# Lab-LVM/imagenet-models

Hardware: AMD Instinct MI355X
Metric: images/sec (whole node) GA-ConvNeXt-T 3x224x224 bf16 training step (higher is better)
Workload: dtype bf16; 1 GPU; ga_convnext_tiny_768 train step (fwd + GA loss lam=-0.8 + bwd + all-reduce + adamw lr=0), batch 256/GPU, drop_path 0.2, synthetic 3x224x224; global_batch=256, parallelism=dp1, dist_backend=none, grad_exchange=torch, allreduce_buckets=0

## Files before the change

### imagenet-models_amd/_lib.py

```python
import ctypes as C
import os

_HERE = os.path.dirname(os.path.abspath(__file__))
LIB_PATH = os.environ.get('GAEXT_LIB') or os.path.join(_HERE, 'csrc', 'libgaext.so')

GA_F32, GA_BF16 = 0, 1
ACT_NONE, ACT_GELU, ACT_RELU = 0, 1, 2
A_PLAIN, A_PATCH2, A_STEM4_NCHW, A_CONV3, A_CONV3S2, A_NEIGH2 = 0, 1, 2, 3, 4, 5
C_PLAIN, C_UNPATCH2 = 0, 1

vp, i32, i64, f32 = C.c_void_p, C.c_int, C.c_int64, C.c_float


class GemmDesc(C.Structure):
    _fields_ = [
        ('M', i32), ('N', i32), ('K', i32), ('batch', i32), ('dtype', i32),
        ('A', vp), ('lda', i64), ('strideA', i64), ('a_batch_mod', i32), ('a_kind', i32),
        ('a_H', i32), ('a_W', i32), ('a_C', i32), ('a_act', i32),
        ('B', vp), ('ldb', i64), ('strideB', i64),
        ('C', vp), ('ldc', i64), ('strideC', i64), ('c_kind', i32),
        ('c_H', i32), ('c_W', i32), ('c_C', i32), ('c_f32', i32), ('C2', vp), ('c2_mode', i32),
        ('alpha', f32), ('bias', vp), ('strideBias', i64), ('act', i32),
        ('H', vp), ('ldh', i64), ('strideH', i64), ('h_is_deriv', i32),
        ('rowscale', vp), ('rows_per_scale', i32),
        ('R', vp), ('ldr', i64), ('strideR', i64), ('relu_after', i32),
        ('colsum', vp), ('colsumsq', vp), ('strideCol', i64),
    ]


class WgradDesc(C.Structure):
    _fields_ = [
        ('M', i32), ('N', i32), ('K', i32), ('batch', i32), ('dtype', i32),
        ('Y', vp), ('ldy', i64), ('strideY', i64),
        ('X', vp), ('ldx', i64), ('strideX', i64), ('x_batch_mod', i32), ('x_kind', i32),
        ('x_H', i32), ('x_W', i32), ('x_C', i32), ('x_act', i32),
        ('dW', vp), ('ldw', i64), ('strideW', i64),
        ('dbias', vp), ('strideDbias', i64),
        ('alpha', f32), ('split_m', i32), ('accumulate', i32), ('workspace', vp), ('ws_bytes', i64),
    ]


class WprepDesc(C.Structure):
    _fields_ = [
        ('w', vp), ('G', i32), ('Co', i32), ('Ci', i32), ('KH', i32), ('KW', i32),
        ('rs', vp), ('cs', vp), ('row_perm', vp), ('dtype', i32),
        ('out', vp), ('ldo', i64), ('outT', vp), ('ldt', i64), ('flip', i32), ('stem', i32), ('t_cols', i32),
    ]


class WunfoldDesc(C.Structure):
    _fields_ = [
        ('G', vp), ('ldg', i64), ('gb', vp), ('W', vp), ('b', vp), ('rs', vp), ('cs', vp), ('v', vp), ('row_perm', vp),
        ('N', i32), ('Ci', i32), ('KH', i32), ('KW', i32), ('stem', i32),
        ('dW', vp), ('db', vp), ('d_rs', vp), ('d_cs', vp), ('d_v', vp),
    ]


class SmallDesc(C.Structure):
    _fields_ = [('kind', i32), ('y', vp), ('x', vp), ('a', f32), ('n', i64), ('R', i32), ('C', i32), ('accumulate', i32),
                ('b', vp), ('rs', vp), ('v', vp), ('row_perm', vp)]


class CswinAttnDesc(C.Structure):
    _fields_ = [('B', i32), ('reso', i32), ('C', i32), ('heads', i32), ('nbranch', i32),
                ('Hs', i32 * 2), ('Ws', i32 * 2), ('lepe_w', vp * 2), ('lepe_b', vp * 2),
                ('scale', f32), ('dtype', i32), ('qkv', vp), ('ldq', i64), ('out', vp), ('ldo', i64)]


class MlpDesc(C.Structure):
    _fields_ = [('X', vp), ('ldx', i64), ('W1', vp), ('ldw1', i64), ('b1', vp), ('W2', vp), ('ldw2', i64), ('b2', vp),
                ('R', vp), ('ldr', i64), ('rowscale', vp), ('rows_per_scale', i32), ('Y', vp), ('ldy', i64),
                ('M', i64), ('C', i32), ('H', i32), ('dtype', i32)]


class MlpBwdDesc(C.Structure):
    _fields_ = [('X', vp), ('ldx', i64), ('DY', vp), ('lddy', i64), ('W1', vp), ('ldw1', i64), ('b1', vp),
                ('W2T', vp), ('ldw2t', i64), ('W1T', vp), ('ldw1t', i64), ('A', vp), ('lda', i64), ('DH', vp), ('lddh', i64),
                ('DX', vp), ('lddx', i64), ('M', i64), ('C', i32), ('H', i32), ('dtype', i32)]


class SmallLinearDesc(C.Structure):
    _fields_ = [('rows', i32), ('groups', i32), ('Ng', i32), ('Kg', i32), ('A', vp), ('lda', i64), ('a_gstride', i64), ('a_perm', vp),
                ('W', vp), ('bias', vp), ('col_scale', vp), ('rowscale', vp), ('rows_per_scale', i32), ('R', vp), ('ldr', i64),
                ('Y', vp), ('ldy', i64), ('Yraw', vp), ('dtype', i32)]


class AttnDesc(C.Structure):
    _fields_ = [('B', i32), ('N', i32), ('H', i32), ('hd', i32), ('scale', f32), ('dtype', i32), ('qkv', vp), ('ldq', i64),
                ('out', vp), ('ldo', i64), ('lse', vp)]


_SIGS = {
    'ga_version': ([], i32),
    'ga_last_error': ([C.c_char_p, C.c_size_t], i32),
    'ga_device_info': ([C.POINTER(i32), C.POINTER(i32), C.POINTER(i32)], i32),
    'ga_comm_unique_id': ([vp], i32),
    'ga_comm_init': ([C.POINTER(vp), i32, i32, vp], i32),
    'ga_comm_destroy': ([vp], i32),
    'ga_comm_info': ([vp, C.POINTER(i32), C.POINTER(i32)], i32),
    'ga_allreduce_workspace': ([i64, i32], C.c_size_t),
    'ga_allreduce_bucket': ([vp, vp, i64, i32, f32, vp, C.c_size_t, vp], i32),
    'ga_reduce_scatter_bucket': ([vp, vp, vp, i64, f32, vp], i32),
    'ga_allgather_bucket': ([vp, vp, vp, i64, vp], i32),
    'ga_comm_broadcast': ([vp, vp, i64, i32, vp], i32),
    'ga_set_knob': ([C.c_char_p, i32], i32),
    'ga_unset_knob': ([C.c_char_p], i32),
    'ga_config_string': ([C.c_char_p, C.c_size_t], i32),
    'ga_gemm': ([C.POINTER(GemmDesc), vp], i32),
    'ga_wgrad': ([C.POINTER(WgradDesc), vp], i32),
    'ga_weight_prep': ([C.POINTER(WprepDesc), vp], i32),
    'ga_bias_fold': ([vp, vp, vp, vp, vp, vp, i32, i32, vp], i32),
    'ga_weight_unfold': ([C.POINTER(WunfoldDesc), vp], i32),
    'ga_dwconv7_fwd': ([vp, vp, vp, vp, i32, i32, i32, i32, i32, vp], i32),
    'ga_dwconv7_bwd_data': ([vp, vp, vp, vp, i32, i32, i32, i32, i32, vp], i32),
    'ga_dwconv7_bwd_data2': ([vp, vp, vp, vp, vp, vp, i32, i32, i32, i32, i32, vp], i32),
    'ga_dwconv7_bwd_weight': ([vp, vp, vp, vp, i32, i32, i32, i32, i32, vp, C.c_size_t, vp], i32),
    'ga_dwconv7_bwd_weight_workspace': ([i32, i32, i32, i32, i32], C.c_size_t),
    'ga_dwconv3_fwd': ([vp, vp, vp, i32, i32, i32, i32, i32, vp, vp, i32, vp], i32),
    'ga_dwconv3_bwd_data': ([vp, vp, vp, i32, i32, i32, i32, i32, i32, vp], i32),
    'ga_dwconv3_bwd_weight': ([vp, vp, vp, i32, i32, i32, i32, i32, i32, vp, C.c_size_t, vp], i32),
    'ga_dwconv3_bwd_weight_workspace': ([i32, i32, i32, i32, i32, i32], C.c_size_t),
    'ga_maxpool3s2_fwd': ([vp, vp, vp, i32, i32, i32, i32, i32, vp], i32),
    'ga_maxpool3s2_bwd': ([vp, vp, vp, i32, i32, i32, i32, i32, i32, vp], i32),
    'ga_bn_gelu_fwd': ([vp, vp, vp, vp, i64, i32, i32, vp], i32),
    'ga_bn_gelu_bwd_workspace': ([i64, i32], C.c_size_t),
    'ga_bn_gelu_bwd_reduce': ([vp, vp, vp, vp, vp, vp, vp, vp, i64, i32, i32, vp, C.c_size_t, vp], i32),
    'ga_bn_gelu_bwd_apply': ([vp, vp, vp, vp, vp, vp, vp, vp, vp, i64, vp, i64, i32, i32, vp], i32),
    'ga_se_bn_fwd': ([vp, i32, vp, vp, vp, vp, vp, vp, vp, vp, vp, vp, vp, vp, vp, vp, i32, i32, i32, i32, vp], i32),
    'ga_se_bn_bwd': ([vp, vp, vp, vp, vp, vp, vp, vp, i32, vp, vp, vp, vp, vp, vp, vp, vp, vp, vp, vp, vp, vp, vp, vp, vp, vp, vp, vp,
                      vp, vp, i32, i32, i32, vp], i32),
    'ga_se_residual_fwd': ([vp, vp, vp, vp, vp, vp, vp, vp, vp, i32, i32, i32, i32, vp], i32),
    'ga_se_residual_bwd_a': ([vp, vp, vp, vp, vp, vp, vp, vp, i32, i32, i32, i32, vp], i32),
    'ga_se_residual_bwd_b': ([vp, vp, vp, vp, vp, vp, vp, vp, vp, vp, vp, i32, i32, i32, i32, vp], i32),
    'ga_subsample2_fwd': ([vp, vp, i32, i32, i32, i32, i32, vp], i32),
    'ga_subsample2_bwd': ([vp, vp, i32, i32, i32, i32, i32, i32, vp], i32),
    'ga_wgrad_workspace': ([C.POINTER(WgradDesc)], C.c_size_t),
    'ga_layernorm_fwd': ([vp, vp, vp, vp, vp, vp, i64, i32, f32, i32, vp], i32),
    'ga_layernorm_bwd': ([vp, vp, vp, vp, vp, vp, vp, vp, vp, i64, i32, i32, i32, vp], i32),
    'ga_layernorm_bwd_dp': ([vp, vp, vp, vp, vp, vp, vp, vp, vp, i64, i32, i32, vp, vp, i64, i32, vp], i32),
    'ga_bn_finalize': ([vp, vp, i64, vp, vp, f32, f32, vp, vp, vp, vp, vp, vp, i32, i32, vp], i32),
    'ga_affine_act': ([vp, vp, vp, vp, vp, i64, vp, i64, i32, i32, i32, i64, vp], i32),
    'ga_bn_bwd_reduce': ([vp, vp, vp, vp, vp, vp, i64, vp, vp, i64, i32, i32, i64, vp], i32),
    'ga_bn_bwd_apply': ([vp, vp, vp, vp, vp, vp, vp, vp, vp, i64, i64, vp, i64, i32, i32, i64, i64, vp], i32),
    'ga_pool_concat_fwd': ([vp, vp, i32, i32, i32, i32, i32, i32, i32, i32, i32, i32, vp], i32),
    'ga_pool_concat_bwd': ([vp, vp, vp, i32, i32, i32, i32, i32, i32, i32, i32, i32, i32, vp], i32),
    'ga_spatial_sum': ([vp, vp, vp, i32, i32, i32, f32, i32, vp], i32),
    'ga_se_mlp_fwd': ([vp, vp, vp, vp, vp, vp, vp, i32, i32, i32, vp], i32),
    'ga_se_mlp_bwd': ([vp, vp, vp, vp, vp, vp, vp, f32, vp, vp, vp, vp, i32, i32, i32, vp], i32),
    'ga_chan_scale': ([vp, vp, vp, vp, i32, i32, i32, i32, vp], i32),
    'ga_gram_pack_fwd': ([vp, vp, vp, i32, i32, i32, i32, i32, vp], i32),
    'ga_gram_pack_bwd': ([vp, vp, vp, vp, i32, i32, i32, i32, i32, vp], i32),
    'ga_gram_f64_fwd_workspace': ([i32, i32], C.c_size_t),
    'ga_gram_f64_bwd_workspace': ([i32, i32], C.c_size_t),
    'ga_gram_f64_fwd': ([vp, vp, vp, vp, C.c_size_t, i32, i32, i32, i32, i32, i32, i32, vp], i32),
    'ga_gram_f64_bwd': ([vp, vp, vp, vp, vp, vp, C.c_size_t, i32, i32, i32, i32, i32, i32, i32, vp], i32),
    'ga_token_cat': ([vp, vp, vp, i32, i32, i32, i32, vp], i32),
    'ga_token_split': ([vp, vp, vp, i32, i32, i32, i32, i32, i32, vp], i32),
    'ga_class_attn_fwd': ([vp, vp, vp, vp, i32, i32, i32, i32, f32, i32, vp], i32),
    'ga_class_attn_bwd': ([vp, vp, vp, vp, vp, vp, i32, i32, i32, i32, f32, i32, vp], i32),
    'ga_class_attn_fwd2': ([vp, vp, vp, i64, vp, vp, i32, i32, i32, i32, f32, i32, vp], i32),
    'ga_class_attn_bwd2': ([vp, vp, vp, vp, i64, vp, vp, vp, vp, i32, i32, i32, i32, f32, i32, vp], i32),
    'ga_loss_fwd_bwd': ([vp, vp, vp, vp, i32, i32, i32, f32, i32, f32, f32, i32, vp], i32),
    'ga_heads_topk': ([vp, i32, i32, i32, i32, vp, vp, vp], i32),
    'ga_sgd_step': ([vp, vp, vp, vp, i64, i32, f32, vp], i32),
    'ga_adamw_step': ([vp, vp, vp, vp, vp, i64, f32, vp], i32),
    'ga_weight_prep_batch': ([vp, i32, vp], i32),
    'ga_weight_unfold_batch': ([vp, i32, vp], i32),
    'ga_small_batch': ([vp, i32, vp], i32),
    'ga_cswin_attn_fwd': ([C.POINTER(CswinAttnDesc), vp], i32),
    'ga_cswin_attn_bwd_workspace': ([C.POINTER(CswinAttnDesc)], C.c_size_t),
    'ga_cswin_attn_bwd': ([C.POINTER(CswinAttnDesc), vp, vp, vp, C.c_size_t, vp], i32),
    'ga_cswin_lepe_wgrad_reduce': ([C.POINTER(CswinAttnDesc), vp, vp, vp, vp, vp, vp], i32),
    'ga_cswin_lepe_wgrad': ([C.POINTER(CswinAttnDesc), vp, vp, vp, vp, vp, vp], i32),
    'ga_layernorm_gelu_fwd': ([vp, vp, vp, vp, vp, vp, i64, i32, f32, i32, vp], i32),
    'ga_layernorm_gelu_bwd': ([vp, vp, vp, vp, vp, vp, vp, vp, vp, i64, i32, i32, vp], i32),
    'ga_nchw3_to_nhwc8': ([vp, vp, i32, i32, i32, i32, vp], i32),
    'ga_convw_pack': ([vp, vp, i32, i32, i32, i32, i64, i32, vp], i32),
    'ga_convw_unpack_grad': ([vp, vp, i32, i32, i32, i32, i64, vp], i32),
    'ga_conv3s2_dgrad_prep': ([vp, vp, i32, i32, i64, i32, vp], i32),
    'ga_gram_pack_fwd2': ([vp, vp, vp, i32, i32, i32, i32, i32, i32, vp], i32),
    'ga_gram_pack_bwd2': ([vp, vp, vp, vp, i32, i32, i32, i32, i32, i32, vp], i32),
    'ga_map_tokens_fwd': ([vp, vp, i32, i32, i32, i32, i32, vp], i32),
    'ga_map_tokens_bwd': ([vp, vp, i32, i32, i32, i32, i32, vp], i32),
    'ga_class_attn_mt_fwd': ([vp, vp, vp, i64, vp, vp, vp, i32, i32, i32, i32, i32, f32, i32, vp], i32),
    'ga_class_attn_mt_bwd': ([vp, vp, vp, vp, i64, vp, vp, vp, vp, vp, i64, i32, i32, i32, i32, i32, f32, i32, vp], i32),
    'ga_class_attn_mt_ia_fwd': ([vp, vp, vp, i64, vp, vp, vp, vp, vp, vp, vp, i32, i32, i32, i32, i32, f32, i32, vp], i32),
    'ga_class_attn_mt_ia_bwd': ([vp, vp, vp, vp, i64, vp, vp, vp, vp, vp, vp, vp, vp, i64, vp, vp, vp, vp, i32, i32, i32, i32, i32, f32, i32,
                                 vp], i32),
    'ga_map_loss_fwd_bwd': ([vp, vp, vp, vp, vp, vp, i32, i32, i32, f32, i32, f32, f32, i32, vp], i32),
    'ga_gelu_fwd': ([vp, vp, i64, i32, vp], i32),
    'ga_gelu_bwd': ([vp, vp, vp, i64, i32, vp], i32),
    'ga_relu_drop': ([vp, vp, vp, vp, i64, i32, vp], i32),
    'ga_mask_mul': ([vp, vp, vp, vp, i64, i32, vp], i32),
    'ga_copy2d': ([vp, i64, vp, i64, i64, i32, i32, i32, vp], i32),
    'ga_dropout_mask_sample': ([vp, i64, f32, C.c_uint64, vp, vp], i32),
    'ga_drop_path_sample': ([vp, vp, i32, i32, C.c_uint64, vp, vp], i32),
    'ga_loss_dense_fwd_bwd': ([vp, vp, vp, vp, vp, vp, vp, i32, i32, i32, f32, i32, f32, f32, f32, i32, vp], i32),
    'ga_u8_normalize': ([vp, vp, i32, i32, i32, i32, C.POINTER(f32), C.POINTER(f32), vp], i32),
    'ga_input_erase': ([vp, i32, vp, i32, i32, i32, i32, C.POINTER(f32), C.POINTER(f32), vp, i32, i32, C.c_uint64, C.c_uint64, vp], i32),
    'ga_mixup_batch': ([vp, vp, i32, i32, i32, i32, C.c_double, i32, i32, i32, i32, i32, vp], i32),
    'ga_mixup_target': ([vp, vp, i32, i32, C.c_double, C.c_double, vp], i32),
    'ga_agc_clip': ([vp, vp, vp, i32, f32, f32, vp], i32),
    'ga_small_linear_fwd': ([C.POINTER(SmallLinearDesc), vp], i32),
    'ga_small_linear_bwd': ([C.POINTER(SmallLinearDesc), vp, vp, i32, vp, vp, vp, vp], i32),
    'ga_colstats': ([vp, i64, i32, i32, vp, vp, i32, vp], i32),
    'ga_pad_copy_f32': ([vp, vp, i64, i64, i64, i64, i32, vp], i32),
    'ga_pad_copy': ([vp, vp, i64, i64, i64, i64, i32, i32, vp], i32),
    'ga_stem4_ln_fwd': ([vp, vp, i64, vp, vp, vp, vp, vp, vp, vp, i32, i32, i32, i32, f32, vp], i32),
    'ga_blockdiag_f32': ([vp, vp, i64, i32, i32, i32, i64, i32, i32, vp], i32),
    'ga_pad_groups_f32': ([vp, vp, i64, i64, i32, i32, i32, i32, i32, i32, vp], i32),
    'ga_attn_fwd': ([C.POINTER(AttnDesc), vp], i32),
    'ga_attn_bwd_workspace': ([C.POINTER(AttnDesc)], C.c_size_t),
    'ga_attn_bwd': ([C.POINTER(AttnDesc), vp, vp, vp, C.c_size_t, vp], i32),
    'ga_patchify': ([vp, vp, i32, i32, i32, i32, i32, i32, vp], i32),
    'ga_vit_embed_fwd': ([vp, vp, vp, vp, i32, i32, i32, i32, vp], i32),
    'ga_vit_embed_bwd': ([vp, vp, vp, vp, i32, i32, i32, i32, vp], i32),
    'ga_patchify_strided': ([vp, vp, i32, i32, i32, i32, i32, i32, i32, vp], i32),
    'ga_pos_add_fwd': ([vp, vp, vp, i32, i32, i32, i32, vp], i32),
    'ga_pos_add_bwd': ([vp, vp, i32, i32, i32, i32, vp], i32),
    'ga_dwpool_fwd': ([vp, vp, vp, vp, i32, i32, i32, i32, i32, i32, vp], i32),
    'ga_dwpool_bwd_data': ([vp, vp, vp, i32, i32, i32, i32, i32, i32, vp], i32),
    'ga_dwpool_bwd_weight': ([vp, vp, vp, vp, i32, i32, i32, i32, i32, i32, vp], i32),
    'ga_resize_concat_fwd': ([vp, vp, i32, i32, i32, i32, i32, i32, i64, i32, i32, vp], i32),
    'ga_resize_concat_bwd': ([vp, vp, i32, i32, i32, i32, i32, i32, i64, i32, i32, vp], i32),
    'ga_rows_bcast': ([vp, vp, i32, i32, i32, f32, i32, vp], i32),
    'ga_token_gap_fwd': ([vp, vp, i32, i32, i32, i32, vp], i32),
    'ga_token_gap_bwd': ([vp, vp, i32, i32, i32, i32, vp], i32),
    'ga_mlp_supported': ([i32, i32, i32], i32),
    'ga_mlp_fwd': ([C.POINTER(MlpDesc), vp], i32),
    'ga_mlp_bwd': ([C.POINTER(MlpBwdDesc), vp], i32),
    'ga_memset': ([vp, i32, C.c_size_t, vp], i32),
    'ga_transpose_f32': ([vp, vp, i32, i32, i32, vp], i32),
    'ga_axpy_f32': ([vp, vp, f32, i64, vp], i32),
    'ga_lerp_f32': ([vp, vp, f32, i64, vp], i32),
    'ga_sumsq_f32': ([vp, i64, vp, vp], i32),
    'ga_lamb_stage1': ([vp, vp, vp, vp, vp, vp, vp, vp, i32, vp, vp], i32),
    'ga_lamb_stage2': ([vp, vp, vp, vp, i32, vp, vp], i32),
    'ga_clip_grad_f32': ([vp, i64, vp, f32, i32, vp], i32),
    'ga_rowscale': ([vp, vp, vp, i64, i64, i32, vp], i32),
    'ga_cast_from_f32': ([vp, vp, i64, i32, vp], i32),
    'ga_cast_to_f32': ([vp, vp, i64, i32, vp], i32),
}

_lib = None


def load():
    global _lib
    if _lib is not None:
        return _lib
    if not os.path.exists(LIB_PATH):
        raise RuntimeError(f'libgaext.so not found at {LIB_PATH}: build it with `make -C {os.path.dirname(LIB_PATH)}` '
                           f'(there is no CPU fallback for the product path)')
    lib = C.CDLL(LIB_PATH)
    for name, (argtypes, restype) in _SIGS.items():
        fn = getattr(lib, name)
        fn.argtypes = argtypes
        fn.restype = restype
    _lib = lib
    return lib


def last_error():
    buf = C.create_string_buffer(512)
    load().ga_last_error(buf, 512)
    return buf.value.decode(errors='replace')


def config_string():
    buf = C.create_string_buffer(1024)
    load().ga_config_string(buf, 1024)
    s = buf.value.decode(errors='replace')
    host = sorted(k for k in os.environ if k.startswith(('GAEXT_', 'GA_FUSED_MLP')) and k != 'GAEXT_LIB')
    known = {'GAEXT_ASYNC_WGRAD', 'GAEXT_FWD_SPLIT', 'GAEXT_PAR_BRANCH', 'GAEXT_FWD_SKEW', 'GAEXT_FUSE_DP', 'GAEXT_HEAD_STREAMS',
             'GA_FUSED_MLP', 'GAEXT_SMALL_SINGLE', 'GAEXT_SYNC_DEBUG'}
    for k in host:
        if k in known:
            s += f' host:{k}={os.environ[k]}'
    if os.environ.get('GAEXT_LIB'):
        s += f' lib={os.environ["GAEXT_LIB"]}'
    return s


class knobs:

    def __init__(self, **kv):
        self.kv = kv

    def __enter__(self):
        lib = load()
        for k, v in self.kv.items():
            check(lib.ga_set_knob(k.encode(), int(v)), f'ga_set_knob({k})')
        return self

    def __exit__(self, *exc):
        lib = load()
        for k in self.kv:
            lib.ga_unset_knob(k.encode())
        return False


def check(rc, what):
    if rc != 0:
        raise RuntimeError(f'libgaext {what} failed (code {rc}): {last_error()}')


def exported_symbols():
    return sorted(_SIGS)
```

### imagenet-models_amd/csrc/mlp.hip

```cpp
#include <stdlib.h>
#include <algorithm>
#include "common.h"

namespace {

constexpr int BM = 128;

__device__ __forceinline__ void lds_barrier() { asm volatile("s_waitcnt lgkmcnt(0)\n\ts_barrier" ::: "memory"); }

__device__ __forceinline__ unsigned slab_off(int r, int c) { return r * 64 + ((c ^ ((r >> 2) & 3)) << 4); }

__device__ __forceinline__ bf16x8_t frag(const unsigned char* slab, int r0, int lane) {
    return *reinterpret_cast<const bf16x8_t*>(slab + slab_off(r0 + (lane & 15), lane >> 4));
}

template <int ROWS, int KS, int NTHR>
__device__ __forceinline__ void stage_rows(unsigned char* dst, const bf16_t* src, long ld, long row0, long limit) {
    constexpr int CPR = KS * 4, NP = ROWS * CPR / NTHR;
    static_assert(ROWS * CPR % NTHR == 0, "tile must split evenly over the threads");
    u32x4_t v[NP];
#pragma unroll
    for (int i = 0; i < NP; ++i) {
        const int idx = threadIdx.x + NTHR * i;
        const int r = idx / CPR, c = idx - r * CPR;
        v[i] = u32x4_t{0, 0, 0, 0};
        if (row0 + r < limit) v[i] = __builtin_nontemporal_load(reinterpret_cast<const u32x4_t*>(src + (row0 + r) * ld + c * 8));
    }
#pragma unroll
    for (int i = 0; i < NP; ++i) {
        const int idx = threadIdx.x + NTHR * i;
        const int r = idx / CPR, c = idx - r * CPR;
        *reinterpret_cast<u32x4_t*>(dst + (c >> 2) * ROWS * 64 + slab_off(r, c & 3)) = v[i];
    }
}

template <int C, int NTHR> struct RowPre {
    static constexpr int P8 = C / 8, RG = NTHR / P8, NR = (64 + RG - 1) / RG;
};
template <int C, int NTHR> using PreArr = u32x4_t[BM / 64][RowPre<C, NTHR>::NR];
template <int C, int NTHR>
__device__ __forceinline__ void rows_prefetch(PreArr<C, NTHR>& v, const bf16_t* R, long ldr, long m0, long M) {
    using P = RowPre<C, NTHR>;
    const int c8 = threadIdx.x % P::P8, rg = threadIdx.x / P::P8;
#pragma unroll
    for (int piece = 0; piece < BM / 64; ++piece)
#pragma unroll
        for (int it = 0; it < P::NR; ++it) {
            const int row = rg + it * P::RG;
            const long m = m0 + piece * 64 + row;
            v[piece][it] = u32x4_t{0, 0, 0, 0};
            if (rg < P::RG && row < 64 && m < M) v[piece][it] = __builtin_nontemporal_load(reinterpret_cast<const u32x4_t*>(R + m * ldr + c8 * 8));
        }
}

template <int C, int NTHR, int NWM, int TM>
__device__ __forceinline__ void store_rows(float* Cs, const f32x4_t (&acc)[C / 32][TM], int wm, int wn, int lane, long m0, long M,
                                           const float* bias, const float* rowscale, int rps, bool has_r,
                                           const PreArr<C, NTHR>& pre, bf16_t* Y, long ldy) {
    constexpr int LDC = C + 4, P8 = C / 8, RG = NTHR / P8, WROWS = 16 * TM, WPH = 64 / WROWS;
    constexpr int NR = (64 + RG - 1) / RG;
    const int c8 = threadIdx.x % P8, rg = threadIdx.x / P8;
    float bv[8];
#pragma unroll
    for (int j = 0; j < 8; ++j) bv[j] = bias ? bias[c8 * 8 + j] : 0.f;
#pragma unroll
    for (int piece = 0; piece < NWM / WPH; ++piece) {
        if (piece) __syncthreads();
        if (wm / WPH == piece) {
#pragma unroll
            for (int tn = 0; tn < C / 32; ++tn)
#pragma unroll
                for (int tm = 0; tm < TM; ++tm) {
                    const int row = (wm % WPH) * WROWS + 16 * tm + (lane & 15), col = wn * (C / 2) + 16 * tn + 4 * (lane >> 4);
                    *reinterpret_cast<f32x4_t*>(Cs + row * LDC + col) = acc[tn][tm];
                }
        }
        __syncthreads();
        if (rg < RG) {
#pragma unroll
            for (int it = 0; it < NR; ++it) {
                const int row = rg + it * RG;
                const long m = m0 + piece * 64 + row;
                if (row >= 64 || m >= M) break;
                const f32x4_t a = *reinterpret_cast<const f32x4_t*>(Cs + row * LDC + c8 * 8);
                const f32x4_t b = *reinterpret_cast<const f32x4_t*>(Cs + row * LDC + c8 * 8 + 4);
                float v[8] = {a[0], a[1], a[2], a[3], b[0], b[1], b[2], b[3]};
#pragma unroll
                for (int j = 0; j < 8; ++j) v[j] += bv[j];
                if (rowscale) {
                    const float s = rowscale[m / rps];
#pragma unroll
                    for (int j = 0; j < 8; ++j) v[j] *= s;
                }
                if (has_r) {
                    float r[8];
                    const u32x4_t q = pre[piece][it];
                    unpack8(make_uint4(q.x, q.y, q.z, q.w), r);
#pragma unroll
                    for (int j = 0; j < 8; ++j) v[j] += r[j];
                }
                store8_nt(Y + m * ldy + c8 * 8, v);
            }
        }
    }
}

template <int C, int HC>
__global__ __launch_bounds__(256, 2) void mlp_fwd_kernel(const ga_mlp_desc d) {
    constexpr int KS1 = C / 32, KS2 = HC / 32, TN1 = HC / 32, TN2 = C / 32;
    constexpr int XS = KS1 * BM * 64, W1S = KS1 * HC * 64, AS = KS2 * BM * 64;
    constexpr int NI = HC * C / 8 / 256;
    static_assert(HC * C / 8 % 256 == 0, "weight chunk must split evenly");
    extern __shared__ __attribute__((aligned(16))) unsigned char smem[];
    unsigned char* Xs = smem;
    unsigned char* W1s = Xs + XS;
    unsigned char* As = W1s + W1S;
    unsigned char* W2s = As + AS;
    float* B1s = reinterpret_cast<float*>(W2s + KS2 * C * 64);
    const int tid = threadIdx.x, lane = tid & 63, wave = tid >> 6, wm = wave >> 1, wn = wave & 1, g = lane >> 4;
    const long m0 = (long)blockIdx.x * BM;
    const bf16_t* W1 = reinterpret_cast<const bf16_t*>(d.W1);
    const bf16_t* W2 = reinterpret_cast<const bf16_t*>(d.W2);

    u32x4_t w1r[NI], w2r[NI];
    auto w_load = [&](int j0) {
#pragma unroll
        for (int i = 0; i < NI; ++i) {
            const int idx = tid + 256 * i;
            const int r1 = idx / (KS1 * 4), c1 = idx - r1 * (KS1 * 4);
            w1r[i] = *reinterpret_cast<const u32x4_t*>(W1 + (long)(j0 + r1) * d.ldw1 + c1 * 8);
            const int r2 = idx / (HC / 8), c2 = idx - r2 * (HC / 8);
            w2r[i] = *reinterpret_cast<const u32x4_t*>(W2 + (long)r2 * d.ldw2 + j0 + c2 * 8);
        }
    };
    auto w1_store = [&]() {
#pragma unroll
        for (int i = 0; i < NI; ++i) {
            const int idx = tid + 256 * i;
            const int r1 = idx / (KS1 * 4), c1 = idx - r1 * (KS1 * 4);
            *reinterpret_cast<u32x4_t*>(W1s + (c1 >> 2) * HC * 64 + slab_off(r1, c1 & 3)) = w1r[i];
        }
    };
    auto w2_store = [&]() {
#pragma unroll
        for (int i = 0; i < NI; ++i) {
            const int idx = tid + 256 * i;
            const int r2 = idx / (HC / 8), c2 = idx - r2 * (HC / 8);
            *reinterpret_cast<u32x4_t*>(W2s + (c2 >> 2) * C * 64 + slab_off(r2, c2 & 3)) = w2r[i];
        }
    };

    w_load(0);
    stage_rows<BM, KS1, 256>(Xs, reinterpret_cast<const bf16_t*>(d.X), d.ldx, m0, d.M);
    for (int i = tid; i < 4 * C; i += 256) B1s[i] = d.b1[i];
    w1_store();
    w2_store();
    __syncthreads();

    f32x4_t y[TN2][4];
#pragma unroll
    for (int i = 0; i < TN2; ++i)
#pragma unroll
        for (int j = 0; j < 4; ++j) y[i][j] = f32x4_t{0.f, 0.f, 0.f, 0.f};
    auto round = [&](const int j0, const bool more) __attribute__((always_inline)) {
        if (more) w_load(j0 + HC);
        f32x4_t h[TN1][4];
#pragma unroll
        for (int i = 0; i < TN1; ++i)
#pragma unroll
            for (int j = 0; j < 4; ++j) h[i][j] = f32x4_t{0.f, 0.f, 0.f, 0.f};
#pragma unroll
        for (int ks = 0; ks < KS1; ++ks) {
            bf16x8_t xf[4];
#pragma unroll
            for (int tm = 0; tm < 4; ++tm) xf[tm] = frag(Xs + ks * BM * 64, wm * 64 + 16 * tm, lane);
#pragma unroll
            for (int tn = 0; tn < TN1; ++tn) {
                const bf16x8_t wf = frag(W1s + ks * HC * 64, wn * (HC / 2) + 16 * tn, lane);
#pragma unroll
                for (int tm = 0; tm < 4; ++tm) h[tn][tm] = __builtin_amdgcn_mfma_f32_16x16x32_bf16(wf, xf[tm], h[tn][tm], 0, 0, 0);
            }
        }
#pragma unroll
        for (int tn = 0; tn < TN1; ++tn) {
            const int nl = wn * (HC / 2) + 16 * tn + 4 * g;
            const float4 b = *reinterpret_cast<const float4*>(B1s + j0 + nl);
            const float bb[4] = {b.x, b.y, b.z, b.w};
#pragma unroll
            for (int tm = 0; tm < 4; ++tm) {
                float a[4], unused;
#pragma unroll
                for (int r = 0; r < 4; ++r) gelu_both_fast(h[tn][tm][r] + bb[r], a[r], unused);
                const int row = wm * 64 + 16 * tm + (lane & 15);
                uint2 p;
                p.x = pack2bf(a[0], a[1]);
                p.y = pack2bf(a[2], a[3]);
                *reinterpret_cast<uint2*>(As + (nl >> 5) * BM * 64 + slab_off(row, (nl & 31) >> 3) + (nl & 7) * 2) = p;
            }
        }
        lds_barrier();
#pragma unroll
        for (int ks = 0; ks < KS2; ++ks) {
            bf16x8_t af[4];
#pragma unroll
            for (int tm = 0; tm < 4; ++tm) af[tm] = frag(As + ks * BM * 64, wm * 64 + 16 * tm, lane);
#pragma unroll
            for (int tn = 0; tn < TN2; ++tn) {
                const bf16x8_t wf = frag(W2s + ks * C * 64, wn * (C / 2) + 16 * tn, lane);
#pragma unroll
                for (int tm = 0; tm < 4; ++tm) y[tn][tm] = __builtin_amdgcn_mfma_f32_16x16x32_bf16(wf, af[tm], y[tn][tm], 0, 0, 0);
            }
        }
        if (more) w1_store();
        lds_barrier();
        if (more) w2_store();
    };
    for (int j0 = 0; j0 + HC < d.H; j0 += HC) round(j0, true);
    u32x4_t rpre[BM / 64][RowPre<C, 256>::NR];
    if (d.R) rows_prefetch<C, 256>(rpre, reinterpret_cast<const bf16_t*>(d.R), d.ldr, m0, d.M);
    round(d.H - HC, false);
    store_rows<C, 256, 2, 4>(reinterpret_cast<float*>(smem), y, wm, wn, lane, m0, d.M, d.b2, d.rowscale, d.rows_per_scale,
                             d.R != nullptr, rpre, reinterpret_cast<bf16_t*>(d.Y), d.ldy);
}

template <int C, int HC> constexpr int fwd_lds() {
    constexpr int ab = (C / 32) * BM * 64 + (C / 32) * HC * 64 + (HC / 32) * BM * 64 + (HC / 32) * C * 64 + 16 * C;
    constexpr int st = 64 * (C + 4) * 4;
    return ab > st ? ab : st;
}

template <int C, int HC>
__global__ __launch_bounds__(512, 1) void mlp_bwd_kernel(const ga_mlp_bwd_desc d) {
    constexpr int KS1 = C / 32, KS2 = HC / 32, TN1 = HC / 32, TN2 = C / 32;
    constexpr int XS = KS1 * BM * 64, WS = KS1 * HC * 64, TS = KS2 * BM * 64;
    constexpr int NPC = HC * C / 8, NI = (NPC + 511) / 512;
    extern __shared__ __attribute__((aligned(16))) unsigned char smem[];
    unsigned char* Xs = smem;
    unsigned char* Ds = Xs + XS;
    unsigned char* W1s = Ds + XS;
    unsigned char* W2Ts = W1s + WS;
    unsigned char* W1Ts = W2Ts + WS;
    unsigned char* DHs = W1Ts + KS2 * C * 64;
    unsigned char* A2s = DHs + TS;
    float* B1s = reinterpret_cast<float*>(A2s + TS);
    const int tid = threadIdx.x, lane = tid & 63, wave = tid >> 6, wm = wave >> 1, wn = wave & 1, g = lane >> 4;
    const long m0 = (long)blockIdx.x * BM;
    const bf16_t* W1 = reinterpret_cast<const bf16_t*>(d.W1);
    const bf16_t* W2T = reinterpret_cast<const bf16_t*>(d.W2T);
    const bf16_t* W1T = reinterpret_cast<const bf16_t*>(d.W1T);
    bf16_t* Aout = reinterpret_cast<bf16_t*>(d.A);
    bf16_t* DHout = reinterpret_cast<bf16_t*>(d.DH);

    u32x4_t w1r[NI], w2r[NI], w3r[NI];
    auto w_load = [&](int j0) {
#pragma unroll
        for (int i = 0; i < NI; ++i) {
            const int idx = NPC % 512 == 0 ? tid + 512 * i : min(tid + 512 * i, NPC - 1);
            const int r1 = idx / (KS1 * 4), c1 = idx - r1 * (KS1 * 4);
            w1r[i] = *reinterpret_cast<const u32x4_t*>(W1 + (long)(j0 + r1) * d.ldw1 + c1 * 8);
            w2r[i] = *reinterpret_cast<const u32x4_t*>(W2T + (long)(j0 + r1) * d.ldw2t + c1 * 8);
            const int r3 = idx / (HC / 8), c3 = idx - r3 * (HC / 8);
            w3r[i] = *reinterpret_cast<const u32x4_t*>(W1T + (long)r3 * d.ldw1t + j0 + c3 * 8);
        }
    };
    auto w12_store = [&]() {
#pragma unroll
        for (int i = 0; i < NI; ++i) {
            const int idx = NPC % 512 == 0 ? tid + 512 * i : min(tid + 512 * i, NPC - 1);
            const int r1 = idx / (KS1 * 4), c1 = idx - r1 * (KS1 * 4);
            const unsigned o = (c1 >> 2) * HC * 64 + slab_off(r1, c1 & 3);
            *reinterpret_cast<u32x4_t*>(W1s + o) = w1r[i];
            *reinterpret_cast<u32x4_t*>(W2Ts + o) = w2r[i];
        }
    };
    auto w3_store = [&]() {
#pragma unroll
        for (int i = 0; i < NI; ++i) {
            const int idx = NPC % 512 == 0 ? tid + 512 * i : min(tid + 512 * i, NPC - 1);
            const int r3 = idx / (HC / 8), c3 = idx - r3 * (HC / 8);
            *reinterpret_cast<u32x4_t*>(W1Ts + (c3 >> 2) * C * 64 + slab_off(r3, c3 & 3)) = w3r[i];
        }
    };

    w_load(0);
    stage_rows<BM, KS1, 512>(Xs, reinterpret_cast<const bf16_t*>(d.X), d.ldx, m0, d.M);
    stage_rows<BM, KS1, 512>(Ds, reinterpret_cast<const bf16_t*>(d.DY), d.lddy, m0, d.M);
    for (int i = tid; i < 4 * C; i += 512) B1s[i] = d.b1[i];
    w12_store();
    w3_store();
    __syncthreads();

    f32x4_t dx[TN2][2];
#pragma unroll
    for (int i = 0; i < TN2; ++i)
#pragma unroll
        for (int j = 0; j < 2; ++j) dx[i][j] = f32x4_t{0.f, 0.f, 0.f, 0.f};

    for (int j0 = 0; j0 < d.H; j0 += HC) {
        const bool more = j0 + HC < d.H;
        if (more) w_load(j0 + HC);
        f32x4_t h[TN1][2], t[TN1][2];
#pragma unroll
        for (int i = 0; i < TN1; ++i)
#pragma unroll
            for (int j = 0; j < 2; ++j) h[i][j] = t[i][j] = f32x4_t{0.f, 0.f, 0.f, 0.f};
#pragma unroll
        for (int ks = 0; ks < KS1; ++ks) {
            bf16x8_t xf[2], df[2];
#pragma unroll
            for (int tm = 0; tm < 2; ++tm) {
                xf[tm] = frag(Xs + ks * BM * 64, wm * 32 + 16 * tm, lane);
                df[tm] = frag(Ds + ks * BM * 64, wm * 32 + 16 * tm, lane);
            }
#pragma unroll
            for (int tn = 0; tn < TN1; ++tn) {
                const bf16x8_t w1f = frag(W1s + ks * HC * 64, wn * (HC / 2) + 16 * tn, lane);
                const bf16x8_t w2f = frag(W2Ts + ks * HC * 64, wn * (HC / 2) + 16 * tn, lane);
#pragma unroll
                for (int tm = 0; tm < 2; ++tm) {
                    h[tn][tm] = __builtin_amdgcn_mfma_f32_16x16x32_bf16(w1f, xf[tm], h[tn][tm], 0, 0, 0);
                    t[tn][tm] = __builtin_amdgcn_mfma_f32_16x16x32_bf16(w2f, df[tm], t[tn][tm], 0, 0, 0);
                }
            }
        }
#pragma unroll
        for (int tn = 0; tn < TN1; ++tn) {
            const int nl = wn * (HC / 2) + 16 * tn + 4 * g;
            const float4 b = *reinterpret_cast<const float4*>(B1s + j0 + nl);
            const float bb[4] = {b.x, b.y, b.z, b.w};
#pragma unroll
            for (int tm = 0; tm < 2; ++tm) {
                float a[4], dh[4];
#pragma unroll
                for (int r = 0; r < 4; ++r) {
                    float gr;
                    gelu_both_fast(h[tn][tm][r] + bb[r], a[r], gr);
                    dh[r] = t[tn][tm][r] * gr;
                }
                const int row = wm * 32 + 16 * tm + (lane & 15);
                const unsigned o = (nl >> 5) * BM * 64 + slab_off(row, (nl & 31) >> 3) + (nl & 7) * 2;
                uint2 p;
                p.x = pack2bf(a[0], a[1]);
                p.y = pack2bf(a[2], a[3]);
                *reinterpret_cast<uint2*>(A2s + o) = p;
                p.x = pack2bf(dh[0], dh[1]);
                p.y = pack2bf(dh[2], dh[3]);
                *reinterpret_cast<uint2*>(DHs + o) = p;
            }
        }
        lds_barrier();
#pragma unroll
        for (int ks = 0; ks < KS2; ++ks) {
            bf16x8_t af[2];
#pragma unroll
            for (int tm = 0; tm < 2; ++tm) af[tm] = frag(DHs + ks * BM * 64, wm * 32 + 16 * tm, lane);
#pragma unroll
            for (int tn = 0; tn < TN2; ++tn) {
                const bf16x8_t wf = frag(W1Ts + ks * C * 64, wn * (C / 2) + 16 * tn, lane);
#pragma unroll
                for (int tm = 0; tm < 2; ++tm) dx[tn][tm] = __builtin_amdgcn_mfma_f32_16x16x32_bf16(wf, af[tm], dx[tn][tm], 0, 0, 0);
            }
        }
        {
            constexpr int PPR = HC / 8, NP = BM * PPR / 512;
            static_assert(BM * PPR % 512 == 0, "chunk rows must split evenly");
#pragma unroll
            for (int i = 0; i < NP; ++i) {
                const int idx = tid + 512 * i;
                const int r = idx / PPR, c = idx - r * PPR;
                const long m = m0 + r;
                if (m < d.M) {
                    const unsigned o = (c >> 2) * BM * 64 + slab_off(r, c & 3);
                    store16_nt(Aout + m * d.lda + j0 + c * 8, *reinterpret_cast<const uint4*>(A2s + o));
                    store16_nt(DHout + m * d.lddh + j0 + c * 8, *reinterpret_cast<const uint4*>(DHs + o));
                }
            }
        }
        if (more) w12_store();
        lds_barrier();
        if (more) w3_store();
    }
    u32x4_t nopre[BM / 64][RowPre<C, 512>::NR];
#pragma unroll
    for (int i = 0; i < BM / 64; ++i)
#pragma unroll
        for (int j = 0; j < RowPre<C, 512>::NR; ++j) nopre[i][j] = u32x4_t{0, 0, 0, 0};
    store_rows<C, 512, 4, 2>(reinterpret_cast<float*>(smem), dx, wm, wn, lane, m0, d.M, nullptr, nullptr, 1, false, nopre,
                             reinterpret_cast<bf16_t*>(d.DX), d.lddx);
}

template <int C, int HC> constexpr int bwd_lds() {
    return 2 * (C / 32) * BM * 64 + 2 * (C / 32) * HC * 64 + (HC / 32) * C * 64 + 2 * (HC / 32) * BM * 64 + 16 * C;
}

bool aligned16(const void* p) { return (reinterpret_cast<uintptr_t>(p) & 15) == 0; }

template <typename K> bool set_lds(K kern, size_t bytes) {
    return bytes <= 65536 ||
           hipFuncSetAttribute(reinterpret_cast<const void*>(kern), hipFuncAttributeMaxDynamicSharedMemorySize, (int)bytes) == hipSuccess;
}

}

extern "C" int ga_mlp_supported(int C, int H, int dtype) { return dtype == GA_BF16 && H == 4 * C && (C == 96 || C == 192); }

extern "C" int ga_mlp_fwd(const ga_mlp_desc* d, ga_stream_t stream) {
    GA_REQUIRE(d && d->X && d->W1 && d->b1 && d->W2 && d->Y && d->M > 0, "ga_mlp_fwd: null / empty descriptor");
    GA_REQUIRE(ga_mlp_supported(d->C, d->H, d->dtype), "ga_mlp_fwd: C=%d H=%d dtype=%d has no fused form (ga_mlp_supported)", d->C,
               d->H, d->dtype);
    GA_REQUIRE(aligned16(d->X) && aligned16(d->W1) && aligned16(d->W2) && aligned16(d->Y) && aligned16(d->b1) &&
                   (!d->R || aligned16(d->R)) && d->ldx % 8 == 0 && d->ldw1 % 8 == 0 && d->ldw2 % 8 == 0 && d->ldy % 8 == 0 &&
                   (!d->R || d->ldr % 8 == 0) && d->ldx >= d->C && d->ldw1 >= d->C && d->ldw2 >= d->H && d->ldy >= d->C,
               "ga_mlp_fwd: operands must be 16-byte aligned with leading dimensions in multiples of 8");
    GA_REQUIRE(!d->rowscale || d->rows_per_scale > 0, "ga_mlp_fwd: rows_per_scale");
    hipStream_t s = reinterpret_cast<hipStream_t>(stream);
    const unsigned grid = (unsigned)((d->M + BM - 1) / BM);
    if (d->C == 96) {
        constexpr int lds = fwd_lds<96, 64>();
        GA_REQUIRE(set_lds(mlp_fwd_kernel<96, 64>, lds), "ga_mlp_fwd: LDS");
        hipLaunchKernelGGL((mlp_fwd_kernel<96, 64>), dim3(grid), dim3(256), lds, s, *d);
    } else {
        constexpr int lds = fwd_lds<192, 32>();
        GA_REQUIRE(set_lds(mlp_fwd_kernel<192, 32>, lds), "ga_mlp_fwd: LDS");
        hipLaunchKernelGGL((mlp_fwd_kernel<192, 32>), dim3(grid), dim3(256), lds, s, *d);
    }
    return ga_check_launch("ga_mlp_fwd");
}

extern "C" int ga_mlp_bwd(const ga_mlp_bwd_desc* d, ga_stream_t stream) {
    GA_REQUIRE(d && d->X && d->DY && d->W1 && d->b1 && d->W2T && d->W1T && d->A && d->DH && d->DX && d->M > 0,
               "ga_mlp_bwd: null / empty descriptor");
    GA_REQUIRE(ga_mlp_supported(d->C, d->H, d->dtype), "ga_mlp_bwd: C=%d H=%d dtype=%d has no fused form (ga_mlp_supported)", d->C,
               d->H, d->dtype);
    GA_REQUIRE(aligned16(d->X) && aligned16(d->DY) && aligned16(d->W1) && aligned16(d->W2T) && aligned16(d->W1T) &&
                   aligned16(d->A) && aligned16(d->DH) && aligned16(d->DX) && aligned16(d->b1) && d->ldx % 8 == 0 &&
                   d->lddy % 8 == 0 && d->ldw1 % 8 == 0 && d->ldw2t % 8 == 0 && d->ldw1t % 8 == 0 && d->lda % 8 == 0 &&
                   d->lddh % 8 == 0 && d->lddx % 8 == 0 && d->ldx >= d->C && d->lddy >= d->C && d->ldw1 >= d->C &&
                   d->ldw2t >= d->C && d->ldw1t >= d->H && d->lda >= d->H && d->lddh >= d->H && d->lddx >= d->C,
               "ga_mlp_bwd: operands must be 16-byte aligned with leading dimensions in multiples of 8");
    hipStream_t s = reinterpret_cast<hipStream_t>(stream);
    const unsigned grid = (unsigned)((d->M + BM - 1) / BM);
    if (d->C == 96) {
        constexpr int lds = bwd_lds<96, 64>();
        GA_REQUIRE(set_lds(mlp_bwd_kernel<96, 64>, lds), "ga_mlp_bwd: LDS");
        hipLaunchKernelGGL((mlp_bwd_kernel<96, 64>), dim3(grid), dim3(512), lds, s, *d);
    } else {
        constexpr int lds = bwd_lds<192, 32>();
        GA_REQUIRE(set_lds(mlp_bwd_kernel<192, 32>, lds), "ga_mlp_bwd: LDS");
        hipLaunchKernelGGL((mlp_bwd_kernel<192, 32>), dim3(grid), dim3(512), lds, s, *d);
    }
    return ga_check_launch("ga_mlp_bwd");
}
```

### imagenet-models_amd/engine.py

```python
import contextlib
import os

import torch

from . import ops
from .ops import (A_CONV3, A_PATCH2, A_STEM4_NCHW, ACT_GELU, ASYNC_LANE, C_UNPATCH2, GA_BF16, GA_F32, Plan)


def pad8(n):
    return (n + 7) // 8 * 8


def tap_indices(nblocks, naggre):
    taps = []
    if nblocks > 5:
        for i in range(nblocks):
            if (i + 1) % (nblocks // (naggre + 1)) == 0 and len(taps) < naggre:
                taps.append(i)
    return taps


class GAFunction(torch.autograd.Function):

    @staticmethod
    def forward(ctx, eng, x, anchor):
        ctx.eng = eng
        return eng.forward(x)

    @staticmethod
    def backward(ctx, dlogits):
        ctx.eng.backward(dlogits)
        return None, None, None


class GAEngine:
    def __init__(self, model, batch, training, mode):
        self.m = model
        self.cfg = model.cfg
        self.B = batch
        self.training = training
        self.dt = GA_BF16 if mode == 'bf16' else GA_F32
        self.tdt = ops.torch_dtype(self.dt)
        flat = model.flat_state()
        self.dev = flat['params'].device
        self.P = dict(model.named_parameters())
        self.Bf = dict(model.named_buffers())
        self.bufs = {}
        self.tmps = {}
        self.async_wgrad = os.environ.get('GAEXT_ASYNC_WGRAD', '1') != '0'
        self.fwd_split = max(1, int(os.environ.get('GAEXT_FWD_SPLIT', '2')))
        self.par_branch = os.environ.get('GAEXT_PAR_BRANCH', '1') != '0'
        self.fwd_skew = int(os.environ.get('GAEXT_FWD_SKEW', '-1'))
        self._chain = None
        self._cur_stage = 0
        self._bwd_seq = 0
        self._pre_dyz = {}
        self.fuse_dp = os.environ.get('GAEXT_FUSE_DP', '1') != '0'
        self.sync_bn = getattr(model, 'sync_bn_comm', None)
        self.W = {}
        self.weights_dirty = True
        self.anchor = torch.zeros((), device=self.dev, requires_grad=True)
        self.input_descs = []
        self.blocks = {}
        self.x_ref = None
        self.img = 224
        self.dp_rates = self._drop_path_rates()
        self.dp_scale = {}
        if training:
            sites = [pre for pre, r in self.dp_rates.items() if r > 0]
            if sites:
                self.dp_all = torch.ones(len(sites), batch, device=self.dev)
                self.dp_keep = torch.tensor([1.0 - self.dp_rates[p] for p in sites], device=self.dev)
                self.dp_counter = torch.zeros(1, dtype=torch.int64, device=self.dev)
                self.dp_plan = Plan(name='droppath')
                self.dp_plan.drop_path_sample(self.dp_all, self.dp_keep, len(sites), batch, torch.initial_seed(), self.dp_counter)
                for i, pre in enumerate(sites):
                    self.dp_scale[pre] = self.dp_all[i]
        self.arena = None
        self.arena_off = 0
        if training:
            self.arena = torch.zeros(int(flat['total'] * 1.15) + (1 << 20) + self._arena_extra(), device=self.dev)
        self._nbt = [t for n, t in self.Bf.items() if n.endswith('num_batches_tracked')]
        self.prep = Plan(name='prep', defer_small=True)
        self.fwd = Plan(name='fwd')
        self.bwd = Plan(name='bwd', defer_small=True) if training else None
        self.bn_pool = torch.zeros(1 << 16, device=self.dev)
        self.bn_pool_off = 0
        self.bott_prefix = 'stages.4.'
        self.ppad, self.pgrad = {}, {}
        self.pad_gmlp = os.environ.get('GAEXT_PAD_GMLP', '1') != '0'
        self._build()
        assert not self.pgrad or getattr(self, '_unpadded', False), 'padded parameter gradients were never copied back'

    def buf(self, name, shape, dtype=None, zero=False):
        dtype = dtype or self.tdt
        if name not in self.bufs:
            self.bufs[name] = (torch.zeros if zero else torch.empty)(shape, dtype=dtype, device=self.dev)
        t = self.bufs[name]
        assert tuple(t.shape) == tuple(shape) and t.dtype == dtype, name
        return t

    def _chains(self):
        n = self.fwd_split if self.B >= 2 * self.fwd_split else 1
        if n <= 1:
            return [(0, 0, self.B)]
        per = self.B // n
        cuts = [s_ * per for s_ in range(n)] + [self.B]
        return [(1 + s_, cuts[s_], cuts[s_ + 1]) for s_ in range(n)]

    def _fsplits(self, HW):
        ch = getattr(self, '_chain', None)
        if ch is None:
            return [(0, 0, self.B * HW, 0, self.B)]
        lane, b0, b1 = ch
        return [(lane, b0 * HW, b1 * HW, b0, b1)]

    @contextlib.contextmanager
    def _wlane(self):
        Bk = self.bwd
        prev = Bk.lane
        if self.async_wgrad and prev == 0:
            Bk.lane = ASYNC_LANE
        try:
            yield
        finally:
            Bk.lane = prev

    def tmp(self, tag, shape, dtype=None):
        dtype = dtype or self.tdt
        key = (getattr(self, 'tmp_prefix', '') + tag, tuple(shape), dtype)
        if key not in self.tmps:
            self.tmps[key] = torch.empty(shape, dtype=dtype, device=self.dev)
        return self.tmps[key]

    def act(self, name, shape, dtype=None):
        return self.buf(name, shape, dtype)

    def blk_act(self, name, shape, dtype=None):
        return self.buf(name, shape, dtype) if self.training else self.tmp(name.rsplit('.', 1)[-1], shape, dtype)

    def gbuf(self, shape):
        n = 1
        for s in shape:
            n *= s
        off = (self.arena_off + 63) // 64 * 64
        assert off + n <= self.arena.numel(), 'gradient scratch arena too small'
        self.arena_off = off + n
        return self.arena[off:off + n].view(shape)

    def grad(self, name):
        return self.P[name].grad

    def _drop_path_rates(self):
        dep = self.cfg['depths']
        rate = self.cfg['drop_path_rate']
        pts = torch.linspace(0, rate, sum(dep)).split(list(dep))
        out = {}
        for i in range(4):
            for j in range(dep[i]):
                out[f'stages.{i}.blocks.{j}.'] = float(pts[i][j])
        out['stages.4.'] = float(rate)
        for k in range(self.cfg['branches']):
            out[f'gram_layer.{k}.blocks.0.'] = float(pts[-1][0])
            out[f'ga.{k}.'] = 0.0
        return out

    def sample_drop_path(self):
        if self.dp_scale:
            self.dp_plan.run()

    def set_drop_path_masks(self, masks):
        for pre, t in self.dp_scale.items():
            t.copy_(masks[pre].to(self.dev).float())

    NAMES = dict(stem_conv='stem.0.', stem_ln='stem.1.', ds_ln='stages.{i}.downsample.0.', ds_conv='stages.{i}.downsample.1.',
                 block='stages.{i}.blocks.{j}.', dw='conv_dw.', fc1='mlp.fc1.', fc2='mlp.fc2.')

    def _build(self):
        cfg = self.cfg
        d = cfg['dims']
        B, T, F = self.B, self.training, self.fwd
        dt = self.dt
        feats, taps, stage_in, _ = self._build_trunk()
        Hc = 14
        M4 = B * Hc * Hc
        ctot = sum(d[:-1]) + d[2] * cfg['naggre']
        cat = self.act('agg.cat', (M4, ctot))
        segs = [(feats[0][0], feats[0][1], d[0], 0), (feats[1][0], feats[1][1], d[1], 0)]
        segs += [(t, feats[2][1], d[2], 0) for t in taps]
        segs += [(feats[2][0], feats[2][1], d[2], 0), (feats[3][0], feats[3][1], d[3], 1)]
        off = 0
        self.agg_segs = []
        for src, hw, c, mode in segs:
            F.pool_concat_fwd(src, cat, B, hw, hw, c, Hc, Hc, ctot, off, mode, dt, label=f'agg.{off}')
            self.agg_segs.append((src, hw, c, mode, off))
            off += c
        assert off == ctot
        x4 = self._bottleneck_fwd(cat, M4, ctot, d[4])
        self.cout = d[4]
        self._build_heads(x4, M4, Hc)
        if T:
            self._build_backward(feats, taps, stage_in, x4, M4, ctot)
            if self.async_wgrad:
                self.bwd.join_async()
            self.bwd.flush('end.')
        self.prep.flush('prep.')

    def _build_trunk(self):
        cfg, nm = self.cfg, self.NAMES
        d, dep = cfg['dims'], cfg['depths']
        B, T, F = self.B, self.training, self.fwd
        dt = self.dt
        S0 = self.img // 4
        self.x_in = None
        M0 = B * S0 * S0
        if T:
            F.zero(self.bn_pool, label='zero.bn_sums')
        sc, sl = nm['stem_conv'], nm['stem_ln']
        Wst = self._w_plain(sc + 'weight', d[0], 3, 4, 4, stem=True, need_T=False)
        stem_pre = self.act('stem.pre', (M0, d[0]))
        self.x_placeholder = torch.zeros(8, device=self.dev)
        mean = self.act('stem.mean', (M0,), torch.float32)
        rstd = self.act('stem.rstd', (M0,), torch.float32)
        x = self.buf('stem.out', (M0, d[0]))
        self.stem_call = None
        if dt == GA_BF16 and d[0] in (96, 128) and self.img % 4 == 0 and os.environ.get('GAEXT_STEM_FUSED', '1') != '0':
            self.stem_call = len(F.calls)
            F.stem4_ln_fwd(self.x_placeholder, Wst, Wst.shape[1], self.P[sc + 'bias'], self.P[sl + 'weight'], self.P[sl + 'bias'],
                           stem_pre, x, mean, rstd, B, self.img, self.img, d[0], 1e-6, label='stem.conv+ln')
        else:
            F.gemm(self.x_placeholder, Wst, stem_pre, M0, d[0], 48, dt, a_kind=A_STEM4_NCHW, a_dims=(self.img, self.img, 3),
                   bias=self.P[sc + 'bias'], label='stem.conv')
            self.input_descs.append(self._last_desc(F))
            F.layernorm_fwd(stem_pre, self.P[sl + 'weight'], self.P[sl + 'bias'], x, mean, rstd, M0, d[0], 1e-6, dt,
                            label='stem.ln')
        x_stem = x
        chains = self._chains()
        skew_ev = None
        for ci, chain in enumerate(chains):
            self._chain = chain if len(chains) > 1 else None
            if self._chain is not None and skew_ev is not None:
                F.lane_wait(chain[0], skew_ev)
                skew_ev = None
            feats, taps = [], []
            x = x_stem
            res = S0
            stage_in = []
            for i in range(4):
                if i > 0:
                    Hp = res
                    res //= 2
                    Mi = B * res * res
                    Mp = B * Hp * Hp
                    pre = f'stages.{i}.downsample.'
                    pln, pcv = nm['ds_ln'].format(i=i), nm['ds_conv'].format(i=i)
                    ln = self.act(pre + 'ln', (Mp, d[i - 1]))
                    mean = self.act(pre + 'mean', (Mp,), torch.float32)
                    rstd = self.act(pre + 'rstd', (Mp,), torch.float32)
                    Wd = self._w_plain(pcv + 'weight', d[i], d[i - 1], 2, 2)
                    xo = self.buf(pre + 'out', (Mi, d[i]))
                    for lane, r0, r1, b0, b1 in self._fsplits(Hp * Hp):
                        F.lane = lane
                        F.layernorm_fwd(x[r0:r1], self.P[pln + 'weight'], self.P[pln + 'bias'], ln[r0:r1], mean[r0:r1],
                                        rstd[r0:r1], r1 - r0, d[i - 1], 1e-6, dt, label=pre + 'ln')
                        F.gemm(ln[r0:r1], Wd, xo[r0 // 4:r1 // 4], (r1 - r0) // 4, d[i], 4 * d[i - 1], dt, a_kind=A_PATCH2,
                               a_dims=(Hp, Hp, d[i - 1]), bias=self.P[pcv + 'bias'], label=pre + 'conv')
                    F.lane = 0
                    stage_in.append((x, Hp))
                    x = xo
                tap_at = tap_indices(dep[i], cfg['naggre']) if i == 2 else []
                for j in range(dep[i]):
                    x = self._block_fwd(nm['block'].format(i=i, j=j), x, res, d[i])
                    if j in tap_at:
                        taps.append(x)
                feats.append((x, res))
                if self._chain is not None and i == self.fwd_skew and ci + 1 < len(chains):
                    skew_ev = F.lane_signal(chain[0])
        self._chain = None
        return feats, taps, stage_in, x_stem

    def _build_heads(self, x4, M4, Hc):
        cfg, B, T, F, dt = self.cfg, self.B, self.training, self.fwd, self.dt
        cout = self.cout
        NC, K = cfg['num_classes'], cfg['branches']
        assert NC % 8 == 0, 'num_classes must be a multiple of 8 (pad the classifier)'
        self.logits = self.buf('logits', (K, B, NC), torch.float32)
        self.heads = []
        E_, nh_ = cfg['dim_embed'], cfg['num_heads']
        hd_ = E_ // max(nh_, 1)
        self.hd_p = pad8(hd_)
        self.Ea = nh_ * self.hd_p
        self.shared_tok = E_ % nh_ == 0 and self.Ea <= 512
        if self.shared_tok and self.Ea != E_:
            for k in range(K):
                pre = f'ga.{k}.attn.'
                pk, pv = self.P[pre + 'k.weight'], self.P[pre + 'v.weight']
                assert pv.data_ptr() == pk.data_ptr() + pk.numel() * 4, 'k/v weights must be adjacent in the flat buffer'
                spec = (('k.weight', (2 * self.Ea, cout), 2 * nh_, hd_ * cout, hd_ * cout, self.hd_p * cout),
                        ('q.weight', (self.Ea, cout), nh_, hd_ * cout, hd_ * cout, self.hd_p * cout),
                        ('proj.weight', (cout, self.Ea), cout * nh_, hd_, hd_, self.hd_p))
                for name, shape, rows, cols, lds, ldd in spec:
                    buf = self.buf('pad.' + pre + name, shape, torch.float32, zero=True)
                    self.prep.pad_copy_f32(self.P[pre + name], buf, rows, cols, lds, ldd, label='prep.pad.' + pre + name)
                    self.ppad[pre + name] = (buf, 'copy', (rows, cols, lds, ldd))
        if self.shared_tok:
            self.tok = dict(xn=self.act('ga.tok.xn', (M4, cout)), rstd=self.act('ga.tok.rstd', (M4,), torch.float32))
            F.layernorm_fwd(x4, None, None, self.tok['xn'], None, self.tok['rstd'], M4, cout, 1e-5, dt, label='ga.tok.ln')
            E2 = 2 * self.Ea
            tk = self.tok
            tk['E2'], tk['ld'] = E2, K * E2
            tk['W'] = self.buf('w.ga.kv_all', (K * E2, cout))
            tk['WT'] = self.buf('wT.ga.kv_all', (cout, K * E2)) if T else None
            tk['b'] = self.buf('w.ga.bkv_all', (K * E2,), torch.float32)
            P = self.P
            for k in range(K):
                pre = f'ga.{k}.'
                pk, pv = P[pre + 'attn.k.weight'], P[pre + 'attn.v.weight']
                assert pv.data_ptr() == pk.data_ptr() + pk.numel() * 4, 'k/v weights must be adjacent in the flat buffer'
                pk = self._pw(pre + 'attn.k.weight')
                self.prep.weight_prep(pk, 1, E2, cout, 1, 1, dt, out=tk['W'][k * E2:], ldo=cout,
                                      outT=tk['WT'][:, k * E2:] if T else None, ldt=K * E2 if T else 0,
                                      cs=P[pre + 'norm1.weight'], t_cols=E2, label='prep.' + pre + 'kv')
                self.prep.bias_fold(pk, None, None, P[pre + 'norm1.bias'], tk['b'][k * E2:], E2, cout)
            tk['kv'] = self.act('ga.kv_all', (M4, K * E2))
            F.gemm(tk['xn'], tk['W'], tk['kv'], M4, K * E2, cout, dt, bias=tk['b'], label='ga.kv_all')
        self._contract_all_fwd(x4, M4)
        fa = self.fc_all = dict(x=self.act('fc.all.x', (K, B, cout)))
        ldn = pad8(NC)
        fa['W'] = self.buf('w.fc.all', (K, NC, cout))
        fa['WT'] = self.buf('wT.fc.all', (K, cout, ldn)) if T else None
        fa['b'] = self.buf('w.fc.ball', (K, NC), torch.float32)
        for k in range(K):
            self.prep.weight_prep(self.P[f'fc.{k}.weight'], 1, NC, cout, 1, 1, dt, out=fa['W'][k], ldo=cout,
                                  outT=fa['WT'][k] if T else None, ldt=ldn if T else 0, label=f'prep.fc.{k}')
            self.prep.bias_fold(None, self.P[f'fc.{k}.bias'], None, None, fa['b'][k], NC, cout)
        self.head_lanes = int(os.environ.get('GAEXT_HEAD_STREAMS', '5')) if self.shared_tok else 1
        for k in range(K):
            if self.head_lanes > 1:
                F.lane, self.tmp_prefix = 1 + k % self.head_lanes, f'h{k}.'
            self.heads.append(self._head_fwd(k, x4, M4, cout, Hc))
        F.lane, self.tmp_prefix = 0, ''
        F.gemm(fa['x'], fa['W'], self.logits, B, NC, cout, dt, batch=K, strideA=B * cout, strideB=NC * cout, strideC=B * NC,
               bias=fa['b'], strideBias=NC, c_f32=True, label='fc.all')

    def _arena_extra(self):
        cfg = self.cfg
        d = cfg.get('dims')
        if not d or len(d) < 5 or any(k not in cfg for k in ('gram_dim', 'gram_groups', 'mlp_groups', 'dim_embed', 'num_heads', 'branches')):
            return 0
        cout, g, groups = d[4], cfg['gram_dim'], cfg['gram_groups']
        if cout % (8 * groups) == 0 and cout % (8 * cfg['mlp_groups']) == 0 and (cfg['dim_embed'] // max(cfg['num_heads'], 1)) % 8 == 0:
            return 0
        cp = cout + 8 * max(groups, cfg['mlp_groups'])
        return cfg['branches'] * (cp * (g * (g + 1) // 2 // groups + 8) + 8 * cp * cp // cfg['mlp_groups'] + 4 * cp * 512) + (1 << 20)

    def _pw(self, name):
        return self.ppad[name][0] if name in self.ppad else self.P[name]

    def _pg(self, name):
        if name not in self.ppad:
            return self.grad(name)
        if name not in self.pgrad:
            self.pgrad[name] = self.gbuf(tuple(self.ppad[name][0].shape))
        return self.pgrad[name]

    def _pad_groups(self, name, R, Cdim, RG, RGp, CG, CGp):
        if name not in self.ppad:
            buf = self.buf('pad.' + name, (R // RG * RGp, Cdim // CG * CGp), torch.float32, zero=True)
            self.prep.pad_groups_f32(self.P[name], buf, R, Cdim, RG, RGp, CG, CGp, label='prep.pad.' + name)
            self.ppad[name] = (buf, 'groups', (R, Cdim, RG, RGp, CG, CGp))
        return self.ppad[name][0]

    def _unpad_all(self):
        self._unpadded = True
        for name, g in self.pgrad.items():
            _, kind, a = self.ppad[name]
            if kind == 'copy':
                rows, cols, lds, ldd = a
                self.bwd.pad_copy_f32(g, self.grad(name), rows, cols, ldd, lds, accumulate=True, label=name + '.unpad')
            else:
                self.bwd.pad_groups_f32(g, self.grad(name), *a, unpad=True, accumulate=True, label=name + '.unpad')

    def _contract_all_fwd(self, x4, M4):
        cfg, T, F, dt, cout = self.cfg, self.training, self.fwd, self.dt, self.cout
        K = cfg['branches']
        g_ = cfg['gram_dim']
        gc = self.gcon = dict(ld=K * g_)
        gc['W'] = self.buf('w.gram_contraction.all', (K * g_, cout))
        gc['WT'] = self.buf('wT.gram_contraction.all', (cout, K * g_)) if T else None
        gc['b'] = self.buf('w.gram_contraction.ball', (K * g_,), torch.float32)
        gc['s'], gc['q'] = self._bn_pool(K * g_), self._bn_pool(K * g_)
        for k in range(K):
            pre = f'gram_contraction.{k}.'
            self.prep.weight_prep(self.P[pre + '0.weight'], 1, g_, cout, 1, 1, dt, out=gc['W'][k * g_:], ldo=cout,
                                  outT=gc['WT'][:, k * g_:] if T else None, ldt=K * g_ if T else 0, t_cols=g_,
                                  label='prep.' + pre + 'w')
            self.prep.bias_fold(None, self.P[pre + '0.bias'], None, None, gc['b'][k * g_:], g_, cout)
        gc['out'] = self.act('gram_contraction.all.out', (M4, K * g_))
        F.gemm(x4, gc['W'], gc['out'], M4, K * g_, cout, dt, bias=gc['b'], colsum=gc['s'] if T else None,
               colsumsq=gc['q'] if T else None, label='gram_contraction.all')

    @staticmethod
    def _last_desc(plan):
        for obj in reversed(plan.keep):
            if hasattr(obj, '_fields_'):
                return obj
        raise RuntimeError('no descriptor')

    def _w_plain(self, name, Co, Ci, KH, KW, stem=False, need_T=True, flip=False, groups=1, rs=None, cs=None,
                 row_perm=None, ldo=None, key=None, src=None):
        key = key or name
        if key in self.W:
            return self.W[key]
        KK = Ci * KH * KW
        ldo = ldo or pad8(KK)
        out = self.buf('w.' + key, (groups * Co, ldo))
        outT = None
        ldt = 0
        if need_T and self.training:
            if flip:
                ldt = pad8(KH * KW * Co)
                outT = self.buf('wT.' + key, (groups * Ci, ldt))
            else:
                ldt = pad8(Co)
                outT = self.buf('wT.' + key, (groups * KK, ldt))
            self.W[key + '.T'] = outT
        self.prep.weight_prep(self.P[name] if src is None else src, groups, Co, Ci, KH, KW, self.dt, out=out, ldo=ldo, outT=outT, ldt=ldt, rs=rs,
                              cs=cs, flip=flip, stem=stem, row_perm=row_perm, label='prep.' + key)
        self.W[key] = out
        return out

    def _block_weights(self, pre, C):
        if pre + 'w49' in self.W:
            return
        P = self.P
        w49 = self.buf('w.' + pre + 'w49', (49, C), torch.float32)
        self.prep.transpose_f32(P[pre + self.NAMES['dw'] + 'weight'], w49, C, 49, label='prep.' + pre + 'w49')
        self.W[pre + 'w49'] = w49
        self._w_plain(pre + self.NAMES['fc1'] + 'weight', 4 * C, C, 1, 1, cs=P[pre + 'norm.weight'])
        b1e = self.buf('w.' + pre + 'b1e', (4 * C,), torch.float32)
        self.prep.bias_fold(P[pre + self.NAMES['fc1'] + 'weight'], P[pre + self.NAMES['fc1'] + 'bias'], None, P[pre + 'norm.bias'], b1e, 4 * C, C)
        self.W[pre + 'b1e'] = b1e
        self._w_plain(pre + self.NAMES['fc2'] + 'weight', C, 4 * C, 1, 1, rs=P[pre + 'gamma'])
        b2e = self.buf('w.' + pre + 'b2e', (C,), torch.float32)
        self.prep.bias_fold(None, P[pre + self.NAMES['fc2'] + 'bias'], P[pre + 'gamma'], None, b2e, C, 4 * C)
        self.W[pre + 'b2e'] = b2e

    def _block_fwd(self, pre, x, res, C):
        assert C % 8 == 0
        F, dt, B = self.fwd, self.dt, self.B
        M = B * res * res
        self._block_weights(pre, C)
        W = self.W
        u = self.tmp('u', (M, C))
        xn = self.blk_act(pre + 'xn', (M, C))
        rstd = self.blk_act(pre + 'rstd', (M,), torch.float32)
        fused = self._mlp_fused(C)
        a = None if fused else self.blk_act(pre + 'a', (M, 4 * C))
        g = self.buf(pre + 'g', (M, 4 * C)) if (self.training and not fused) else None
        y = self.buf(pre + 'y', (M, C))
        dp = self.dp_scale.get(pre)
        cur = F.lane
        for lane, r0, r1, b0, b1 in (self._fsplits(res * res) if cur == 0 else [(cur, 0, M, 0, B)]):
            F.lane = lane
            F.dwconv7_fwd(x[r0:r1], W[pre + 'w49'], self.P[pre + self.NAMES['dw'] + 'bias'], u[r0:r1], b1 - b0, res, res, C, dt,
                          label=pre + 'dw')
            F.layernorm_fwd(u[r0:r1], None, None, xn[r0:r1], None, rstd[r0:r1], r1 - r0, C, 1e-6, dt, label=pre + 'ln')
            if fused:
                F.mlp_fwd(xn[r0:r1], W[pre + self.NAMES['fc1'] + 'weight'], W[pre + 'b1e'], W[pre + self.NAMES['fc2'] + 'weight'],
                          W[pre + 'b2e'], y[r0:r1], r1 - r0, C, dt, R=x[r0:r1], rowscale=dp[b0:b1] if dp is not None else None,
                          rows_per_scale=res * res, label=pre + 'mlp')
                continue
            F.gemm(xn[r0:r1], W[pre + self.NAMES['fc1'] + 'weight'], a[r0:r1], r1 - r0, 4 * C, C, dt, bias=W[pre + 'b1e'], act=ACT_GELU,
                   C2=g[r0:r1] if g is not None else None, c2_mode=2 if g is not None else 0, label=pre + 'fc1')
            F.gemm(a[r0:r1], W[pre + self.NAMES['fc2'] + 'weight'], y[r0:r1], r1 - r0, C, 4 * C, dt, bias=W[pre + 'b2e'],
                   rowscale=dp[b0:b1] if dp is not None else None, rows_per_scale=res * res, R=x[r0:r1], ldr=C,
                   label=pre + 'fc2')
        F.lane = cur
        self.blocks[pre] = dict(x=x, xn=xn, rstd=rstd, a=a, g=g, y=y, res=res, C=C, fused=fused)
        return y

    def _mlp_fused(self, C):
        allowed = [int(v) for v in os.environ.get('GA_FUSED_MLP', '96').split(',') if v.strip()]
        if not self.training and 'GA_FUSED_MLP' not in os.environ:
            allowed.append(192)
        return C in allowed and ops.mlp_supported(C, 4 * C, self.dt)

    def _block_bwd(self, pre, dy, dx, next_pre=None):
        Bk, dt, B, P, W = self.bwd, self.dt, self.B, self.P, self.W
        b = self.blocks[pre]
        res, C = b['res'], b['C']
        M = B * res * res
        dp = self.dp_scale.get(pre)
        dyz = dy
        par, dz_tag = '', 'dyz'
        if self.async_wgrad and Bk.lane == 0:
            self._bwd_seq += 1
            par = str(self._bwd_seq & 1)
            dz_tag = f'dyz{self._bwd_seq % 3}'
            Bk.join_async(f'blk{self._bwd_seq - 2}')
        if dp is not None:
            if pre in self._pre_dyz:
                dyz = self._pre_dyz.pop(pre)
            else:
                dyz = self.tmp(dz_tag, (M, C))
                Bk.rowscale(dy, dp, dyz, M * C, res * res * C, dt, label=pre + 'dp')
        side = self.async_wgrad and Bk.lane == 0
        wl = ASYNC_LANE if side else Bk.lane
        ml = Bk.lane
        G2, gb2 = self.gbuf((C, 4 * C)), self.gbuf((C,))
        dh = self.tmp('dh' + par, (M, 4 * C))
        gb1 = self.gbuf((4 * C,))
        G1 = self.gbuf((4 * C, C))
        g = self.tmp('g', (M, C))
        if b['fused']:
            a = self.tmp('a' + par, (M, 4 * C))
            Bk.mlp_bwd(b['xn'], dyz, W[pre + self.NAMES['fc1'] + 'weight'], W[pre + 'b1e'], W[pre + self.NAMES['fc2'] + 'weight.T'],
                       W[pre + self.NAMES['fc1'] + 'weight.T'], a, dh, g, M, C, dt, label=pre + 'mlpb')
            Bk.lane = wl
            Bk.wgrad(dyz, a, G2, M, C, 4 * C, dt, dbias=gb2, label=pre + 'wg2')
            Bk.wgrad(dh, b['xn'], G1, M, 4 * C, C, dt, dbias=gb1, label=pre + 'wg1')
            Bk.lane = ml
        else:
            Bk.lane = wl
            Bk.wgrad(dyz, b['a'], G2, M, C, 4 * C, dt, dbias=gb2, label=pre + 'wg2')
            Bk.lane = ml
            Bk.gemm(dyz, W[pre + self.NAMES['fc2'] + 'weight.T'], dh, M, 4 * C, C, dt, H=b['g'], ldh=4 * C, h_is_deriv=True, colsum=gb1,
                    label=pre + 'dg2')
            Bk.lane = wl
            Bk.wgrad(dh, b['xn'], G1, M, 4 * C, C, dt, label=pre + 'wg1')
            Bk.lane = ml
            Bk.gemm(dh, W[pre + self.NAMES['fc1'] + 'weight.T'], g, M, C, 4 * C, dt, label=pre + 'dg1')
        du = self.tmp('du' + par, (M, C))
        Bk.layernorm_bwd(g, b['xn'], None, b['rstd'], None, None, du, None, None, M, C, True, dt, label=pre + 'lnb')
        dw49 = self.gbuf((49, C))
        Bk.lane = wl
        Bk.dwconv7_bwd_weight(du, b['x'], dw49, self.grad(pre + self.NAMES['dw'] + 'bias'), B, res, res, C, dt, label=pre + 'dww')
        Bk.lane = ml
        if side:
            Bk.async_mark(f'blk{self._bwd_seq}')
        dx2 = dp_next = None
        if next_pre is not None and self.fuse_dp:
            dp_next = self.dp_scale.get(next_pre)
            if dp_next is not None:
                nxt = f'dyz{(self._bwd_seq + 1) % 3}' if side else 'dyz'
                dx2 = self._pre_dyz[next_pre] = self.tmp(nxt, (M, C))
        Bk.dwconv7_bwd_data(du, W[pre + 'w49'], dy, dx, B, res, res, C, dt, dx2=dx2, scale2=dp_next, label=pre + 'dwd')
        Bk.weight_unfold(G2, 4 * C, C, 4 * C, gb=gb2, W=P[pre + self.NAMES['fc2'] + 'weight'], b=P[pre + self.NAMES['fc2'] + 'bias'],
                         rs=P[pre + 'gamma'], dW=self.grad(pre + self.NAMES['fc2'] + 'weight'), db=self.grad(pre + self.NAMES['fc2'] + 'bias'),
                         d_rs=self.grad(pre + 'gamma'), label=pre + 'unf2')
        Bk.weight_unfold(G1, C, 4 * C, C, gb=gb1, W=P[pre + self.NAMES['fc1'] + 'weight'], b=P[pre + self.NAMES['fc1'] + 'bias'],
                         cs=P[pre + 'norm.weight'], v=P[pre + 'norm.bias'], dW=self.grad(pre + self.NAMES['fc1'] + 'weight'),
                         db=self.grad(pre + self.NAMES['fc1'] + 'bias'), d_cs=self.grad(pre + 'norm.weight'),
                         d_v=self.grad(pre + 'norm.bias'), label=pre + 'unf1')
        Bk.transpose_f32(dw49, self.grad(pre + self.NAMES['dw'] + 'weight'), 49, C, accumulate=True, label=pre + 'unfdw')

    def _bn_pool(self, C):
        off = (self.bn_pool_off + 63) // 64 * 64
        assert off + C <= self.bn_pool.numel()
        self.bn_pool_off = off + C
        return self.bn_pool[off:off + C]

    def _bn_bufs(self, pre, C, zero=False):
        return dict(s=self._bn_pool(C), q=self._bn_pool(C),
                    mean=self.buf(pre + 'bmean', (C,), torch.float32, zero=zero), rstd=self.buf(pre + 'brstd', (C,), torch.float32, zero=zero),
                    scale=self.buf(pre + 'scale', (C,), torch.float32, zero=zero), shift=self.buf(pre + 'shift', (C,), torch.float32, zero=zero))

    def _sync_allreduce(self, plan, t, label):
        c = self.sync_bn
        plan._add('ga_allreduce_bucket', (c.handle, ops._ptr(t), t.numel(), GA_F32, 1.0, None, 0), label, keep=(t, c))

    def _bn_finalize(self, pre, bn, n, C):
        if self.sync_bn is not None and self.training:
            self._sync_allreduce(self.fwd, bn['s'], pre + 'sync.s')
            self._sync_allreduce(self.fwd, bn['q'], pre + 'sync.q')
            n = n * self.sync_bn.world
        self.fwd.bn_finalize(bn['s'], bn['q'], n, self.P[pre + 'weight'], self.P[pre + 'bias'], 1e-5, 0.1,
                             self.Bf[pre + 'running_mean'], self.Bf[pre + 'running_var'], bn['mean'], bn['rstd'],
                             bn['scale'], bn['shift'], C, self.training, label=pre + 'fin')

    def _bn_bwd(self, pre, bn, dy, y_relu, x, dx, rows, C, rowscale=None, rps=1, ldx=0, lddx=0, weight=None, c_real=None):
        Bk = self.bwd
        s1, s2 = self.gbuf((C,)), self.gbuf((C,))
        Bk.bn_bwd_reduce(dy, y_relu, x, bn['mean'], bn['rstd'], s1, s2, rows, C, self.dt, rowscale=rowscale,
                         rows_per_scale=rps, ldx=ldx, label=pre + 'bnr')
        n = rows
        if self.sync_bn is not None:
            Bk._add('ga_axpy_f32', (ops._ptr(self.grad(pre + 'weight')), ops._ptr(s2), 1.0, c_real or C), pre + 'dgamma', keep=(s2,))
            Bk._add('ga_axpy_f32', (ops._ptr(self.grad(pre + 'bias')), ops._ptr(s1), 1.0, c_real or C), pre + 'dbeta', keep=(s1,))
            self._sync_allreduce(Bk, s1, pre + 'sync.s1')
            self._sync_allreduce(Bk, s2, pre + 'sync.s2')
            n = rows * self.sync_bn.world
        Bk.bn_bwd_apply(dy, y_relu, x, bn['mean'], bn['rstd'], self.P[pre + 'weight'] if weight is None else weight, s1, s2, n, dx,
                        rows, C, self.dt, rowscale=rowscale, rows_per_scale=rps, ldx=ldx, lddx=lddx, label=pre + 'bna')
        if self.sync_bn is None:
            Bk.axpy_f32(self.grad(pre + 'weight'), s2, 1.0, c_real or C)
            Bk.axpy_f32(self.grad(pre + 'bias'), s1, 1.0, c_real or C)

    def _bott_pad(self, pre, w, wp, ctot, cout):
        P = self.P
        R = P[pre + 'se.fc1.weight'].shape[0]
        spec = {'conv1.weight': ((wp, ctot), w, ctot, ctot, ctot), 'conv2.weight': ((wp, wp, 3, 3), w, 9 * w, 9 * w, 9 * wp),
                'conv3.weight': ((cout, wp), cout, w, w, wp), 'se.fc1.weight': ((R, wp), R, w, w, wp),
                'se.fc2.weight': ((wp, R), w, R, R, R), 'se.fc2.bias': ((wp,), 1, w, w, wp)}
        for bn in ('bn1', 'bn2'):
            spec[bn + '.weight'] = ((wp,), 1, w, w, wp)
            spec[bn + '.bias'] = ((wp,), 1, w, w, wp)
        PB, back = {}, []
        for name, (shape, rows, cols, lds, ldd) in spec.items():
            buf = self.buf('pad.' + pre + name, shape, torch.float32, zero=True)
            self.prep.pad_copy_f32(P[pre + name], buf, rows, cols, lds, ldd, label='prep.pad.' + pre + name)
            PB[pre + name] = buf
            back.append((name, rows, cols, lds, ldd))
        return PB, back

    def _bottleneck_fwd(self, cat, M4, ctot, cout):
        F, dt, B, P, T = self.fwd, self.dt, self.B, self.P, self.training
        pre = self.bott_prefix
        w_real = cout // 4
        w = pad8(w_real)
        HW = M4 // B
        st = self.bott = dict(cat=cat, w=w, w_real=w_real, cout=cout, ctot=ctot, PB=None)
        if w != w_real:
            st['PB'], st['back'] = self._bott_pad(pre, w_real, w, ctot, cout)
            P = dict(P)
            P.update(st['PB'])
        st['P'] = P
        stats = T

        def conv_bn(name, bnname, A, Wt, N, Kdim, bias=None, n_real=None, **kw):
            c = self.act(pre + name + '.out', (M4, N))
            bn = self._bn_bufs(pre + bnname + '.', N, zero=bool(n_real) and n_real != N)
            F.gemm(A, Wt, c, M4, N, Kdim, dt, bias=bias, colsum=bn['s'] if stats else None,
                   colsumsq=bn['q'] if stats else None, label=pre + name, **kw)
            self._bn_finalize(pre + bnname + '.', bn, M4, n_real or N)
            return c, bn

        F.lane = ASYNC_LANE if self.par_branch else 0
        Wds = self._w_plain(pre + 'downsample.0.weight', cout, ctot, 1, 1)
        st['sc'], st['bnd'] = conv_bn('downsample.0', 'downsample.1', cat, Wds, cout, ctot, bias=P[pre + 'downsample.0.bias'])
        t = self.tmp('bott.t', (M4, cout))
        F.affine_act(st['sc'], st['bnd']['scale'], st['bnd']['shift'], None, t, M4, cout, False, dt, label=pre + 'bnd')
        F.lane = 0
        Wc1 = self._w_plain(pre + 'conv1.weight', w, ctot, 1, 1, src=P[pre + 'conv1.weight'])
        st['c1'], st['bn1'] = conv_bn('conv1', 'bn1', cat, Wc1, w, ctot, n_real=w_real)
        st['y1'] = self.act(pre + 'y1', (M4, w))
        F.affine_act(st['c1'], st['bn1']['scale'], st['bn1']['shift'], None, st['y1'], M4, w, True, dt, label=pre + 'bn1')
        Wc2 = self._w_plain(pre + 'conv2.weight', w, w, 3, 3, flip=True, src=P[pre + 'conv2.weight'])
        st['c2'], st['bn2'] = conv_bn('conv2', 'bn2', st['y1'], Wc2, w, 9 * w, n_real=w_real, a_kind=A_CONV3, a_dims=(14, 14, w))
        st['y2'] = self.act(pre + 'y2', (M4, w))
        F.affine_act(st['c2'], st['bn2']['scale'], st['bn2']['shift'], None, st['y2'], M4, w, True, dt, label=pre + 'bn2')
        R = P[pre + 'se.fc1.weight'].shape[0]
        st['R'] = R
        st['sp'] = self.act(pre + 'se.sp', (B, w), torch.float32)
        st['hid'] = self.act(pre + 'se.hid', (B, R), torch.float32)
        st['gate'] = self.act(pre + 'se.gate', (B, w), torch.float32)
        F.spatial_sum(st['y2'], None, st['sp'], B, HW, w, 1.0 / HW, dt, label=pre + 'se.pool')
        F.se_mlp_fwd(st['sp'], P[pre + 'se.fc1.weight'], P[pre + 'se.fc1.bias'], P[pre + 'se.fc2.weight'],
                     P[pre + 'se.fc2.bias'], st['hid'], st['gate'], B, w, R, label=pre + 'se.mlp')
        st['z'] = self.act(pre + 'se.z', (M4, w))
        F.chan_scale(st['y2'], st['gate'], None, st['z'], B, HW, w, dt, label=pre + 'se.scale')
        Wc3 = self._w_plain(pre + 'conv3.weight', cout, w, 1, 1, src=P[pre + 'conv3.weight'])
        st['c3'], st['bn3'] = conv_bn('conv3', 'bn3', st['z'], Wc3, cout, w)
        x4 = self.buf(pre + 'out', (M4, cout))
        if self.par_branch:
            F.join_async()
        F.affine_act(st['c3'], st['bn3']['scale'], st['bn3']['shift'], t, x4, M4, cout, True, dt,
                     rowscale=self.dp_scale.get(pre), rows_per_scale=HW, label=pre + 'bn3+add')
        st['x4'] = x4
        return x4

    def _bottleneck_bwd(self, dx4, dcat):
        Bk, dt, B, P, W = self.bwd, self.dt, self.B, self.bott['P'], self.W
        pre = self.bott_prefix
        st = self.bott
        w, cout, ctot = st['w'], st['cout'], st['ctot']
        padded = st['PB'] is not None
        GB = {pre + name: self.gbuf(tuple(st['PB'][pre + name].shape)) for name, *_ in st['back']} if padded else {}

        def grad(name):
            return GB[name] if name in GB else self.grad(name)

        M4 = dx4.shape[0]
        HW = M4 // B
        dp = self.dp_scale.get(pre)
        dc3 = self.tmp('bott.dc3', (M4, cout))
        self._bn_bwd(pre + 'bn3.', st['bn3'], dx4, st['x4'], st['c3'], dc3, M4, cout, rowscale=dp, rps=HW)
        dsc = self.tmp('bott.dsc', (M4, cout))
        with self._wlane():
            self._bn_bwd(pre + 'downsample.1.', st['bnd'], dx4, st['x4'], st['sc'], dsc, M4, cout)
            Bk.wgrad(dsc, st['cat'], self.grad(pre + 'downsample.0.weight'), M4, cout, ctot, dt,
                     dbias=self.grad(pre + 'downsample.0.bias'), label=pre + 'ds.wg')
            Bk.gemm(dsc, W[pre + 'downsample.0.weight.T'], dcat, M4, ctot, cout, dt, ldb=pad8(cout), label=pre + 'ds.dg')
        with self._wlane():
            Bk.wgrad(dc3, st['z'], grad(pre + 'conv3.weight'), M4, cout, w, dt, label=pre + 'conv3.wg')
        dz = self.tmp('bott.dz', (M4, w))
        Bk.gemm(dc3, W[pre + 'conv3.weight.T'], dz, M4, w, cout, dt, label=pre + 'conv3.dg')
        dgate = self.tmp('bott.dgate', (B, w), torch.float32)
        dsp = self.tmp('bott.dsp', (B, w), torch.float32)
        Bk.spatial_sum(dz, st['y2'], dgate, B, HW, w, 1.0, dt, label=pre + 'se.dgate')
        Bk.se_mlp_bwd(dgate, st['gate'], st['hid'], st['sp'], P[pre + 'se.fc1.weight'], P[pre + 'se.fc2.weight'], dsp,
                      grad(pre + 'se.fc1.weight'), grad(pre + 'se.fc1.bias'), grad(pre + 'se.fc2.weight'),
                      grad(pre + 'se.fc2.bias'), B, w, st['R'], ds_scale=1.0 / HW, label=pre + 'se.mlpb')
        dy2 = self.tmp('bott.dy2', (M4, w))
        Bk.chan_scale(dz, st['gate'], dsp, dy2, B, HW, w, dt, label=pre + 'se.back')
        dc2 = self.tmp('bott.dc2', (M4, w))
        self._bn_bwd(pre + 'bn2.', st['bn2'], dy2, st['y2'], st['c2'], dc2, M4, w, weight=P[pre + 'bn2.weight'] if padded else None,
                     c_real=st['w_real'])
        G = self.gbuf((w, 9 * w))
        with self._wlane():
            Bk.wgrad(dc2, st['y1'], G, M4, w, 9 * w, dt, x_kind=A_CONV3, x_dims=(14, 14, w), label=pre + 'conv2.wg')
        Bk.weight_unfold(G, 9 * w, w, w, 3, 3, dW=grad(pre + 'conv2.weight'), label=pre + 'conv2.unf')
        dy1 = self.tmp('bott.dy1', (M4, w))
        Bk.gemm(dc2, W[pre + 'conv2.weight.T'], dy1, M4, w, 9 * w, dt, a_kind=A_CONV3, a_dims=(14, 14, w),
                ldb=pad8(9 * w), label=pre + 'conv2.dg')
        dc1 = self.tmp('bott.dc1', (M4, w))
        self._bn_bwd(pre + 'bn1.', st['bn1'], dy1, st['y1'], st['c1'], dc1, M4, w, weight=P[pre + 'bn1.weight'] if padded else None,
                     c_real=st['w_real'])
        with self._wlane():
            Bk.wgrad(dc1, st['cat'], grad(pre + 'conv1.weight'), M4, w, ctot, dt, label=pre + 'conv1.wg')
        if self.async_wgrad:
            Bk.join_async()
        Bk.gemm(dc1, W[pre + 'conv1.weight.T'], dcat, M4, ctot, w, dt, ldb=pad8(w), R=dcat, ldr=ctot, label=pre + 'conv1.dg')
        if padded:
            skip = ('bn1.weight', 'bn1.bias', 'bn2.weight', 'bn2.bias')
            Bk.flush(pre + 'pad.')
            for name, rows, cols, lds, ldd in st['back']:
                if name not in skip:
                    Bk.pad_copy_f32(GB[pre + name], self.grad(pre + name), rows, cols, ldd, lds, accumulate=True, label=pre + name + '.unpad')

    def _gmlp_fwd(self, pre, t, rows, C, mg, out, R, rowscale, rps, gamma_name=None, act='gelu', drop_mask=None, ratio=4):
        F, dt, P, T = self.fwd, self.dt, self.P, self.training
        gamma = self._pw(gamma_name) if gamma_name else None
        Hd = int(ratio * C)
        gc_ = Hd // mg
        Nv = gc_ // mg
        cin = C // mg
        n_idx = torch.arange(Hd)
        perm = ((n_idx % gc_) * mg + n_idx // gc_).to(torch.int32).to(self.dev)
        if (Nv % 8 or cin % 8) and self.pad_gmlp and C % mg == 0:
            assert Hd == 4 * C, 'the padded odd-width layout is laid out for mlp_ratio 4'
            cin_p = pad8(cin)
            Cp = mg * cin_p
            self._pad_groups(pre + 'fc1.weight', Hd, cin, 4 * cin, 4 * cin_p, cin, cin_p)
            self._pad_groups(pre + 'fc1.bias', 1, Hd, 1, 1, 4 * cin, 4 * cin_p)
            self._pad_groups(pre + 'fc2.weight', C, gc_, cin, cin_p, cin, cin_p)
            self._pad_groups(pre + 'fc2.bias', 1, C, 1, 1, cin, cin_p)
            if gamma_name:
                self._pad_groups(gamma_name, 1, C, 1, 1, cin, cin_p)
            tp = self.buf(pre + 't.pad', (rows, Cp), zero=True)
            F.pad_copy(t, tp, rows * mg, cin, cin, cin_p, dt, label=pre + 't.pad')
            Rp = None
            if R is not None:
                Rp = self.buf(pre + 'R.pad', (rows, Cp), zero=True)
                F.pad_copy(R, Rp, rows * mg, cin, cin, cin_p, dt, label=pre + 'R.pad')
            outp = self.tmp('gmlp.out.pad', (rows, Cp))
            st = self._gmlp_fwd(pre, tp, rows, Cp, mg, outp, Rp, rowscale, rps, gamma_name=gamma_name, act=act, drop_mask=drop_mask)
            F.pad_copy(outp, out, rows * mg, cin, cin_p, cin, dt, label=pre + 'out.unpad')
            st['pad'] = dict(tp=tp, Cp=Cp, cin=cin, cin_p=cin_p)
            return st
        if Nv % 8 or cin % 8:
            assert act == 'gelu' and drop_mask is None and rows <= 4096, (pre, C, mg, rows)
            st = dict(naive=True, Hd=Hd, hpre=self.act(pre + 'hpre', (rows, Hd)), am=self.act(pre + 'am', (rows, Hd)),
                      yraw=self.act(pre + 'yraw', (rows, C)) if T else None)
            st['d1'] = F.small_linear_desc(t, P[pre + 'fc1.weight'], st['hpre'], rows, mg, gc_, cin, dt, lda=C, a_gstride=cin, ldy=Hd,
                                           bias=P[pre + 'fc1.bias'])
            F.small_linear_fwd(st['d1'], label=pre + 'fc1')
            F.gelu_fwd(st['hpre'], st['am'], rows * Hd, dt, label=pre + 'gelu')
            kw = dict(bias=P[pre + 'fc2.bias'], a_perm=perm, col_scale=gamma, Yraw=st['yraw'])
            d2 = F.small_linear_desc(st['am'], P[pre + 'fc2.weight'], out, rows, mg, cin, gc_, dt, lda=Hd, a_gstride=gc_, ldy=C,
                                     rowscale=rowscale, rows_per_scale=rps, R=R, ldr=C, **kw)
            F.small_linear_fwd(d2, label=pre + 'fc2')
            st['d2b'] = F.small_linear_desc(st['am'], P[pre + 'fc2.weight'], out, rows, mg, cin, gc_, dt, lda=Hd, a_gstride=gc_, ldy=C, **kw)
            return st
        assert gc_ % mg == 0, (pre, C, mg)
        Wm1 = self._w_plain(pre + 'fc1.weight', Nv, cin, 1, 1, groups=mg * mg, row_perm=perm, src=self._pw(pre + 'fc1.weight'))
        bm1 = self.buf('w.' + pre + 'bm1', (Hd,), torch.float32)
        self.prep.bias_fold(None, self._pw(pre + 'fc1.bias'), None, None, bm1, Hd, cin, row_perm=perm)
        st = dict(perm=perm, Hd=Hd, gc=gc_, Nv=Nv, cin=cin)
        st['am'] = self.act(pre + 'am', (rows, Hd))
        st['gm'] = self.act(pre + 'gm', (rows, Hd)) if T else None
        if act == 'gelu':
            assert drop_mask is None
            F.gemm(t, Wm1, st['am'], rows, Nv, cin, dt, lda=C, batch=mg * mg, strideA=cin, a_batch_mod=mg,
                   strideB=Nv * pad8(cin), ldb=pad8(cin), ldc=Hd, strideC=Nv, bias=bm1, strideBias=Nv, act=ACT_GELU,
                   C2=st['gm'], c2_mode=2 if T else 0, label=pre + 'fc1')
        else:
            two = T or drop_mask is not None
            raw = self.tmp('am_raw', (rows, Hd)) if two else st['am']
            F.gemm(t, Wm1, raw, rows, Nv, cin, dt, lda=C, batch=mg * mg, strideA=cin, a_batch_mod=mg,
                   strideB=Nv * pad8(cin), ldb=pad8(cin), ldc=Hd, strideC=Nv, bias=bm1, strideBias=Nv, act=ops.ACT_RELU,
                   label=pre + 'fc1')
            if two:
                F.relu_drop(raw, drop_mask, st['am'], st['gm'], rows * Hd, dt, label=pre + 'relu')
        Wm2 = self._w_plain(pre + 'fc2.weight', cin, gc_, 1, 1, groups=mg, rs=gamma, src=self._pw(pre + 'fc2.weight'))
        bm2 = self.buf('w.' + pre + 'bm2', (C,), torch.float32)
        self.prep.bias_fold(None, self._pw(pre + 'fc2.bias'), gamma, None, bm2, C, gc_)
        F.gemm(st['am'], Wm2, out, rows, cin, gc_, dt, lda=Hd, batch=mg, strideA=gc_, strideB=cin * pad8(gc_),
               ldb=pad8(gc_), ldc=C, strideC=cin, bias=bm2, strideBias=cin, rowscale=rowscale,
               rows_per_scale=rps, R=R, ldr=C, strideR=cin, label=pre + 'fc2')
        return st

    def _gmlp_bwd(self, pre, st, dmz, t, rows, C, mg, dtk, gamma_name=None):
        Bk, dt, P, W = self.bwd, self.dt, self.P, self.W
        gamma = self._pw(gamma_name) if gamma_name else None
        if 'pad' in st:
            pd = st.pop('pad')
            cin, cin_p, Cp = pd['cin'], pd['cin_p'], pd['Cp']
            dmzp = self.buf(pre + 'dmz.pad', (rows, Cp), zero=True)
            Bk.pad_copy(dmz, dmzp, rows * mg, cin, cin, cin_p, dt, label=pre + 'dmz.pad')
            dtkp = self.tmp('gmlp.dt.pad', (rows, Cp))
            self._gmlp_bwd(pre, st, dmzp, pd['tp'], rows, Cp, mg, dtkp, gamma_name=gamma_name)
            Bk.pad_copy(dtkp, dtk, rows * mg, cin, cin_p, cin, dt, label=pre + 'dt.unpad')
            st['pad'] = pd
            return
        if st.get('naive'):
            Hd = st['Hd']
            dam, dh = self.tmp('dam', (rows, Hd)), self.tmp('dhm', (rows, Hd))
            Bk.small_linear_bwd(st['d2b'], dmz, dA=dam, dW=self.grad(pre + 'fc2.weight'), dbias=self.grad(pre + 'fc2.bias'),
                                dcol_scale=self.grad(gamma_name) if gamma_name else None, label=pre + 'fc2.bwd')
            Bk.gelu_bwd(dam, st['hpre'], dh, rows * Hd, dt, label=pre + 'geluB')
            Bk.small_linear_bwd(st['d1'], dh, dA=dtk, dW=self.grad(pre + 'fc1.weight'), dbias=self.grad(pre + 'fc1.bias'),
                                label=pre + 'fc1.bwd')
            return
        Hd, gc_, Nv, cin = st['Hd'], st['gc'], st['Nv'], st['cin']
        Gm2, gbm2 = self.gbuf((C, gc_)), self.gbuf((C,))
# ... 501 lines not shown
```

### imagenet-models_amd/ops.py

```python
import ctypes as C
import os

import torch

from . import _lib as L
from ._lib import (A_CONV3, A_CONV3S2, A_NEIGH2, A_PATCH2, A_PLAIN, A_STEM4_NCHW, ACT_GELU, ACT_NONE, ACT_RELU, C_PLAIN, C_UNPATCH2,
                   GA_BF16, GA_F32)


def ga_dtype(t):
    if isinstance(t, torch.dtype):
        dt = t
    else:
        dt = t.dtype
    if dt == torch.bfloat16:
        return GA_BF16
    if dt == torch.float32:
        return GA_F32
    raise TypeError(f'unsupported dtype {dt}')


def torch_dtype(ga):
    return torch.bfloat16 if ga == GA_BF16 else torch.float32

# ... 85 lines not shown

    def _small(self, **kw):
        d = L.SmallDesc()
        for k, v in kw.items():
            setattr(d, k, v)
        self._pend['small'].append(d)
        if os.environ.get('GAEXT_SMALL_SINGLE'):
            self.flush(f'single.k{d.kind}.R{d.R}.C{d.C}.n{d.n}.')

    def _add(self, fname, args, label=None, keep=()):
        fn = getattr(self.lib, fname)
        self.calls.append((fn, args, label or fname))
        self.lanes.append(self.lane)
        self.keep.extend(keep)
        if self.eager:
            L.check(fn(*args, current_stream_ptr()), label or fname)

    def _want_workspace(self, nbytes, patch):
        if self.eager:
            t = torch.empty(nbytes, dtype=torch.uint8, device='cuda')
            self.keep.append(t)
            patch(t.data_ptr(), nbytes)
            return
        self._ws_req.append((self.lane, nbytes, patch))
        self._ws_dirty = True

    def finalize(self):
        if not self._ws_dirty:
            return
        need = {}
        for lane, nbytes, _ in self._ws_req:
            need[lane] = max(need.get(lane, 0), nbytes)
        for lane, nbytes in need.items():
            if lane not in self._ws or self._ws[lane].numel() < nbytes:
                self._ws[lane] = torch.empty(nbytes, dtype=torch.uint8, device='cuda')
        for lane, nbytes, patch in self._ws_req:
            patch(self._ws[lane].data_ptr(), self._ws[lane].numel())
        self._ws_dirty = False

    def run(self, stream=None):
        self.finalize()
        s = current_stream_ptr() if stream is None else stream
        if os.environ.get('GAEXT_SYNC_DEBUG'):
            for fn, args, label in self.calls:
                print(f'[gaext] {self.name}:{label}', flush=True)
                L.check(fn(*args, s), f'{self.name}:{label}')
                torch.cuda.synchronize()
            return
        if any(self.lanes):
            return self._run_lanes(0, len(self.calls))
        for fn, args, label in self.calls:
            rc = fn(*args, s)
            if rc != 0:
                L.check(rc, f'{self.name}:{label}')

    def join_async(self, tag=None):
        self.calls.append((_join_marker, () if tag is None else (tag,), 'join_async'))
        self.lanes.append(0)

    def lane_signal(self, lane):
        ev = torch.cuda.Event()
        self.calls.append((_lsig_marker, (lane, ev), 'lane_signal'))
        self.lanes.append(lane)
        return ev

    def lane_wait(self, lane, ev):
        self.calls.append((_lwait_marker, (lane, ev), 'lane_wait'))
        self.lanes.append(lane)

    def async_mark(self, tag):
        self.calls.append((_amark_marker, (tag,), 'async_mark'))
        self.lanes.append(0)

    def _run_lanes(self, start, end):
        main = torch.cuda.current_stream()
        if self._side is None:
            self._side = max(max(self.lanes), 0)
        streams, done, fork = _side_pool(self._side)
        astream, adone, afork = _async_pool()
        apend = False
        aev = {}
        lsig = set()
        s0 = main.cuda_stream
        used = []

        def ajoin():
            adone.record(astream)
            main.wait_event(adone)

        for i in range(start, end):
            fn, args, label = self.calls[i]
            lane = self.lanes[i]
            if fn is _join_marker:
                if args:
                    ev = aev.get(args[0])
                    if ev is not None:
                        main.wait_event(ev)
                elif apend:
                    ajoin()
                    apend = False
                continue
            if fn is _amark_marker:
                if apend:
                    ev = self._aevents.get(args[0])
                    if ev is None:
                        ev = self._aevents[args[0]] = torch.cuda.Event()
                    ev.record(astream)
                    aev[args[0]] = ev
                continue
            if fn is _lsig_marker:
                if args[0] in used:
                    args[1].record(streams[args[0] - 1])
                    lsig.add(args[1])
                continue
            if fn is _lwait_marker:
                if args[1] in lsig:
                    if not used:
                        fork.record(main)
                    if args[0] not in used:
                        streams[args[0] - 1].wait_event(fork)
                        used.append(args[0])
                    streams[args[0] - 1].wait_event(args[1])
                continue
            if lane == ASYNC_LANE:
                if used:
                    for ln in used:
                        done[ln - 1].record(streams[ln - 1])
                        main.wait_event(done[ln - 1])
                    used = []
                afork.record(main)
                astream.wait_event(afork)
                apend = True
                rc = fn(*args, astream.cuda_stream)
            elif lane == 0:
                if used:
                    for ln in used:
                        done[ln - 1].record(streams[ln - 1])
                        main.wait_event(done[ln - 1])
                    used = []
                rc = fn(*args, s0)
            else:
                if not used:
                    if apend:
                        ajoin()
                        apend = False
                    fork.record(main)
                if lane not in used:
                    streams[lane - 1].wait_event(fork)
                    used.append(lane)
                rc = fn(*args, streams[lane - 1].cuda_stream)
            if rc != 0:
                L.check(rc, f'{self.name}:{label}')
        for ln in used:
            done[ln - 1].record(streams[ln - 1])
            main.wait_event(done[ln - 1])
        if apend:
            ajoin()

    def __len__(self):
        return len(self.calls)

    def mark(self, name):
        self.marks[name] = len(self.calls)

    def run_range(self, start, end, stream=None):
        self.finalize()
        s = current_stream_ptr() if stream is None else stream
        if any(self.lanes[start:end]):
            return self._run_lanes(start, end)
        for fn, args, label in self.calls[start:end]:
            rc = fn(*args, s)
            if rc != 0:
                L.check(rc, f'{self.name}:{label}')

    def gemm(self, A, B, Cout, M, N, K, dtype, lda=None, ldb=None, ldc=None, batch=1, strideA=0, strideB=0, strideC=0,
             a_batch_mod=0, a_kind=A_PLAIN, a_dims=(0, 0, 0), a_act=ACT_NONE, c_kind=C_PLAIN, c_dims=(0, 0, 0),
             c_f32=False, alpha=1.0, bias=None, strideBias=0, act=ACT_NONE, H=None, ldh=0, strideH=0, rowscale=None,
             rows_per_scale=1, R=None, ldr=0, strideR=0, relu_after=False, colsum=None, colsumsq=None, strideCol=0,
             C2=None, c2_mode=0, h_is_deriv=False, label=None):
        d = L.GemmDesc()
        d.M, d.N, d.K, d.batch, d.dtype = M, N, K, batch, dtype
        d.A, d.lda, d.strideA, d.a_batch_mod, d.a_kind = _ptr(A), (K if lda is None else lda), strideA, a_batch_mod, a_kind
        d.a_H, d.a_W, d.a_C = a_dims
        d.a_act = a_act
        d.B, d.ldb, d.strideB = _ptr(B), (K if ldb is None else ldb), strideB
        d.C, d.ldc, d.strideC, d.c_kind = _ptr(Cout), (N if ldc is None else ldc), strideC, c_kind
        d.c_H, d.c_W, d.c_C = c_dims
        d.c_f32 = int(c_f32)
        d.C2, d.c2_mode = _ptr(C2), c2_mode
        d.h_is_deriv = int(h_is_deriv)
        d.alpha = alpha
        d.bias, d.strideBias, d.act = _ptr(bias), strideBias, act
        d.H, d.ldh, d.strideH = _ptr(H), ldh, strideH
        d.rowscale, d.rows_per_scale = _ptr(rowscale), rows_per_scale
        d.R, d.ldr, d.strideR, d.relu_after = _ptr(R), ldr, strideR, int(relu_after)
        d.colsum, d.colsumsq, d.strideCol = _ptr(colsum), _ptr(colsumsq), strideCol
        self._add('ga_gemm', (C.byref(d),), label, keep=(d, A, B, Cout, bias, H, rowscale, R, colsum, colsumsq, C2))

    def attn_desc(self, qkv, out, lse, B, N, H, hd, scale, dtype, ldq=None, ldo=None):
        d = L.AttnDesc()
        d.B, d.N, d.H, d.hd, d.scale, d.dtype = B, N, H, hd, scale, dtype
        d.qkv, d.ldq, d.out, d.ldo, d.lse = _ptr(qkv), (3 * H * hd if ldq is None else ldq), _ptr(out), (H * hd if ldo is None else ldo), _ptr(lse)
        self.keep.extend([d, qkv, out, lse])
        return d

    def attn_fwd(self, d, label=None):
        self._add('ga_attn_fwd', (C.byref(d),), label, keep=(d,))

    def attn_bwd(self, d, dout, dqkv, ws, label=None):
        self._add('ga_attn_bwd', (C.byref(d), _ptr(dout), _ptr(dqkv), _ptr(ws), ws.numel() * ws.element_size()), label,
                  keep=(d, dout, dqkv, ws))

    def patchify(self, x, out, P, dtype, label=None):
        B, CH, H, W = x.shape
        self._add('ga_patchify', (_ptr(x), _ptr(out), B, CH, H, W, P, dtype), label, keep=(x, out))

    def patchify_strided(self, x, out, P, S, dtype, label=None):
        B, CH, H, W = x.shape
        self._add('ga_patchify_strided', (_ptr(x), _ptr(out), B, CH, H, W, P, S, dtype), label, keep=(x, out))

    def pos_add_fwd(self, tok, pos, x0, B, Np, Cdim, dtype, label=None):
        self._add('ga_pos_add_fwd', (_ptr(tok), _ptr(pos), _ptr(x0), B, Np, Cdim, dtype), label, keep=(tok, pos, x0))

    def pos_add_bwd(self, dx0, dpos, B, Np, Cdim, dtype, label=None):
        self._add('ga_pos_add_bwd', (_ptr(dx0), _ptr(dpos), B, Np, Cdim, dtype), label, keep=(dx0, dpos))

    def dwpool_fwd(self, x, w, bias, y, B, H, W_, Cin, mult, dtype, label=None):
        self._add('ga_dwpool_fwd', (_ptr(x), _ptr(w), _ptr(bias), _ptr(y), B, H, W_, Cin, mult, dtype), label, keep=(x, w, bias, y))

    def dwpool_bwd_data(self, dy, w, dx, B, H, W_, Cin, mult, dtype, label=None):
        self._add('ga_dwpool_bwd_data', (_ptr(dy), _ptr(w), _ptr(dx), B, H, W_, Cin, mult, dtype), label, keep=(dy, w, dx))

    def dwpool_bwd_weight(self, dy, x, dw, db, B, H, W_, Cin, mult, dtype, label=None):
        self._add('ga_dwpool_bwd_weight', (_ptr(dy), _ptr(x), _ptr(dw), _ptr(db), B, H, W_, Cin, mult, dtype), label, keep=(dy, x, dw, db))

    def resize_concat_fwd(self, src, dst, B, Hin, Win, Cdim, Hout, Wout, ldd, c_off, dtype, label=None):
        self._add('ga_resize_concat_fwd', (_ptr(src), _ptr(dst), B, Hin, Win, Cdim, Hout, Wout, ldd, c_off, dtype), label, keep=(src, dst))

    def resize_concat_bwd(self, dcat, dsrc, B, Hin, Win, Cdim, Hout, Wout, ldd, c_off, dtype, label=None):
        self._add('ga_resize_concat_bwd', (_ptr(dcat), _ptr(dsrc), B, Hin, Win, Cdim, Hout, Wout, ldd, c_off, dtype), label, keep=(dcat, dsrc))

    def rows_bcast(self, src, dst, B, HW, Cdim, scale, dtype, label=None):
        self._add('ga_rows_bcast', (_ptr(src), _ptr(dst), B, HW, Cdim, scale, dtype), label, keep=(src, dst))

    def token_gap_fwd(self, x, y, B, N, Cdim, dtype, label=None):
        self._add('ga_token_gap_fwd', (_ptr(x), _ptr(y), B, N, Cdim, dtype), label, keep=(x, y))

    def token_gap_bwd(self, dy, dx, B, N, Cdim, dtype, label=None):
        self._add('ga_token_gap_bwd', (_ptr(dy), _ptr(dx), B, N, Cdim, dtype), label, keep=(dy, dx))

    def vit_embed_fwd(self, tok, cls, pos, x0, B, Np, Cdim, dtype, label=None):
        self._add('ga_vit_embed_fwd', (_ptr(tok), _ptr(cls), _ptr(pos), _ptr(x0), B, Np, Cdim, dtype), label, keep=(tok, cls, pos, x0))

    def vit_embed_bwd(self, dx0, dtok, dcls, dpos, B, Np, Cdim, dtype, label=None):
        self._add('ga_vit_embed_bwd', (_ptr(dx0), _ptr(dtok), _ptr(dcls), _ptr(dpos), B, Np, Cdim, dtype), label, keep=(dx0, dtok, dcls, dpos))

    def small_linear_desc(self, A, W, Y, rows, groups, Ng, Kg, dtype, lda, a_gstride, ldy, bias=None, a_perm=None, col_scale=None,
                          rowscale=None, rows_per_scale=1, R=None, ldr=0, Yraw=None):
        d = L.SmallLinearDesc()
        d.rows, d.groups, d.Ng, d.Kg, d.dtype = rows, groups, Ng, Kg, dtype
        d.A, d.lda, d.a_gstride, d.a_perm = _ptr(A), lda, a_gstride, _ptr(a_perm)
        d.W, d.bias, d.col_scale = _ptr(W), _ptr(bias), _ptr(col_scale)
        d.rowscale, d.rows_per_scale, d.R, d.ldr = _ptr(rowscale), rows_per_scale, _ptr(R), ldr
        d.Y, d.ldy, d.Yraw = _ptr(Y), ldy, _ptr(Yraw)
        self.keep.extend([d, A, W, Y, bias, a_perm, col_scale, rowscale, R, Yraw])
        return d

    def small_linear_fwd(self, d, label=None):
        self._add('ga_small_linear_fwd', (C.byref(d),), label, keep=(d,))

    def small_linear_bwd(self, d, dY, dA=None, accumulate_dA=False, dW=None, dbias=None, dcol_scale=None, label=None):
        self._add('ga_small_linear_bwd', (C.byref(d), _ptr(dY), _ptr(dA), int(accumulate_dA), _ptr(dW), _ptr(dbias), _ptr(dcol_scale)),
                  label, keep=(d, dY, dA, dW, dbias, dcol_scale))

    def colstats(self, x, ld, rows, Cdim, s, q, dtype, label=None):
        self._add('ga_colstats', (_ptr(x), ld, rows, Cdim, _ptr(s), _ptr(q), dtype), label, keep=(x, s, q))

    def pad_copy_f32(self, src, dst, rows, cols, lds, ldd, accumulate=False, label=None):
        self._add('ga_pad_copy_f32', (_ptr(src), _ptr(dst), rows, cols, lds, ldd, int(accumulate)), label, keep=(src, dst))

    def stem4_ln_fwd(self, x, W, ldw, bias, gamma, beta, pre, y, mean, rstd, B, H, W_, Cdim, eps, label=None):
        self._add('ga_stem4_ln_fwd', (_ptr(x), _ptr(W), ldw, _ptr(bias), _ptr(gamma), _ptr(beta), _ptr(pre), _ptr(y), _ptr(mean), _ptr(rstd),
                                      B, H, W_, Cdim, eps), label, keep=(x, W, bias, gamma, beta, pre, y, mean, rstd))

    def blockdiag_f32(self, src, dst, R, rg, ng, cg, ld, to_diag=True, accumulate=False, label=None):
        self._add('ga_blockdiag_f32', (_ptr(src), _ptr(dst), R, rg, ng, cg, ld, int(to_diag), int(accumulate)), label, keep=(src, dst))

    def pad_groups_f32(self, src, dst, R, Cdim, RG, RGp, CG, CGp, unpad=False, accumulate=False, label=None):
        self._add('ga_pad_groups_f32', (_ptr(src), _ptr(dst), R, Cdim, RG, RGp, CG, CGp, int(unpad), int(accumulate)), label,
                  keep=(src, dst))

    def pad_copy(self, src, dst, rows, cols, lds, ldd, dtype, accumulate=False, label=None):
        self._add('ga_pad_copy', (_ptr(src), _ptr(dst), rows, cols, lds, ldd, int(accumulate), dtype), label, keep=(src, dst))

    def mlp_fwd(self, X, W1, b1, W2, b2, Y, M, Cdim, dtype, ldw1=None, ldw2=None, R=None, rowscale=None, rows_per_scale=1, label=None):
        d = L.MlpDesc()
        H = 4 * Cdim
        d.X, d.ldx, d.W1, d.ldw1, d.b1 = _ptr(X), Cdim, _ptr(W1), (Cdim if ldw1 is None else ldw1), _ptr(b1)
        d.W2, d.ldw2, d.b2 = _ptr(W2), (H if ldw2 is None else ldw2), _ptr(b2)
        d.R, d.ldr, d.rowscale, d.rows_per_scale = _ptr(R), Cdim, _ptr(rowscale), rows_per_scale
        d.Y, d.ldy, d.M, d.C, d.H, d.dtype = _ptr(Y), Cdim, M, Cdim, H, dtype
        self._add('ga_mlp_fwd', (C.byref(d),), label, keep=(d, X, W1, b1, W2, b2, R, rowscale, Y))

    def mlp_bwd(self, X, DY, W1, b1, W2T, W1T, A, DH, DX, M, Cdim, dtype, ldw1=None, ldw2t=None, ldw1t=None, label=None):
        d = L.MlpBwdDesc()
        H = 4 * Cdim
        d.X, d.ldx, d.DY, d.lddy = _ptr(X), Cdim, _ptr(DY), Cdim
        d.W1, d.ldw1, d.b1 = _ptr(W1), (Cdim if ldw1 is None else ldw1), _ptr(b1)
        d.W2T, d.ldw2t, d.W1T, d.ldw1t = _ptr(W2T), (Cdim if ldw2t is None else ldw2t), _ptr(W1T), (H if ldw1t is None else ldw1t)
        d.A, d.lda, d.DH, d.lddh, d.DX, d.lddx = _ptr(A), H, _ptr(DH), H, _ptr(DX), Cdim
        d.M, d.C, d.H, d.dtype = M, Cdim, H, dtype
        self._add('ga_mlp_bwd', (C.byref(d),), label, keep=(d, X, DY, W1, b1, W2T, W1T, A, DH, DX))

    def wgrad(self, Y, X, dW, M, N, K, dtype, ldy=None, ldx=None, ldw=None, batch=1, strideY=0, strideX=0, strideW=0,
              x_kind=A_PLAIN, x_dims=(0, 0, 0), x_act=ACT_NONE, dbias=None, strideDbias=0, alpha=1.0, split_m=None,
              accumulate=True, x_batch_mod=0, label=None):
        d = L.WgradDesc()
        d.M, d.N, d.K, d.batch, d.dtype = M, N, K, batch, dtype
        d.Y, d.ldy, d.strideY = _ptr(Y), (N if ldy is None else ldy), strideY
        d.X, d.ldx, d.strideX, d.x_kind = _ptr(X), (K if ldx is None else ldx), strideX, x_kind
        d.x_batch_mod = x_batch_mod
        d.x_H, d.x_W, d.x_C = x_dims
        d.x_act = x_act
        d.dW, d.ldw, d.strideW = _ptr(dW), (K if ldw is None else ldw), strideW
        d.dbias, d.strideDbias = _ptr(dbias), strideDbias
        d.alpha = alpha
        if split_m is None:
            split_m = pick_split_m(M, N, K, batch, dtype)
        d.split_m, d.accumulate = split_m, int(accumulate)
        need = self.lib.ga_wgrad_workspace(C.byref(d))
        if need:
            def patch(ptr, nbytes, d=d):
                d.workspace, d.ws_bytes = ptr, nbytes
            self._want_workspace(int(need), patch)
        self._add('ga_wgrad', (C.byref(d),), label, keep=(d, Y, X, dW, dbias))

    def weight_prep(self, w, G, Co, Ci, KH, KW, dtype, out=None, ldo=0, outT=None, ldt=0, rs=None, cs=None, flip=False,
                    stem=False, row_perm=None, t_cols=0, label=None):
        d = L.WprepDesc()
        d.w, d.G, d.Co, d.Ci, d.KH, d.KW = _ptr(w), G, Co, Ci, KH, KW
        d.rs, d.cs, d.row_perm, d.dtype = _ptr(rs), _ptr(cs), _ptr(row_perm), dtype
        d.out, d.ldo, d.outT, d.ldt, d.flip, d.stem = _ptr(out), ldo, _ptr(outT), ldt, int(flip), int(stem)
        d.t_cols = t_cols
        if self.defer:
            self._pend['wprep'].append(d)
            self.keep.extend((w, out, outT, rs, cs, row_perm))
            return
        self._add('ga_weight_prep', (C.byref(d),), label, keep=(d, w, out, outT, rs, cs, row_perm))

    def bias_fold(self, W, b, rs, v, be, N, Cdim, row_perm=None, label=None):
        if self.defer:
            self._small(kind=2, y=_ptr(be), x=_ptr(W), R=N, C=Cdim, b=_ptr(b), rs=_ptr(rs), v=_ptr(v), row_perm=_ptr(row_perm))
            self.keep.extend((W, b, rs, v, be, row_perm))
            return
        self._add('ga_bias_fold', (_ptr(W), _ptr(b), _ptr(rs), _ptr(v), _ptr(row_perm), _ptr(be), N, Cdim), label,
                  keep=(W, b, rs, v, be, row_perm))

    def weight_unfold(self, G, ldg, N, Ci, KH=1, KW=1, gb=None, W=None, b=None, rs=None, cs=None, v=None, stem=False, dW=None,
                      db=None, d_rs=None, d_cs=None, d_v=None, row_perm=None, label=None):
        d = L.WunfoldDesc()
        d.G, d.ldg, d.gb, d.W, d.b, d.rs, d.cs, d.v = _ptr(G), ldg, _ptr(gb), _ptr(W), _ptr(b), _ptr(rs), _ptr(cs), _ptr(v)
        d.row_perm = _ptr(row_perm)
        d.N, d.Ci, d.KH, d.KW, d.stem = N, Ci, KH, KW, int(stem)
        d.dW, d.db, d.d_rs, d.d_cs, d.d_v = _ptr(dW), _ptr(db), _ptr(d_rs), _ptr(d_cs), _ptr(d_v)
        if self.defer:
            self._pend['unfold'].append(d)
            self.keep.extend((G, gb, W, b, rs, cs, v, dW, db, d_rs, d_cs, d_v, row_perm))
            return
        self._add('ga_weight_unfold', (C.byref(d),), label, keep=(d, G, gb, W, b, rs, cs, v, dW, db, d_rs, d_cs, d_v, row_perm))

    def dwconv7_fwd(self, x, w49, bias, y, B, H, W, Cdim, dtype, label=None):
        self._add('ga_dwconv7_fwd', (_ptr(x), _ptr(w49), _ptr(bias), _ptr(y), B, H, W, Cdim, dtype), label,
                  keep=(x, w49, bias, y))

    def dwconv7_bwd_data(self, dy, w49, res, dx, B, H, W, Cdim, dtype, dx2=None, scale2=None, label=None):
        if dx2 is not None:
            self._add('ga_dwconv7_bwd_data2', (_ptr(dy), _ptr(w49), _ptr(res), _ptr(dx), _ptr(dx2), _ptr(scale2), B, H, W,
                                               Cdim, dtype), label, keep=(dy, w49, res, dx, dx2, scale2))
            return
        self._add('ga_dwconv7_bwd_data', (_ptr(dy), _ptr(w49), _ptr(res), _ptr(dx), B, H, W, Cdim, dtype), label,
                  keep=(dy, w49, res, dx))

    def dwconv7_bwd_weight(self, dy, x, dw49, dbias, B, H, W, Cdim, dtype, label=None):
        need = int(self.lib.ga_dwconv7_bwd_weight_workspace(B, H, W, Cdim, dtype))
        head = (_ptr(dy), _ptr(x), _ptr(dw49), _ptr(dbias), B, H, W, Cdim, dtype)
        box = {}

        def patch(ptr, nbytes):
            box['ws'] = (ptr, nbytes)
            if 'idx' in box:
                fn, _, lb = self.calls[box['idx']]
                self.calls[box['idx']] = (fn, head + (ptr, nbytes), lb)
        self._want_workspace(need, patch)
        self._add('ga_dwconv7_bwd_weight', head + box.get('ws', (None, 0)), label, keep=(dy, x, dw49, dbias))
        box['idx'] = len(self.calls) - 1

    def dwconv3_fwd(self, x, w9, y, B, H, W, Cdim, stride, dtype, colsum=None, colsumsq=None, label=None):
        self._add('ga_dwconv3_fwd', (_ptr(x), _ptr(w9), _ptr(y), B, H, W, Cdim, stride, _ptr(colsum), _ptr(colsumsq), dtype), label,
                  keep=(x, w9, y, colsum, colsumsq))

    def dwconv3_bwd_data(self, dy, w9, dx, B, H, W, Cdim, stride, dtype, label=None):
        self._add('ga_dwconv3_bwd_data', (_ptr(dy), _ptr(w9), _ptr(dx), B, H, W, Cdim, stride, dtype), label, keep=(dy, w9, dx))

    def dwconv3_bwd_weight(self, dy, x, dw9, B, H, W, Cdim, stride, dtype, label=None):
        need = int(self.lib.ga_dwconv3_bwd_weight_workspace(B, H, W, Cdim, stride, dtype))
        head = (_ptr(dy), _ptr(x), _ptr(dw9), B, H, W, Cdim, stride, dtype)
        box = {}

        def patch(ptr, nbytes):
            box['ws'] = (ptr, nbytes)
            if 'idx' in box:
                fn, _, lb = self.calls[box['idx']]
                self.calls[box['idx']] = (fn, head + (ptr, nbytes), lb)
        self._want_workspace(need, patch)
        self._add('ga_dwconv3_bwd_weight', head + box.get('ws', (None, 0)), label, keep=(dy, x, dw9))
        box['idx'] = len(self.calls) - 1

    def maxpool3s2_fwd(self, x, y, idx, B, H, W, Cdim, dtype, label=None):
        self._add('ga_maxpool3s2_fwd', (_ptr(x), _ptr(y), _ptr(idx), B, H, W, Cdim, dtype), label, keep=(x, y, idx))

    def maxpool3s2_bwd(self, dy, idx, dx, B, H, W, Cdim, dtype, accumulate=False, label=None):
        self._add('ga_maxpool3s2_bwd', (_ptr(dy), _ptr(idx), _ptr(dx), B, H, W, Cdim, int(accumulate), dtype), label, keep=(dy, idx, dx))

    def bn_gelu_fwd(self, x, scale, shift, y, rows, Cdim, dtype, label=None):
        self._add('ga_bn_gelu_fwd', (_ptr(x), _ptr(scale), _ptr(shift), _ptr(y), rows, Cdim, dtype), label, keep=(x, scale, shift, y))

    def bn_gelu_bwd_reduce(self, dy, x, scale, shift, mean, rstd, s1, s2, rows, Cdim, dtype, label=None):
        need = int(self.lib.ga_bn_gelu_bwd_workspace(rows, Cdim))
        head = (_ptr(dy), _ptr(x), _ptr(scale), _ptr(shift), _ptr(mean), _ptr(rstd), _ptr(s1), _ptr(s2), rows, Cdim, dtype)
        box = {}

        def patch(ptr, nbytes):
            box['ws'] = (ptr, nbytes)
            if 'idx' in box:
                fn, _, lb = self.calls[box['idx']]
                self.calls[box['idx']] = (fn, head + (ptr, nbytes), lb)
        self._want_workspace(need, patch)
        self._add('ga_bn_gelu_bwd_reduce', head + box.get('ws', (None, 0)), label, keep=(dy, x, scale, shift, mean, rstd, s1, s2))
        box['idx'] = len(self.calls) - 1

    def bn_gelu_bwd_apply(self, dy, x, scale, shift, mean, rstd, w, s1, s2, n, dx, rows, Cdim, dtype, label=None):
        self._add('ga_bn_gelu_bwd_apply', (_ptr(dy), _ptr(x), _ptr(scale), _ptr(shift), _ptr(mean), _ptr(rstd), _ptr(w), _ptr(s1), _ptr(s2), n,
                                           _ptr(dx), rows, Cdim, dtype), label, keep=(dy, x, scale, shift, mean, rstd, w, s1, s2, dx))

    def se_bn_fwd(self, S, HW, scale3, shift3, W1, g1, b1, rmean, rvar, W2, b2, hpre, mean, rstd, h, gate, B, Cdim, R, training, label=None):
        args = (S, scale3, shift3, W1, g1, b1, rmean, rvar, W2, b2, hpre, mean, rstd, h, gate)
        self._add('ga_se_bn_fwd', (_ptr(S), HW) + tuple(_ptr(t) for t in args[1:]) + (B, Cdim, R, int(training)), label, keep=args)

    def se_bn_bwd(self, P1, P2, rowscale, g3, b3, mean3, rstd3, S, HW, scale3, shift3, W1, g1, b1, W2, hpre, mean, rstd, h, gate, dz, dhpre,
                  ds, s1, s2, dW1, dg1, db1, dW2, db2, B, Cdim, R, label=None):
        pre = (P1, P2, rowscale, g3, b3, mean3, rstd3, S)
        post = (scale3, shift3, W1, g1, b1, W2, hpre, mean, rstd, h, gate, dz, dhpre, ds, s1, s2, dW1, dg1, db1, dW2, db2)
        self._add('ga_se_bn_bwd', tuple(_ptr(t) for t in pre) + (HW,) + tuple(_ptr(t) for t in post) + (B, Cdim, R), label, keep=pre + post)

    def se_residual_fwd(self, x3, scale3, shift3, gate, rowscale, res, rscale, rshift, y, B, HW, Cdim, dtype, label=None):
        args = (x3, scale3, shift3, gate, rowscale, res, rscale, rshift, y)
        self._add('ga_se_residual_fwd', tuple(_ptr(t) for t in args) + (B, HW, Cdim, dtype), label, keep=args)

    def se_residual_bwd_a(self, dy, y, x3, mean3, rstd3, dm, P1, P2, B, HW, Cdim, dtype, label=None):
        args = (dy, y, x3, mean3, rstd3, dm, P1, P2)
        self._add('ga_se_residual_bwd_a', tuple(_ptr(t) for t in args) + (B, HW, Cdim, dtype), label, keep=args)

    def se_residual_bwd_b(self, dm, x3, mean3, rstd3, g3, gate, rowscale, ds, s1, s2, dx3, B, HW, Cdim, dtype, label=None):
        args = (dm, x3, mean3, rstd3, g3, gate, rowscale, ds, s1, s2, dx3)
        self._add('ga_se_residual_bwd_b', tuple(_ptr(t) for t in args) + (B, HW, Cdim, dtype), label, keep=args)

    def subsample2_fwd(self, x, y, B, H, W, Cdim, dtype, label=None):
        self._add('ga_subsample2_fwd', (_ptr(x), _ptr(y), B, H, W, Cdim, dtype), label, keep=(x, y))

    def subsample2_bwd(self, dy, dx, B, H, W, Cdim, dtype, accumulate=False, label=None):
        self._add('ga_subsample2_bwd', (_ptr(dy), _ptr(dx), B, H, W, Cdim, int(accumulate), dtype), label, keep=(dy, dx))

    def layernorm_fwd(self, x, w, b, y, mean, rstd, rows, Cdim, eps, dtype, label=None):
        self._add('ga_layernorm_fwd', (_ptr(x), _ptr(w), _ptr(b), _ptr(y), _ptr(mean), _ptr(rstd), rows, Cdim, eps, dtype),
                  label, keep=(x, w, b, y, mean, rstd))

    def layernorm_bwd(self, g, x, mean, rstd, w, dres, dx, dw, db, rows, Cdim, x_is_normalized, dtype, label=None, dx2=None,
                      scale2=None, rows_per_scale=1):
        if dx2 is not None:
            self._add('ga_layernorm_bwd_dp', (_ptr(g), _ptr(x), _ptr(mean), _ptr(rstd), _ptr(w), _ptr(dres), _ptr(dx), _ptr(dw), _ptr(db),
                                              rows, Cdim, int(x_is_normalized), _ptr(dx2), _ptr(scale2), rows_per_scale, dtype), label,
                      keep=(g, x, mean, rstd, w, dres, dx, dw, db, dx2, scale2))
            return
        self._add('ga_layernorm_bwd', (_ptr(g), _ptr(x), _ptr(mean), _ptr(rstd), _ptr(w), _ptr(dres), _ptr(dx), _ptr(dw),
                                       _ptr(db), rows, Cdim, int(x_is_normalized), dtype), label,
                  keep=(g, x, mean, rstd, w, dres, dx, dw, db))

    def bn_finalize(self, ssum, ssq, n, w, b, eps, momentum, rmean, rvar, mean_out, rstd_out, scale, shift, Cdim,
                    training, label=None):
        self._add('ga_bn_finalize', (_ptr(ssum), _ptr(ssq), n, _ptr(w), _ptr(b), eps, momentum, _ptr(rmean), _ptr(rvar),
                                     _ptr(mean_out), _ptr(rstd_out), _ptr(scale), _ptr(shift), Cdim, int(training)),
                  label, keep=(ssum, ssq, w, b, rmean, rvar, mean_out, rstd_out, scale, shift))

    def affine_act(self, x, scale, shift, res, y, rows, Cdim, relu, dtype, rowscale=None, rows_per_scale=1, ldx=0, label=None):
        self._add('ga_affine_act', (_ptr(x), _ptr(scale), _ptr(shift), _ptr(res), _ptr(rowscale), rows_per_scale, _ptr(y),
                                    rows, Cdim, int(relu), dtype, ldx), label, keep=(x, scale, shift, res, y, rowscale))

    def bn_bwd_reduce(self, dy, y_relu, x, mean, rstd, s1, s2, rows, Cdim, dtype, rowscale=None, rows_per_scale=1, ldx=0,
                      label=None):
        self._add('ga_bn_bwd_reduce', (_ptr(dy), _ptr(y_relu), _ptr(x), _ptr(mean), _ptr(rstd), _ptr(rowscale),
                                       rows_per_scale, _ptr(s1), _ptr(s2), rows, Cdim, dtype, ldx), label,
                  keep=(dy, y_relu, x, mean, rstd, s1, s2, rowscale))

    def bn_bwd_apply(self, dy, y_relu, x, mean, rstd, w, s1, s2, n, dx, rows, Cdim, dtype, rowscale=None,
                     rows_per_scale=1, ldx=0, lddx=0, label=None):
        self._add('ga_bn_bwd_apply', (_ptr(dy), _ptr(y_relu), _ptr(x), _ptr(mean), _ptr(rstd), _ptr(w), _ptr(s1), _ptr(s2),
                                      _ptr(rowscale), rows_per_scale, n, _ptr(dx), rows, Cdim, dtype, ldx, lddx), label,
                  keep=(dy, y_relu, x, mean, rstd, w, s1, s2, dx, rowscale))

    def pool_concat_fwd(self, src, dst, B, Hin, Win, Cdim, Hout, Wout, ldd, c_off, mode, dtype, label=None):
        self._add('ga_pool_concat_fwd', (_ptr(src), _ptr(dst), B, Hin, Win, Cdim, Hout, Wout, ldd, c_off, mode, dtype),
                  label, keep=(src, dst))

    def pool_concat_bwd(self, dcat, dres, dsrc, B, Hin, Win, Cdim, Hout, Wout, ldd, c_off, mode, dtype, label=None):
        self._add('ga_pool_concat_bwd', (_ptr(dcat), _ptr(dres), _ptr(dsrc), B, Hin, Win, Cdim, Hout, Wout, ldd, c_off,
                                         mode, dtype), label, keep=(dcat, dres, dsrc))

    def spatial_sum(self, a, b2, out, B, HW, Cdim, scale, dtype, label=None):
        self._add('ga_spatial_sum', (_ptr(a), _ptr(b2), _ptr(out), B, HW, Cdim, scale, dtype), label, keep=(a, b2, out))

    def se_mlp_fwd(self, s, W1, b1, W2, b2, hid, gate, B, Cdim, R, label=None):
        self._add('ga_se_mlp_fwd', (_ptr(s), _ptr(W1), _ptr(b1), _ptr(W2), _ptr(b2), _ptr(hid), _ptr(gate), B, Cdim, R),
                  label, keep=(s, W1, b1, W2, b2, hid, gate))

    def se_mlp_bwd(self, dgate, gate, hid, s, W1, W2, ds, dW1, db1, dW2, db2, B, Cdim, R, ds_scale=1.0, label=None):
        self._add('ga_se_mlp_bwd', (_ptr(dgate), _ptr(gate), _ptr(hid), _ptr(s), _ptr(W1), _ptr(W2), _ptr(ds), ds_scale, _ptr(dW1),
                                    _ptr(db1), _ptr(dW2), _ptr(db2), B, Cdim, R), label,
                  keep=(dgate, gate, hid, s, W1, W2, ds, dW1, db1, dW2, db2))

    def chan_scale(self, x, g, add, y, B, HW, Cdim, dtype, label=None):
        self._add('ga_chan_scale', (_ptr(x), _ptr(g), _ptr(add), _ptr(y), B, HW, Cdim, dtype), label, keep=(x, g, add, y))

    def gram_pack_fwd(self, G, out, inv_norm, B, Cdim, groups, Kp, dtype, label=None):
        self._add('ga_gram_pack_fwd', (_ptr(G), _ptr(out), _ptr(inv_norm), B, Cdim, groups, Kp, dtype), label,
                  keep=(G, out, inv_norm))

    def gram_pack_bwd(self, dvec, vhat, inv_norm, S, B, Cdim, groups, Kp, dtype, label=None):
        self._add('ga_gram_pack_bwd', (_ptr(dvec), _ptr(vhat), _ptr(inv_norm), _ptr(S), B, Cdim, groups, Kp, dtype), label,
                  keep=(dvec, vhat, inv_norm, S))

    @staticmethod
    def _nbytes(t):
        return 0 if t is None else t.numel() * t.element_size()

    def gram_f64_fwd(self, x, vec, inv_norm, G64, B, HW, Cdim, H, groups, Kp, dtype, label=None):
        self._add('ga_gram_f64_fwd', (_ptr(x), _ptr(vec), _ptr(inv_norm), _ptr(G64), self._nbytes(G64), B, HW, Cdim, H, groups, Kp,
                                      dtype), label, keep=(x, vec, inv_norm, G64))

    def gram_f64_bwd(self, dvec, x, G64, inv_norm, dx, ws, B, HW, Cdim, H, groups, Kp, dtype, label=None):
        self._add('ga_gram_f64_bwd', (_ptr(dvec), _ptr(x), _ptr(G64), _ptr(inv_norm), _ptr(dx), _ptr(ws), self._nbytes(ws), B, HW,
                                      Cdim, H, groups, Kp, dtype), label, keep=(dvec, x, G64, inv_norm, dx, ws))

    def token_cat(self, cls, tok, u, B, N, Cdim, dtype, label=None):
        self._add('ga_token_cat', (_ptr(cls), _ptr(tok), _ptr(u), B, N, Cdim, dtype), label, keep=(cls, tok, u))

    def token_split(self, du, dcls, dtok, B, N, Cdim, acc_cls, acc_tok, dtype, label=None):
        self._add('ga_token_split', (_ptr(du), _ptr(dcls), _ptr(dtok), B, N, Cdim, int(acc_cls), int(acc_tok), dtype),
                  label, keep=(du, dcls, dtok))

    def class_attn_fwd(self, q, kv, out, P, B, N, heads, hd, scale, dtype, label=None):
        self._add('ga_class_attn_fwd', (_ptr(q), _ptr(kv), _ptr(out), _ptr(P), B, N, heads, hd, scale, dtype), label,
                  keep=(q, kv, out, P))

    def class_attn_bwd(self, dout, q, kv, P, dq, dkv, B, N, heads, hd, scale, dtype, label=None):
        self._add('ga_class_attn_bwd', (_ptr(dout), _ptr(q), _ptr(kv), _ptr(P), _ptr(dq), _ptr(dkv), B, N, heads, hd,
                                        scale, dtype), label, keep=(dout, q, kv, P, dq, dkv))

    def class_attn_fwd2(self, q, kv_cls, kv_tok, out, P, B, N, heads, hd, scale, dtype, tok_ld=0, label=None):
        self._add('ga_class_attn_fwd2', (_ptr(q), _ptr(kv_cls), _ptr(kv_tok), tok_ld, _ptr(out), _ptr(P), B, N, heads, hd, scale,
                                         dtype),
                  label, keep=(q, kv_cls, kv_tok, out, P))

    def class_attn_bwd2(self, dout, q, kv_cls, kv_tok, P, dq, dkv_cls, dkv_tok, B, N, heads, hd, scale, dtype, tok_ld=0,
                        label=None):
        self._add('ga_class_attn_bwd2', (_ptr(dout), _ptr(q), _ptr(kv_cls), _ptr(kv_tok), tok_ld, _ptr(P), _ptr(dq), _ptr(dkv_cls),
                                         _ptr(dkv_tok), B, N, heads, hd, scale, dtype), label,
                  keep=(dout, q, kv_cls, kv_tok, P, dq, dkv_cls, dkv_tok))

    def cswin_desc(self, qkv, out, B, reso, Cdim, heads, stripes, lepe, scale, dtype, ldq=None, ldo=None):
        d = L.CswinAttnDesc()
        d.B, d.reso, d.C, d.heads, d.nbranch = B, reso, Cdim, heads, len(stripes)
        for i, ((hs, ws), (w, b)) in enumerate(zip(stripes, lepe)):
            d.Hs[i], d.Ws[i] = hs, ws
            d.lepe_w[i], d.lepe_b[i] = _ptr(w), _ptr(b)
        d.scale, d.dtype = scale, dtype
        d.qkv, d.ldq = _ptr(qkv), (3 * Cdim if ldq is None else ldq)
        d.out, d.ldo = _ptr(out), (Cdim if ldo is None else ldo)
        self.keep.extend([d, qkv, out] + [t for pair in lepe for t in pair])
        return d

    def cswin_attn_fwd(self, d, label=None):
        self._add('ga_cswin_attn_fwd', (C.byref(d),), label, keep=(d,))

    def cswin_attn_bwd(self, d, dout, dqkv, lepe_ws=None, label=None):
        nbytes = 0 if lepe_ws is None else lepe_ws.numel() * lepe_ws.element_size()
        self._add('ga_cswin_attn_bwd', (C.byref(d), _ptr(dout), _ptr(dqkv), _ptr(lepe_ws), nbytes), label, keep=(d, dout, dqkv, lepe_ws))

    def cswin_lepe_wgrad_reduce(self, d, lepe_ws, grads, label=None):
        g = list(grads) + [(None, None)] * (2 - len(grads))
        self._add('ga_cswin_lepe_wgrad_reduce', (C.byref(d), _ptr(lepe_ws), _ptr(g[0][0]), _ptr(g[0][1]), _ptr(g[1][0]), _ptr(g[1][1])),
                  label, keep=(d, lepe_ws) + tuple(t for pair in grads for t in pair))

    def cswin_lepe_wgrad(self, d, dout, grads, label=None):
        g = list(grads) + [(None, None)] * (2 - len(grads))
        self._add('ga_cswin_lepe_wgrad', (C.byref(d), _ptr(dout), _ptr(g[0][0]), _ptr(g[0][1]), _ptr(g[1][0]), _ptr(g[1][1])),
                  label, keep=(d, dout) + tuple(t for pair in grads for t in pair))

    def layernorm_gelu_fwd(self, x, w, b, y, mean, rstd, rows, Cdim, eps, dtype, label=None):
        self._add('ga_layernorm_gelu_fwd', (_ptr(x), _ptr(w), _ptr(b), _ptr(y), _ptr(mean), _ptr(rstd), rows, Cdim, eps, dtype),
                  label, keep=(x, w, b, y, mean, rstd))

    def layernorm_gelu_bwd(self, g, x, mean, rstd, w, b, dx, dw, db, rows, Cdim, dtype, label=None):
        self._add('ga_layernorm_gelu_bwd', (_ptr(g), _ptr(x), _ptr(mean), _ptr(rstd), _ptr(w), _ptr(b), _ptr(dx), _ptr(dw),
                                            _ptr(db), rows, Cdim, dtype), label, keep=(g, x, mean, rstd, w, b, dx, dw, db))

    def nchw3_to_nhwc8(self, x, y, B, H, W, dtype, label=None):
        self._add('ga_nchw3_to_nhwc8', (_ptr(x), _ptr(y), B, H, W, dtype), label, keep=(x, y))

    def convw_pack(self, w, out, Co, Ci, taps, Cp, ldo, dtype, label=None):
        self._add('ga_convw_pack', (_ptr(w), _ptr(out), Co, Ci, taps, Cp, ldo, dtype), label, keep=(w, out))

    def convw_unpack_grad(self, G, dW, Co, Ci, taps, Cp, ldg, label=None):
        self._add('ga_convw_unpack_grad', (_ptr(G), _ptr(dW), Co, Ci, taps, Cp, ldg), label, keep=(G, dW))

    def conv3s2_dgrad_prep(self, w, out, Co, Ci, ldo, dtype, label=None):
        self._add('ga_conv3s2_dgrad_prep', (_ptr(w), _ptr(out), Co, Ci, ldo, dtype), label, keep=(w, out))

    def gram_pack_fwd2(self, G, out, inv_norm, B, Cdim, groups, Kp, ntok, dtype, label=None):
        self._add('ga_gram_pack_fwd2', (_ptr(G), _ptr(out), _ptr(inv_norm), B, Cdim, groups, Kp, ntok, dtype), label,
                  keep=(G, out, inv_norm))

    def gram_pack_bwd2(self, dvec, vhat, inv_norm, S, B, Cdim, groups, Kp, ntok, dtype, label=None):
        self._add('ga_gram_pack_bwd2', (_ptr(dvec), _ptr(vhat), _ptr(inv_norm), _ptr(S), B, Cdim, groups, Kp, ntok, dtype), label,
                  keep=(dvec, vhat, inv_norm, S))

    def map_tokens_fwd(self, e, tok, B, Cdim, T, add_mean, dtype, label=None):
        self._add('ga_map_tokens_fwd', (_ptr(e), _ptr(tok), B, Cdim, T, int(add_mean), dtype), label, keep=(e, tok))

    def map_tokens_bwd(self, dtok, de, B, Cdim, T, add_mean, dtype, label=None):
        self._add('ga_map_tokens_bwd', (_ptr(dtok), _ptr(de), B, Cdim, T, int(add_mean), dtype), label, keep=(dtok, de))

    def class_attn_mt_fwd(self, q, kv_cls, kv_tok, tok_ld, out, P, mask, B, T, N, heads, hd, scale, dtype, label=None):
        self._add('ga_class_attn_mt_fwd', (_ptr(q), _ptr(kv_cls), _ptr(kv_tok), tok_ld, _ptr(out), _ptr(P), _ptr(mask), B, T, N, heads,
                                           hd, scale, dtype), label, keep=(q, kv_cls, kv_tok, out, P, mask))

    def class_attn_mt_bwd(self, dout, q, kv_cls, kv_tok, tok_ld, P, mask, dq, dkv_cls, dkv_tok, dtok_ld, B, T, N, heads, hd, scale,
                          dtype, label=None):
        self._add('ga_class_attn_mt_bwd', (_ptr(dout), _ptr(q), _ptr(kv_cls), _ptr(kv_tok), tok_ld, _ptr(P), _ptr(mask), _ptr(dq),
                                           _ptr(dkv_cls), _ptr(dkv_tok), dtok_ld, B, T, N, heads, hd, scale, dtype), label,
                  keep=(dout, q, kv_cls, kv_tok, P, mask, dq, dkv_cls, dkv_tok))

    def class_attn_mt_ia_fwd(self, q, kv_cls, kv_tok, tok_ld, out, P, mask, W1, b1, W2, b2, B, T, N, heads, hd, scale, dtype, label=None):
        self._add('ga_class_attn_mt_ia_fwd', (_ptr(q), _ptr(kv_cls), _ptr(kv_tok), tok_ld, _ptr(out), _ptr(P), _ptr(mask), _ptr(W1), _ptr(b1),
                                              _ptr(W2), _ptr(b2), B, T, N, heads, hd, scale, dtype), label,
                  keep=(q, kv_cls, kv_tok, out, P, mask, W1, b1, W2, b2))

    def class_attn_mt_ia_bwd(self, dout, q, kv_cls, kv_tok, tok_ld, P, mask, W1, W2, b2, dq, dkv_cls, dkv_tok, dtok_ld, dW1, db1, dW2, db2,
                             B, T, N, heads, hd, scale, dtype, label=None):
        self._add('ga_class_attn_mt_ia_bwd', (_ptr(dout), _ptr(q), _ptr(kv_cls), _ptr(kv_tok), tok_ld, _ptr(P), _ptr(mask), _ptr(W1), _ptr(W2),
                                              _ptr(b2), _ptr(dq), _ptr(dkv_cls), _ptr(dkv_tok), dtok_ld, _ptr(dW1), _ptr(db1), _ptr(dW2),
                                              _ptr(db2), B, T, N, heads, hd, scale, dtype), label,
                  keep=(dout, q, kv_cls, kv_tok, P, mask, W1, W2, b2, dq, dkv_cls, dkv_tok, dW1, db1, dW2, db2))

    def map_loss_fwd_bwd(self, org, avg, target, loss, dorg, davg, K, B, NC, lam, kind, smoothing, grad_scale, dtype, label=None):
        self._add('ga_map_loss_fwd_bwd', (_ptr(org), _ptr(avg), _ptr(target), _ptr(loss), _ptr(dorg), _ptr(davg), K, B, NC, lam, kind,
                                          smoothing, grad_scale, dtype), label, keep=(org, avg, target, loss, dorg, davg))

    def loss_dense_fwd_bwd(self, org, avg, target, dense, loss, dorg, davg, K, B, NC, lam, kind, smoothing, bce_threshold, grad_scale,
                           dtype, label=None):
        self._add('ga_loss_dense_fwd_bwd', (_ptr(org), _ptr(avg), _ptr(target), _ptr(dense), _ptr(loss), _ptr(dorg), _ptr(davg), K, B, NC,
                                            lam, kind, smoothing, bce_threshold, grad_scale, dtype), label,
                  keep=(org, avg, target, dense, loss, dorg, davg))

    def u8_normalize(self, x, out, mean, std, label=None):
        B, CH, H, W = x.shape
        m = (C.c_float * CH)(*[float(v) for v in mean])
        s = (C.c_float * CH)(*[float(v) for v in std])
        self._add('ga_u8_normalize', (_ptr(x), _ptr(out), B, CH, H, W, m, s), label, keep=(x, out, m, s))

    def input_erase(self, x, out, boxes, max_count, mode, seed, offset, mean=None, std=None, label=None):
        B, CH, H, W = x.shape
        u8 = x.dtype == torch.uint8
        m = (C.c_float * CH)(*[float(v) for v in mean]) if u8 else None
        s = (C.c_float * CH)(*[float(v) for v in std]) if u8 else None
        mask = (1 << 64) - 1
        self._add('ga_input_erase', (_ptr(x), int(u8), _ptr(out), B, CH, H, W, m, s, _ptr(boxes), int(max_count), int(mode),
                                     int(seed) & mask, int(offset) & mask), label, keep=(x, out, boxes, m, s))

    def mixup_batch(self, x, out, lam, cutmix=False, box=(0, 0, 0, 0), label=None):
        B, CH, H, W = x.shape
        yl, yh, xl, xh = (int(v) for v in box)
        self._add('ga_mixup_batch', (_ptr(x), _ptr(out), B, CH, H, W, float(lam), int(cutmix), yl, yh, xl, xh), label, keep=(x, out))

    def mixup_target(self, target, out, NC, lam, smoothing, label=None):
        self._add('ga_mixup_target', (_ptr(target), _ptr(out), target.numel(), NC, float(lam), float(smoothing)), label, keep=(target, out))

    def agc_clip(self, params, grads, units, nunits, clip_factor, eps=1e-3, label=None):
        self._add('ga_agc_clip', (_ptr(params), _ptr(grads), _ptr(units), nunits, float(clip_factor), float(eps)), label,
                  keep=(params, grads, units))

    def gelu_fwd(self, x, y, n, dtype, label=None):
        self._add('ga_gelu_fwd', (_ptr(x), _ptr(y), n, dtype), label, keep=(x, y))

    def gelu_bwd(self, dy, x, dx, n, dtype, label=None):
        self._add('ga_gelu_bwd', (_ptr(dy), _ptr(x), _ptr(dx), n, dtype), label, keep=(dy, x, dx))

    def relu_drop(self, a, mask, out, deriv, n, dtype, label=None):
        self._add('ga_relu_drop', (_ptr(a), _ptr(mask), _ptr(out), _ptr(deriv), n, dtype), label, keep=(a, mask, out, deriv))

    def mask_mul(self, x, mask, res, y, n, dtype, label=None):
        self._add('ga_mask_mul', (_ptr(x), _ptr(mask), _ptr(res), _ptr(y), n, dtype), label, keep=(x, mask, res, y))

    def copy2d(self, src, lds, dst, ldd, rows, cols, dtype, accumulate=False, label=None):
        self._add('ga_copy2d', (_ptr(src), lds, _ptr(dst), ldd, rows, cols, int(accumulate), dtype), label, keep=(src, dst))

    def loss_fwd_bwd(self, logits, target, loss, dlogits, K, B, NC, lam, kind, smoothing, grad_scale, dtype, label=None):
        self._add('ga_loss_fwd_bwd', (_ptr(logits), _ptr(target), _ptr(loss), _ptr(dlogits), K, B, NC, lam, kind,
                                      smoothing, grad_scale, dtype), label, keep=(logits, target, loss, dlogits))

    def heads_topk(self, logits, K, B, NC, topk, out_sum, out_idx, label=None):
        self._add('ga_heads_topk', (_ptr(logits), K, B, NC, topk, _ptr(out_sum), _ptr(out_idx)), label,
                  keep=(logits, out_sum, out_idx))

    def sgd_step(self, p, g, buf, hp, n, nesterov, wd_mult, label=None):
        self._add('ga_sgd_step', (_ptr(p), _ptr(g), _ptr(buf), _ptr(hp), n, int(nesterov), wd_mult), label,
                  keep=(p, g, buf, hp))

    def adamw_step(self, p, g, m, v, hp, n, wd_mult, label=None):
        self._add('ga_adamw_step', (_ptr(p), _ptr(g), _ptr(m), _ptr(v), _ptr(hp), n, wd_mult), label,
                  keep=(p, g, m, v, hp))

    def drop_path_sample(self, out, keep, sites, B, seed, counter, label=None):
        self._add('ga_drop_path_sample', (_ptr(out), _ptr(keep), sites, B, int(seed) & ((1 << 64) - 1), _ptr(counter)), label,
                  keep=(out, keep, counter))

    def dropout_mask_sample(self, out, n, keep, seed, counter, label=None):
        self._add('ga_dropout_mask_sample', (_ptr(out), n, float(keep), int(seed) & ((1 << 64) - 1), _ptr(counter)), label,
                  keep=(out, counter))

    def transpose_f32(self, src, dst, R, Cdim, accumulate=False, label=None):
        if self.defer:
            self._small(kind=1, y=_ptr(dst), x=_ptr(src), R=R, C=Cdim, accumulate=int(accumulate))
            self.keep.extend((src, dst))
            return
        self._add('ga_transpose_f32', (_ptr(src), _ptr(dst), R, Cdim, int(accumulate)), label, keep=(src, dst))

    def axpy_f32(self, y, x, a, n, label=None):
        if self.defer:
            self._small(kind=0, y=_ptr(y), x=_ptr(x), a=a, n=n)
            self.keep.extend((y, x))
            return
        self._add('ga_axpy_f32', (_ptr(y), _ptr(x), a, n), label, keep=(y, x))

    def lamb_stage1(self, p, g, m, v, u, hp, gsumsq, chunks, nchunks, norms, label=None):
        self._add('ga_lamb_stage1', (_ptr(p), _ptr(g), _ptr(m), _ptr(v), _ptr(u), _ptr(hp), _ptr(gsumsq), _ptr(chunks), nchunks,
                                     _ptr(norms)), label, keep=(p, g, m, v, u, hp, gsumsq, chunks, norms))

    def lamb_stage2(self, p, u, hp, chunks, nchunks, norms, label=None):
        self._add('ga_lamb_stage2', (_ptr(p), _ptr(u), _ptr(hp), _ptr(chunks), nchunks, _ptr(norms)), label,
                  keep=(p, u, hp, chunks, norms))

    def lerp_f32(self, y, x, w, n, label=None):
        self._add('ga_lerp_f32', (_ptr(y), _ptr(x), float(w), n), label, keep=(y, x))

    def sumsq_f32(self, x, n, out, label=None):
        self._add('ga_sumsq_f32', (_ptr(x), n, _ptr(out)), label, keep=(x, out))

    def clip_grad_f32(self, g, n, sumsq, limit, mode, label=None):
        self._add('ga_clip_grad_f32', (_ptr(g), n, _ptr(sumsq), float(limit), int(mode)), label, keep=(g, sumsq))

    def rowscale(self, x, s, y, n, elems_per_scale, dtype, label=None):
        self._add('ga_rowscale', (_ptr(x), _ptr(s), _ptr(y), n, elems_per_scale, dtype), label, keep=(x, s, y))

    def cast_from_f32(self, src, dst, n, dtype, label=None):
        self._add('ga_cast_from_f32', (_ptr(src), _ptr(dst), n, dtype), label, keep=(src, dst))

    def cast_to_f32(self, src, dst, n, dtype, label=None):
        self._add('ga_cast_to_f32', (_ptr(src), _ptr(dst), n, dtype), label, keep=(src, dst))

    def zero(self, t, label=None):
        self._add('ga_memset', (_ptr(t), 0, t.numel() * t.element_size()), label or 'zero', keep=(t,))


def mlp_supported(Cdim, H, dtype):
    return bool(L.load().ga_mlp_supported(Cdim, H, dtype))


def cswin_attn_bwd_workspace(d):
    return int(L.load().ga_cswin_attn_bwd_workspace(C.byref(d)))


def zero_(t):
    L.check(L.load().ga_memset(_ptr(t), 0, t.numel() * t.element_size(), current_stream_ptr()), 'ga_memset')
    return t


_NUM_CU = None


def num_cus():
    global _NUM_CU
    if _NUM_CU is None:
        n = C.c_int(256)
        L.check(L.load().ga_device_info(C.byref(n), None, None), 'ga_device_info')
        _NUM_CU = n.value
    return _NUM_CU


def pick_split_m(M, N, K, batch, dtype):
    slab = 64 if dtype == GA_BF16 else 32
    tiles = ((N + 127) // 128) * ((K + 127) // 128) * batch
    want = max(1, (2 * 256) // tiles)
    return int(max(1, min(want, (M + 4 * slab - 1) // (4 * slab))))
```

### include/gaext.h

```cpp
#ifndef GAEXT_H
#define GAEXT_H
#include <stddef.h>
#include <stdint.h>

#ifdef __cplusplus
extern "C" {
#endif

typedef void* ga_stream_t;

enum { GA_F32 = 0, GA_BF16 = 1 };
enum { GA_OK = 0, GA_ERR_BAD_ARG = -1, GA_ERR_UNSUPPORTED = -2, GA_ERR_HIP = -3 };

enum { GA_ACT_NONE = 0, GA_ACT_GELU = 1, GA_ACT_RELU = 2 };

enum {
    GA_A_PLAIN = 0,
    GA_A_PATCH2 = 1,
    GA_A_STEM4_NCHW = 2,
    GA_A_CONV3 = 3,
    GA_A_CONV3S2 = 4,
    GA_A_NEIGH2 = 5
};
enum {
// ... 20 lines not shown
    int a_H, a_W, a_C;
    int a_act;
    const void* B;
    int64_t ldb, strideB;
    void* C;
    int64_t ldc, strideC;
    int c_kind;
    int c_H, c_W, c_C;
    int c_f32;
    void* C2;
    int c2_mode;
    float alpha;
    const float* bias;
    int64_t strideBias;
    int act;
    const void* H;
    int64_t ldh, strideH;
    int h_is_deriv;
    const float* rowscale;
    int rows_per_scale;
    const void* R;
    int64_t ldr, strideR;
    int relu_after;
    float* colsum;
    float* colsumsq;
    int64_t strideCol;
} ga_gemm_desc;
int ga_gemm(const ga_gemm_desc* d, ga_stream_t stream);

typedef struct {
    int M, N, K;
    int batch;
    int dtype;
    const void* Y;
    int64_t ldy, strideY;
    const void* X;
    int64_t ldx, strideX;
    int x_batch_mod;
    int x_kind;
    int x_H, x_W, x_C;
    int x_act;
    float* dW;
    int64_t ldw, strideW;
    float* dbias;
    int64_t strideDbias;
    float alpha;
    int split_m;
    int accumulate;
    void* workspace;
    int64_t ws_bytes;
} ga_wgrad_desc;
int ga_wgrad(const ga_wgrad_desc* d, ga_stream_t stream);
size_t ga_wgrad_workspace(const ga_wgrad_desc* d);

typedef struct {
    const float* w;
    int G, Co, Ci, KH, KW;
    const float* rs;
    const float* cs;
    const int* row_perm;
    int dtype;
    void* out;  int64_t ldo;
    void* outT; int64_t ldt;
    int flip;
    int stem;
    int t_cols;
} ga_wprep_desc;
int ga_weight_prep(const ga_wprep_desc* d, ga_stream_t stream);
int ga_bias_fold(const float* W, const float* b, const float* rs, const float* v, const int* row_perm, float* be, int N,
                 int C, ga_stream_t stream);
typedef struct {
    const float* G; int64_t ldg;
    const float* gb;
    const float* W; const float* b;
    const float* rs; const float* cs; const float* v;
    const int* row_perm;
    int N, Ci, KH, KW;
    int stem;
    float* dW; float* db; float* d_rs; float* d_cs; float* d_v;
} ga_wunfold_desc;
int ga_weight_unfold(const ga_wunfold_desc* d, ga_stream_t stream);

int ga_dwconv7_fwd(const void* x, const float* w49, const float* bias, void* y, int B, int H, int W, int C,
                   int dtype, ga_stream_t stream);
int ga_dwconv7_bwd_data(const void* dy, const float* w49, const void* res, void* dx, int B, int H, int W, int C,
                        int dtype, ga_stream_t stream);
int ga_dwconv7_bwd_data2(const void* dy, const float* w49, const void* res, void* dx, void* dx2, const float* scale2,
                         int B, int H, int W, int C, int dtype, ga_stream_t stream);
size_t ga_dwconv7_bwd_weight_workspace(int B, int H, int W, int C, int dtype);
int ga_dwconv7_bwd_weight(const void* dy, const void* x, float* dw49, float* dbias, int B, int H, int W, int C,
                          int dtype, void* workspace, size_t ws_bytes, ga_stream_t stream);

int ga_dwconv3_fwd(const void* x, const float* w9, void* y, int B, int H, int W, int C, int stride, float* colsum,
                   float* colsumsq, int dtype, ga_stream_t stream);
int ga_dwconv3_bwd_data(const void* dy, const float* w9, void* dx, int B, int H, int W, int C, int stride, int dtype,
                        ga_stream_t stream);
size_t ga_dwconv3_bwd_weight_workspace(int B, int H, int W, int C, int stride, int dtype);
int ga_dwconv3_bwd_weight(const void* dy, const void* x, float* dw9, int B, int H, int W, int C, int stride, int dtype,
                          void* workspace, size_t ws_bytes, ga_stream_t stream);

int ga_maxpool3s2_fwd(const void* x, void* y, unsigned char* idx, int B, int H, int W, int C, int dtype, ga_stream_t stream);
int ga_maxpool3s2_bwd(const void* dy, const unsigned char* idx, void* dx, int B, int H, int W, int C, int accumulate, int dtype,
                      ga_stream_t stream);
int ga_bn_gelu_fwd(const void* x, const float* scale, const float* shift, void* y, int64_t rows, int C, int dtype, ga_stream_t stream);
size_t ga_bn_gelu_bwd_workspace(int64_t rows, int C);
int ga_bn_gelu_bwd_reduce(const void* dy, const void* x, const float* scale, const float* shift, const float* mean, const float* rstd,
                          float* s1, float* s2, int64_t rows, int C, int dtype, void* workspace, size_t ws_bytes, ga_stream_t stream);
int ga_bn_gelu_bwd_apply(const void* dy, const void* x, const float* scale, const float* shift, const float* mean, const float* rstd,
                         const float* w, const float* s1, const float* s2, int64_t n, void* dx, int64_t rows, int C, int dtype,
                         ga_stream_t stream);
int ga_se_bn_fwd(const float* S, int HW, const float* scale3, const float* shift3, const float* W1, const float* g1, const float* b1,
                 float* rmean, float* rvar, const float* W2, const float* b2, float* hpre, float* mean, float* rstd, float* h, float* gate,
                 int B, int C, int R, int training, ga_stream_t stream);
int ga_se_bn_bwd(const float* P1, const float* P2, const float* rowscale, const float* g3, const float* b3, const float* mean3,
                 const float* rstd3, const float* S, int HW, const float* scale3, const float* shift3, const float* W1, const float* g1,
                 const float* b1, const float* W2, const float* hpre, const float* mean, const float* rstd, const float* h,
                 const float* gate, float* dz, float* dhpre, float* ds, float* s1, float* s2, float* dW1, float* dg1, float* db1,
                 float* dW2, float* db2, int B, int C, int R, ga_stream_t stream);
int ga_se_residual_fwd(const void* x3, const float* scale3, const float* shift3, const float* gate, const float* rowscale, const void* res,
                       const float* rscale, const float* rshift, void* y, int B, int HW, int C, int dtype, ga_stream_t stream);
int ga_se_residual_bwd_a(const void* dy, const void* y, const void* x3, const float* mean3, const float* rstd3, void* dm, float* P1,
                         float* P2, int B, int HW, int C, int dtype, ga_stream_t stream);
int ga_se_residual_bwd_b(const void* dm, const void* x3, const float* mean3, const float* rstd3, const float* g3, const float* gate,
                         const float* rowscale, const float* ds, const float* s1, const float* s2, void* dx3, int B, int HW, int C,
                         int dtype, ga_stream_t stream);
int ga_subsample2_fwd(const void* x, void* y, int B, int H, int W, int C, int dtype, ga_stream_t stream);
int ga_subsample2_bwd(const void* dy, void* dx, int B, int H, int W, int C, int accumulate, int dtype, ga_stream_t stream);

int ga_layernorm_fwd(const void* x, const float* w, const float* b, void* y, float* mean, float* rstd, int64_t rows,
                     int C, float eps, int dtype, ga_stream_t stream);
int ga_layernorm_bwd(const void* g, const void* x, const float* mean, const float* rstd, const float* w,
                     const void* dres, void* dx, float* dw, float* db, int64_t rows, int C, int x_is_normalized,
                     int dtype, ga_stream_t stream);
int ga_layernorm_bwd_dp(const void* g, const void* x, const float* mean, const float* rstd, const float* w, const void* dres,
                        void* dx, float* dw, float* db, int64_t rows, int C, int x_is_normalized, void* dx2, const float* scale2,
                        int64_t rows_per_scale, int dtype, ga_stream_t stream);

int ga_bn_finalize(const float* sum, const float* sumsq, int64_t n, const float* w, const float* b, float eps,
                   float momentum, float* running_mean, float* running_var, float* mean_out, float* rstd_out,
                   float* scale, float* shift, int C, int training, ga_stream_t stream);
int ga_affine_act(const void* x, const float* scale, const float* shift, const void* res, const float* rowscale,
                  int64_t rows_per_scale, void* y, int64_t rows, int C, int relu, int dtype, int64_t ldx, ga_stream_t stream);
int ga_bn_bwd_reduce(const void* dy, const void* y_relu, const void* x, const float* mean, const float* rstd,
                     const float* rowscale, int64_t rows_per_scale, float* s1, float* s2, int64_t rows, int C, int dtype,
                     int64_t ldx, ga_stream_t stream);
int ga_bn_bwd_apply(const void* dy, const void* y_relu, const void* x, const float* mean, const float* rstd,
                    const float* w, const float* s1, const float* s2, const float* rowscale, int64_t rows_per_scale,
                    int64_t n, void* dx, int64_t rows, int C, int dtype, int64_t ldx, int64_t lddx, ga_stream_t stream);

int ga_pool_concat_fwd(const void* src, void* dst, int B, int Hin, int Win, int C, int Hout, int Wout, int ldd,
                       int c_off, int mode, int dtype, ga_stream_t stream);
int ga_pool_concat_bwd(const void* dcat, const void* dres, void* dsrc, int B, int Hin, int Win, int C, int Hout,
                       int Wout, int ldd, int c_off, int mode, int dtype, ga_stream_t stream);

int ga_spatial_sum(const void* a, const void* b2, float* out, int B, int HW, int C, float scale, int dtype,
                   ga_stream_t stream);
int ga_se_mlp_fwd(const float* s, const float* W1, const float* b1, const float* W2, const float* b2, float* hid,
                  float* gate, int B, int C, int R, ga_stream_t stream);
int ga_se_mlp_bwd(const float* dgate, const float* gate, const float* hid, const float* s, const float* W1,
                  const float* W2, float* ds, float ds_scale, float* dW1, float* db1, float* dW2, float* db2, int B,
                  int C, int R, ga_stream_t stream);
int ga_chan_scale(const void* x, const float* g, const float* add, void* y, int B, int HW, int C, int dtype,
                  ga_stream_t stream);

int ga_gram_pack_fwd(const float* G, void* out, float* inv_norm, int B, int C, int groups, int Kp, int dtype,
                     ga_stream_t stream);
int ga_gram_pack_bwd(const void* dvec, const void* vhat, const float* inv_norm, void* S, int B, int C, int groups,
                     int Kp, int dtype, ga_stream_t stream);

size_t ga_gram_f64_fwd_workspace(int B, int C);
size_t ga_gram_f64_bwd_workspace(int B, int C);
int ga_gram_f64_fwd(const void* x, void* vec, double* inv_norm, double* G64, size_t g64_bytes, int B, int HW, int C, int H,
                    int groups, int Kp, int dtype, ga_stream_t stream);
int ga_gram_f64_bwd(const void* dvec, const void* x, const double* G64, const double* inv_norm, void* dx, void* workspace,
                    size_t ws_bytes, int B, int HW, int C, int H, int groups, int Kp, int dtype, ga_stream_t stream);

int ga_token_cat(const void* cls, const void* tok, void* u, int B, int N, int C, int dtype, ga_stream_t stream);
int ga_token_split(const void* du, void* dcls, void* dtok, int B, int N, int C, int acc_cls, int acc_tok, int dtype,
                   ga_stream_t stream);
int ga_class_attn_fwd(const void* q, const void* kv, void* out, float* P, int B, int N, int heads, int hd, float scale,
                      int dtype, ga_stream_t stream);
int ga_class_attn_bwd(const void* dout, const void* q, const void* kv, const float* P, void* dq, void* dkv, int B, int N,
                      int heads, int hd, float scale, int dtype, ga_stream_t stream);
int ga_class_attn_fwd2(const void* q, const void* kv_cls, const void* kv_tok, int64_t tok_ld, void* out, float* P, int B, int N,
                       int heads, int hd, float scale, int dtype, ga_stream_t stream);
int ga_class_attn_bwd2(const void* dout, const void* q, const void* kv_cls, const void* kv_tok, int64_t tok_ld, const float* P,
                       void* dq, void* dkv_cls, void* dkv_tok, int B, int N, int heads, int hd, float scale, int dtype,
                       ga_stream_t stream);

int ga_loss_fwd_bwd(const float* logits, const int64_t* target, float* loss, void* dlogits, int K, int B, int NC,
                    float lam, int kind, float smoothing, float grad_scale, int dtype, ga_stream_t stream);
int ga_heads_topk(const float* logits, int K, int B, int NC, int topk, float* out_sum, int64_t* out_idx,
                  ga_stream_t stream);

int ga_sgd_step(float* p, const float* g, float* buf, const float* hp, int64_t n, int nesterov, float wd_mult,
                ga_stream_t stream);
int ga_adamw_step(float* p, const float* g, float* m, float* v, const float* hp, int64_t n, float wd_mult,
                  ga_stream_t stream);

typedef struct {
    int kind;
    float* y; const float* x; float a; int64_t n;
    int R, C, accumulate;
    const float* b; const float* rs; const float* v; const int* row_perm;
} ga_small_desc;
int ga_weight_prep_batch(const ga_wprep_desc* jobs_dev, int n, ga_stream_t stream);
int ga_weight_unfold_batch(const ga_wunfold_desc* jobs_dev, int n, ga_stream_t stream);
int ga_small_batch(const ga_small_desc* jobs_dev, int n, ga_stream_t stream);

int ga_lamb_stage1(const float* p, const float* g, float* m, float* v, float* u, const float* hp, const float* gsumsq,
                   const int* chunks, int nchunks, float* norms, ga_stream_t stream);
int ga_lamb_stage2(float* p, const float* u, const float* hp, const int* chunks, int nchunks, const float* norms,
                   ga_stream_t stream);

int ga_sumsq_f32(const float* x, int64_t n, float* out, ga_stream_t stream);
int ga_clip_grad_f32(float* g, int64_t n, const float* sumsq, float limit, int mode, ga_stream_t stream);

typedef struct {
    int B, reso, C, heads, nbranch;
    int Hs[2], Ws[2];
    const float* lepe_w[2];
    const float* lepe_b[2];
    float scale;
    int dtype;
    const void* qkv; int64_t ldq;
    void* out; int64_t ldo;
} ga_cswin_attn_desc;
int ga_cswin_attn_fwd(const ga_cswin_attn_desc* d, ga_stream_t stream);
size_t ga_cswin_attn_bwd_workspace(const ga_cswin_attn_desc* d);
int ga_cswin_attn_bwd(const ga_cswin_attn_desc* d, const void* dout, void* dqkv, void* lepe_ws, size_t ws_bytes, ga_stream_t stream);
int ga_cswin_lepe_wgrad_reduce(const ga_cswin_attn_desc* d, const void* lepe_ws, float* dw0, float* db0, float* dw1, float* db1,
                               ga_stream_t stream);
int ga_cswin_lepe_wgrad(const ga_cswin_attn_desc* d, const void* dout, float* dw0, float* db0, float* dw1, float* db1,
                        ga_stream_t stream);
int ga_layernorm_gelu_fwd(const void* x, const float* w, const float* b, void* y, float* mean, float* rstd, int64_t rows,
                          int C, float eps, int dtype, ga_stream_t stream);
int ga_layernorm_gelu_bwd(const void* g, const void* x, const float* mean, const float* rstd, const float* w, const float* b,
                          void* dx, float* dw, float* db, int64_t rows, int C, int dtype, ga_stream_t stream);
int ga_nchw3_to_nhwc8(const float* x, void* y, int B, int H, int W, int dtype, ga_stream_t stream);
int ga_convw_pack(const float* w, void* out, int Co, int Ci, int taps, int Cp, int64_t ldo, int dtype, ga_stream_t stream);
int ga_convw_unpack_grad(const float* G, float* dW, int Co, int Ci, int taps, int Cp, int64_t ldg, ga_stream_t stream);
int ga_conv3s2_dgrad_prep(const float* w, void* out, int Co, int Ci, int64_t ldo, int dtype, ga_stream_t stream);

int ga_gram_pack_fwd2(const float* G, void* out, float* inv_norm, int B, int C, int groups, int Kp, int ntok, int dtype,
                      ga_stream_t stream);
int ga_gram_pack_bwd2(const void* dvec, const void* vhat, const float* inv_norm, void* S, int B, int C, int groups, int Kp,
                      int ntok, int dtype, ga_stream_t stream);
int ga_map_tokens_fwd(const void* e, void* tok, int B, int C, int T, int add_mean, int dtype, ga_stream_t stream);
int ga_map_tokens_bwd(const void* dtok, void* de, int B, int C, int T, int add_mean, int dtype, ga_stream_t stream);
int ga_class_attn_mt_fwd(const void* q, const void* kv_cls, const void* kv_tok, int64_t tok_ld, void* out, float* P,
                         const float* mask, int B, int T, int N, int heads, int hd, float scale, int dtype, ga_stream_t stream);
int ga_class_attn_mt_bwd(const void* dout, const void* q, const void* kv_cls, const void* kv_tok, int64_t tok_ld, const float* P,
                         const float* mask, void* dq, void* dkv_cls, void* dkv_tok, int64_t dtok_ld, int B, int T, int N,
                         int heads, int hd, float scale, int dtype, ga_stream_t stream);
int ga_class_attn_mt_ia_fwd(const void* q, const void* kv_cls, const void* kv_tok, int64_t tok_ld, void* out, float* P,
                            const float* mask, const float* W1, const float* b1, const float* W2, const float* b2, int B, int T, int N,
                            int heads, int hd, float scale, int dtype, ga_stream_t stream);
int ga_class_attn_mt_ia_bwd(const void* dout, const void* q, const void* kv_cls, const void* kv_tok, int64_t tok_ld, const float* P,
                            const float* mask, const float* W1, const float* W2, const float* b2, void* dq, void* dkv_cls,
                            void* dkv_tok, int64_t dtok_ld, float* dW1, float* db1, float* dW2, float* db2, int B, int T, int N,
                            int heads, int hd, float scale, int dtype, ga_stream_t stream);
int ga_map_loss_fwd_bwd(const float* org, const float* avg, const int64_t* target, float* loss, void* dorg, void* davg, int K,
                        int B, int NC, float lam, int kind, float smoothing, float grad_scale, int dtype, ga_stream_t stream);
int ga_loss_dense_fwd_bwd(const float* org, const float* avg, const int64_t* target, const float* dense, float* loss, void* dorg,
                          void* davg, int K, int B, int NC, float lam, int kind, float smoothing, float bce_threshold,
                          float grad_scale, int dtype, ga_stream_t stream);
int ga_mixup_batch(const float* x, float* out, int B, int CH, int H, int W, double lam, int cutmix, int yl, int yh, int xl, int xh,
                   ga_stream_t stream);
int ga_mixup_target(const int64_t* target, float* out, int B, int NC, double lam, double smoothing, ga_stream_t stream);
int ga_u8_normalize(const void* x, float* out, int B, int CH, int H, int W, const float* mean, const float* std, ga_stream_t stream);
int ga_input_erase(const void* x, int x_is_u8, float* out, int B, int CH, int H, int W, const float* mean, const float* std,
                   const int32_t* boxes, int max_count, int mode, uint64_t seed, uint64_t offset, ga_stream_t stream);
int ga_agc_clip(const float* params, float* grads, const int64_t* units, int nunits, float clip_factor, float eps, ga_stream_t stream);
int ga_gelu_fwd(const void* x, void* y, int64_t n, int dtype, ga_stream_t stream);
int ga_gelu_bwd(const void* dy, const void* x, void* dx, int64_t n, int dtype, ga_stream_t stream);
int ga_relu_drop(const void* a, const float* mask, void* out, void* deriv, int64_t n, int dtype, ga_stream_t stream);
int ga_mask_mul(const void* x, const float* mask, const void* res, void* y, int64_t n, int dtype, ga_stream_t stream);
int ga_copy2d(const void* src, int64_t lds, void* dst, int64_t ldd, int64_t rows, int cols, int accumulate, int dtype,
              ga_stream_t stream);

int ga_drop_path_sample(float* out, const float* keep, int sites, int B, uint64_t seed, uint64_t* counter, ga_stream_t stream);

int ga_dropout_mask_sample(float* out, int64_t n, float keep, uint64_t seed, uint64_t* counter, ga_stream_t stream);

typedef struct {
    const void* X; int64_t ldx;
    const void* W1; int64_t ldw1; const float* b1;
    const void* W2; int64_t ldw2; const float* b2;
    const void* R; int64_t ldr;
    const float* rowscale; int rows_per_scale;
    void* Y; int64_t ldy;
    int64_t M; int C, H, dtype;
} ga_mlp_desc;
typedef struct {
    const void* X; int64_t ldx;
    const void* DY; int64_t lddy;
    const void* W1; int64_t ldw1; const float* b1;
    const void* W2T; int64_t ldw2t;
    const void* W1T; int64_t ldw1t;
    void* A; int64_t lda;
    void* DH; int64_t lddh;
    void* DX; int64_t lddx;
    int64_t M; int C, H, dtype;
} ga_mlp_bwd_desc;
int ga_mlp_supported(int C, int H, int dtype);
int ga_mlp_fwd(const ga_mlp_desc* d, ga_stream_t stream);
int ga_mlp_bwd(const ga_mlp_bwd_desc* d, ga_stream_t stream);

typedef struct {
    int rows, groups, Ng, Kg;
    const void* A; int64_t lda; int64_t a_gstride; const int* a_perm;
    const float* W; const float* bias; const float* col_scale;
    const float* rowscale; int rows_per_scale;
    const void* R; int64_t ldr;
    void* Y; int64_t ldy; void* Yraw;
    int dtype;
} ga_small_linear_desc;
int ga_small_linear_fwd(const ga_small_linear_desc* d, ga_stream_t stream);
int ga_small_linear_bwd(const ga_small_linear_desc* d, const void* dY, void* dA, int accumulate_dA, float* dW, float* dbias,
                        float* dcol_scale, ga_stream_t stream);
int ga_colstats(const void* x, int64_t ld, int rows, int C, float* sum, float* sumsq, int dtype, ga_stream_t stream);
int ga_pad_copy_f32(const float* src, float* dst, int64_t rows, int64_t cols, int64_t lds, int64_t ldd, int accumulate, ga_stream_t stream);
int ga_stem4_ln_fwd(const float* x, const void* W, int64_t ldw, const float* bias, const float* gamma, const float* beta, void* pre,
                    void* y, float* mean, float* rstd, int B, int H, int W_, int C, float eps, ga_stream_t stream);
int ga_blockdiag_f32(const float* src, float* dst, int64_t R, int rg, int ng, int cg, int64_t ld, int to_diag, int accumulate,
                     ga_stream_t stream);
int ga_pad_groups_f32(const float* src, float* dst, int64_t R, int64_t C, int RG, int RGp, int CG, int CGp, int unpad, int accumulate,
                      ga_stream_t stream);
int ga_pad_copy(const void* src, void* dst, int64_t rows, int64_t cols, int64_t lds, int64_t ldd, int accumulate, int dtype,
                ga_stream_t stream);

typedef struct {
    int B, N, H, hd;
    float scale;
    int dtype;
    const void* qkv; int64_t ldq;
    void* out; int64_t ldo;
    float* lse;
} ga_attn_desc;
int ga_attn_fwd(const ga_attn_desc* d, ga_stream_t stream);
size_t ga_attn_bwd_workspace(const ga_attn_desc* d);
int ga_attn_bwd(const ga_attn_desc* d, const void* dout, void* dqkv, void* workspace, size_t ws_bytes, ga_stream_t stream);
int ga_patchify(const float* x, void* out, int B, int CH, int H, int W, int P, int dtype, ga_stream_t stream);
int ga_vit_embed_fwd(const void* tok, const float* cls, const float* pos, void* x0, int B, int Np, int C, int dtype, ga_stream_t stream);
int ga_vit_embed_bwd(const void* dx0, void* dtok, float* dcls, float* dpos, int B, int Np, int C, int dtype, ga_stream_t stream);

int ga_patchify_strided(const float* x, void* out, int B, int CH, int H, int W, int P, int S, int dtype, ga_stream_t stream);
int ga_pos_add_fwd(const void* tok, const float* pos, void* x0, int B, int Np, int C, int dtype, ga_stream_t stream);
int ga_pos_add_bwd(const void* dx0, float* dpos, int B, int Np, int C, int dtype, ga_stream_t stream);
int ga_dwpool_fwd(const void* x, const float* w, const float* bias, void* y, int B, int H, int W, int Cin, int mult, int dtype,
                  ga_stream_t stream);
int ga_dwpool_bwd_data(const void* dy, const float* w, void* dx, int B, int H, int W, int Cin, int mult, int dtype, ga_stream_t stream);
int ga_dwpool_bwd_weight(const void* dy, const void* x, float* dw, float* db, int B, int H, int W, int Cin, int mult, int dtype,
                         ga_stream_t stream);
int ga_resize_concat_fwd(const void* src, void* dst, int B, int Hin, int Win, int C, int Hout, int Wout, int64_t ldd, int c_off,
                         int dtype, ga_stream_t stream);
int ga_resize_concat_bwd(const void* dcat, void* dsrc, int B, int Hin, int Win, int C, int Hout, int Wout, int64_t ldd, int c_off,
                         int dtype, ga_stream_t stream);
int ga_rows_bcast(const void* src, void* dst, int B, int HW, int C, float scale, int dtype, ga_stream_t stream);
int ga_token_gap_fwd(const void* x, void* y, int B, int N, int C, int dtype, ga_stream_t stream);
int ga_token_gap_bwd(const void* dy, void* dx, int B, int N, int C, int dtype, ga_stream_t stream);

int ga_memset(void* p, int value, size_t bytes, ga_stream_t stream);
int ga_transpose_f32(const float* in, float* out, int R, int C, int accumulate, ga_stream_t stream);
int ga_axpy_f32(float* y, const float* x, float a, int64_t n, ga_stream_t stream);
int ga_lerp_f32(float* y, const float* x, float w, int64_t n, ga_stream_t stream);
int ga_rowscale(const void* x, const float* s, void* y, int64_t n, int64_t elems_per_scale, int dtype,
                ga_stream_t stream);
int ga_cast_from_f32(const float* src, void* dst, int64_t n, int dtype, ga_stream_t stream);
int ga_cast_to_f32(const void* src, float* dst, int64_t n, int dtype, ga_stream_t stream);

typedef struct ga_comm* ga_comm_t;
int ga_comm_unique_id(void* id128);
int ga_comm_init(ga_comm_t* comm, int rank, int world, const void* id128);
int ga_comm_destroy(ga_comm_t comm);
int ga_comm_info(ga_comm_t comm, int* rank, int* world);
size_t ga_allreduce_workspace(int64_t n, int wire_dtype);
int ga_allreduce_bucket(ga_comm_t comm, float* grads, int64_t n, int wire_dtype, float scale, void* workspace, size_t ws_bytes,
                        ga_stream_t stream);
int ga_reduce_scatter_bucket(ga_comm_t comm, const float* grads, float* shard, int64_t n_per_rank, float scale, ga_stream_t stream);
int ga_allgather_bucket(ga_comm_t comm, const float* shard, float* full, int64_t n_per_rank, ga_stream_t stream);
int ga_comm_broadcast(ga_comm_t comm, void* buf, int64_t n_f32, int root, ga_stream_t stream);

#ifdef __cplusplus
}
#endif
#endif
```

Measured before the change: 10770 images/sec.

## Fuse fc1 weight gradient into MLP backward kernel with per-block partials

For C=96 stages, the MLP backward kernel now computes dW1 and db1 in-kernel. It uses transposed LDS reads and MFMA over the dh and x tiles, loops persistently over row tiles, and writes per-block partials that a small reduce kernel sums. This removes writing the M x 4C dh tensor to memory and the separate wg1 GEMM that re-read it along with xn. The cost is more register and MFMA pressure inside the fused kernel, a smaller persistent grid, and a reduction pass over the partials.

```diff
diff --git a/imagenet-models_amd/_lib.py b/imagenet-models_amd/_lib.py
--- a/imagenet-models_amd/_lib.py
+++ b/imagenet-models_amd/_lib.py
@@ -76,7 +76,8 @@
 class MlpBwdDesc(C.Structure):
     _fields_ = [('X', vp), ('ldx', i64), ('DY', vp), ('lddy', i64), ('W1', vp), ('ldw1', i64), ('b1', vp),
                 ('W2T', vp), ('ldw2t', i64), ('W1T', vp), ('ldw1t', i64), ('A', vp), ('lda', i64), ('DH', vp), ('lddh', i64),
-                ('DX', vp), ('lddx', i64), ('M', i64), ('C', i32), ('H', i32), ('dtype', i32)]
+                ('DX', vp), ('lddx', i64), ('M', i64), ('C', i32), ('H', i32), ('dtype', i32),
+                ('dW1', vp), ('ldw', i64), ('db1', vp), ('partials', vp), ('partials_bytes', C.c_size_t), ('max_blocks', i32)]
 
 
 class SmallLinearDesc(C.Structure):
@@ -229,6 +230,8 @@
     'ga_mlp_supported': ([i32, i32, i32], i32),
     'ga_mlp_fwd': ([C.POINTER(MlpDesc), vp], i32),
     'ga_mlp_bwd': ([C.POINTER(MlpBwdDesc), vp], i32),
+    'ga_mlp_bwd_wgrad_supported': ([i32, i32, i32], i32),
+    'ga_mlp_bwd_partials': ([C.POINTER(MlpBwdDesc)], C.c_size_t),
     'ga_memset': ([vp, i32, C.c_size_t, vp], i32),
     'ga_transpose_f32': ([vp, vp, i32, i32, i32, vp], i32),
     'ga_axpy_f32': ([vp, vp, f32, i64, vp], i32),
@@ -273,7 +276,7 @@
     s = buf.value.decode(errors='replace')
     host = sorted(k for k in os.environ if k.startswith(('GAEXT_', 'GA_FUSED_MLP')) and k != 'GAEXT_LIB')
     known = {'GAEXT_ASYNC_WGRAD', 'GAEXT_FWD_SPLIT', 'GAEXT_PAR_BRANCH', 'GAEXT_FWD_SKEW', 'GAEXT_FUSE_DP', 'GAEXT_HEAD_STREAMS',
-             'GA_FUSED_MLP', 'GAEXT_SMALL_SINGLE', 'GAEXT_SYNC_DEBUG'}
+             'GA_FUSED_MLP', 'GAEXT_SMALL_SINGLE', 'GAEXT_SYNC_DEBUG', 'GAEXT_MLP_WG1'}
     for k in host:
         if k in known:
             s += f' host:{k}={os.environ[k]}'
diff --git a/imagenet-models_amd/csrc/mlp.hip b/imagenet-models_amd/csrc/mlp.hip
--- a/imagenet-models_amd/csrc/mlp.hip
+++ b/imagenet-models_amd/csrc/mlp.hip
@@ -15,20 +15,20 @@
 }
 
 template <int ROWS, int KS, int NTHR>
-__device__ __forceinline__ void stage_rows(unsigned char* dst, const bf16_t* src, long ld, long row0, long limit) {
+__device__ __forceinline__ void stage_rows(unsigned char* dst, const bf16_t* src, long ld, long row0, long limit, int tid) {
     constexpr int CPR = KS * 4, NP = ROWS * CPR / NTHR;
     static_assert(ROWS * CPR % NTHR == 0, "tile must split evenly over the threads");
     u32x4_t v[NP];
 #pragma unroll
     for (int i = 0; i < NP; ++i) {
-        const int idx = threadIdx.x + NTHR * i;
+        const int idx = tid + NTHR * i;
         const int r = idx / CPR, c = idx - r * CPR;
         v[i] = u32x4_t{0, 0, 0, 0};
         if (row0 + r < limit) v[i] = __builtin_nontemporal_load(reinterpret_cast<const u32x4_t*>(src + (row0 + r) * ld + c * 8));
     }
 #pragma unroll
     for (int i = 0; i < NP; ++i) {
-        const int idx = threadIdx.x + NTHR * i;
+        const int idx = tid + NTHR * i;
         const int r = idx / CPR, c = idx - r * CPR;
         *reinterpret_cast<u32x4_t*>(dst + (c >> 2) * ROWS * 64 + slab_off(r, c & 3)) = v[i];
     }
@@ -56,10 +56,10 @@
 template <int C, int NTHR, int NWM, int TM>
 __device__ __forceinline__ void store_rows(float* Cs, const f32x4_t (&acc)[C / 32][TM], int wm, int wn, int lane, long m0, long M,
                                            const float* bias, const float* rowscale, int rps, bool has_r,
-                                           const PreArr<C, NTHR>& pre, bf16_t* Y, long ldy) {
+                                           const PreArr<C, NTHR>& pre, bf16_t* Y, long ldy, int tid) {
     constexpr int LDC = C + 4, P8 = C / 8, RG = NTHR / P8, WROWS = 16 * TM, WPH = 64 / WROWS;
     constexpr int NR = (64 + RG - 1) / RG;
-    const int c8 = threadIdx.x % P8, rg = threadIdx.x / P8;
+    const int c8 = tid % P8, rg = tid / P8;
     float bv[8];
 #pragma unroll
     for (int j = 0; j < 8; ++j) bv[j] = bias ? bias[c8 * 8 + j] : 0.f;
@@ -151,7 +151,7 @@
     };
 
     w_load(0);
-    stage_rows<BM, KS1, 256>(Xs, reinterpret_cast<const bf16_t*>(d.X), d.ldx, m0, d.M);
+    stage_rows<BM, KS1, 256>(Xs, reinterpret_cast<const bf16_t*>(d.X), d.ldx, m0, d.M, tid);
     for (int i = tid; i < 4 * C; i += 256) B1s[i] = d.b1[i];
     w1_store();
     w2_store();
@@ -220,7 +220,7 @@
     if (d.R) rows_prefetch<C, 256>(rpre, reinterpret_cast<const bf16_t*>(d.R), d.ldr, m0, d.M);
     round(d.H - HC, false);
     store_rows<C, 256, 2, 4>(reinterpret_cast<float*>(smem), y, wm, wn, lane, m0, d.M, d.b2, d.rowscale, d.rows_per_scale,
-                             d.R != nullptr, rpre, reinterpret_cast<bf16_t*>(d.Y), d.ldy);
+                             d.R != nullptr, rpre, reinterpret_cast<bf16_t*>(d.Y), d.ldy, tid);
 }
 
 template <int C, int HC> constexpr int fwd_lds() {
@@ -229,11 +229,24 @@
     return ab > st ? ab : st;
 }
 
-template <int C, int HC>
+__device__ __forceinline__ unsigned tr_off(int lane, int hf, int u0) {
+    const int i = lane & 15, row = 8 * (lane >> 4) + 4 * hf + (i >> 2);
+    return slab_off(row, u0 + ((i & 3) >> 1)) + 8 * (i & 1);
+}
+__device__ __forceinline__ bf16x8_t tr_frag(const unsigned char* lo, const unsigned char* hi) {
+    s16x4_t v[2];
+    v[0] = __builtin_amdgcn_ds_read_tr16_b64_v4i16((__attribute__((address_space(3))) s16x4_t*)lo);
+    v[1] = __builtin_amdgcn_ds_read_tr16_b64_v4i16((__attribute__((address_space(3))) s16x4_t*)hi);
+    return *reinterpret_cast<const bf16x8_t*>(&v[0]);
+}
+
+template <int C, int HC, bool WG>
 __global__ __launch_bounds__(512, 1) void mlp_bwd_kernel(const ga_mlp_bwd_desc d) {
     constexpr int KS1 = C / 32, KS2 = HC / 32, TN1 = HC / 32, TN2 = C / 32;
     constexpr int XS = KS1 * BM * 64, WS = KS1 * HC * 64, TS = KS2 * BM * 64;
     constexpr int NPC = HC * C / 8, NI = (NPC + 511) / 512;
+    constexpr int NCH = 4 * C / HC;
+    static_assert(!WG || (HC == 64 && C == 96), "the in-kernel weight gradient is laid out for 4 x 6 tiles over 8 waves");
     extern __shared__ __attribute__((aligned(16))) unsigned char smem[];
     unsigned char* Xs = smem;
     unsigned char* Ds = Xs + XS;
@@ -244,7 +257,6 @@
     unsigned char* A2s = DHs + TS;
     float* B1s = reinterpret_cast<float*>(A2s + TS);
     const int tid = threadIdx.x, lane = tid & 63, wave = tid >> 6, wm = wave >> 1, wn = wave & 1, g = lane >> 4;
-    const long m0 = (long)blockIdx.x * BM;
     const bf16_t* W1 = reinterpret_cast<const bf16_t*>(d.W1);
     const bf16_t* W2T = reinterpret_cast<const bf16_t*>(d.W2T);
     const bf16_t* W1T = reinterpret_cast<const bf16_t*>(d.W1T);
@@ -282,111 +294,224 @@
         }
     };
 
+    constexpr int NDW = WG ? NCH : 1;
+    f32x4_t dw[NDW][3];
+    float bsum[NDW];
+    unsigned tra[2];
+    if constexpr (WG) {
+#pragma unroll
+        for (int i = 0; i < NDW; ++i) {
+            bsum[i] = 0.f;
+#pragma unroll
+            for (int j = 0; j < 3; ++j) dw[i][j] = f32x4_t{0.f, 0.f, 0.f, 0.f};
+        }
+        tra[0] = tr_off(lane, 0, 0);
+        tra[1] = tr_off(lane, 1, 0);
+    }
+    const int wu = __builtin_amdgcn_readfirstlane(wave);
+    auto tr_blk = [&](const unsigned char* img, int blk, int ks) __attribute__((always_inline)) {
+        const unsigned o = (unsigned)(img - smem) + (blk >> 1) * BM * 64 + ks * 2048, x = (blk & 1) << 5;
+        return tr_frag(smem + ((tra[0] ^ x) + o), smem + ((tra[1] ^ x) + o));
+    };
+
+    for (int i = tid; i < 4 * C; i += 512) B1s[i] = d.b1[i];
+    const long ntiles = (d.M + BM - 1) / BM;
+    long tile = blockIdx.x;
     w_load(0);
-    stage_rows<BM, KS1, 512>(Xs, reinterpret_cast<const bf16_t*>(d.X), d.ldx, m0, d.M);
-    stage_rows<BM, KS1, 512>(Ds, reinterpret_cast<const bf16_t*>(d.DY), d.lddy, m0, d.M);
-    for (int i = tid; i < 4 * C; i += 512) B1s[i] = d.b1[i];
-    w12_store();
-    w3_store();
+    while (true) {
+        const long m0 = tile * BM;
+        const bool first = !WG || tile == (long)blockIdx.x;
+        const bool next_tile = WG && tile + (long)gridDim.x < ntiles;
+        int ttid = tid;
+        if constexpr (WG) asm volatile("" : "+v"(ttid));
+        stage_rows<BM, KS1, 512>(Xs, reinterpret_cast<const bf16_t*>(d.X), d.ldx, m0, d.M, ttid);
+        stage_rows<BM, KS1, 512>(Ds, reinterpret_cast<const bf16_t*>(d.DY), d.lddy, m0, d.M, ttid);
+        if (first) {
+            w12_store();
+            w3_store();
+        }
+        __syncthreads();
+
+        f32x4_t dx[TN2][2];
+#pragma unroll
+        for (int i = 0; i < TN2; ++i)
+#pragma unroll
+            for (int j = 0; j < 2; ++j) dx[i][j] = f32x4_t{0.f, 0.f, 0.f, 0.f};
+
+        auto wg_chunk = [&](f32x4_t (&dwc)[3], float& bs) __attribute__((always_inline)) {
+            typedef __attribute__((ext_vector_type(2))) __bf16 bf16x2_t;
+            const bf16x2_t ones2 = {(__bf16)1.0f, (__bf16)1.0f};
+#pragma unroll
+            for (int ks = 0; ks < BM / 32; ++ks) {
+                const bf16x8_t hf8 = tr_blk(DHs, wu >> 1, ks);
+#pragma unroll
+                for (int tc = 0; tc < 3; ++tc) {
+                    const bf16x8_t xf8 = tr_blk(Xs, 3 * (wu & 1) + tc, ks);
+                    dwc[tc] = __builtin_amdgcn_mfma_f32_16x16x32_bf16(hf8, xf8, dwc[tc], 0, 0, 0);
+                }
+                if ((wu & 1) == 0) {
+#pragma unroll
+                    for (int j = 0; j < 4; ++j)
+                        bs = __builtin_amdgcn_fdot2_f32_bf16(bf16x2_t{hf8[2 * j], hf8[2 * j + 1]}, ones2, bs, false);
+                }
+            }
+        };
+        auto chunk = [&](const int j0, const bool more, const int jn) __attribute__((always_inline)) {
+            if (more) w_load(jn);
+            f32x4_t h[TN1][2], t[TN1][2];
+#pragma unroll
+            for (int i = 0; i < TN1; ++i)
+#pragma unroll
+                for (int j = 0; j < 2; ++j) h[i][j] = t[i][j] = f32x4_t{0.f, 0.f, 0.f, 0.f};
+#pragma unroll
+            for (int ks = 0; ks < KS1; ++ks) {
+                bf16x8_t xf[2], df[2];
+#pragma unroll
+                for (int tm = 0; tm < 2; ++tm) {
+                    xf[tm] = frag(Xs + ks * BM * 64, wm * 32 + 16 * tm, lane);
+                    df[tm] = frag(Ds + ks * BM * 64, wm * 32 + 16 * tm, lane);
+                }
+#pragma unroll
+                for (int tn = 0; tn < TN1; ++tn) {
+                    const bf16x8_t w1f = frag(W1s + ks * HC * 64, wn * (HC / 2) + 16 * tn, lane);
+                    const bf16x8_t w2f = frag(W2Ts + ks * HC * 64, wn * (HC / 2) + 16 * tn, lane);
+#pragma unroll
+                    for (int tm = 0; tm < 2; ++tm) {
+                        h[tn][tm] = __builtin_amdgcn_mfma_f32_16x16x32_bf16(w1f, xf[tm], h[tn][tm], 0, 0, 0);
+                        t[tn][tm] = __builtin_amdgcn_mfma_f32_16x16x32_bf16(w2f, df[tm], t[tn][tm], 0, 0, 0);
+                    }
+                }
+            }
+#pragma unroll
+            for (int tn = 0; tn < TN1; ++tn) {
+                const int nl = wn * (HC / 2) + 16 * tn + 4 * g;
+                const float4 b = *reinterpret_cast<const float4*>(B1s + j0 + nl);
+                const float bb[4] = {b.x, b.y, b.z, b.w};
+#pragma unroll
+                for (int tm = 0; tm < 2; ++tm) {
+                    float a[4], dh[4];
+#pragma unroll
+                    for (int r = 0; r < 4; ++r) {
+                        float gr;
+                        gelu_both_fast(h[tn][tm][r] + bb[r], a[r], gr);
+                        dh[r] = t[tn][tm][r] * gr;
+                    }
+                    const int row = wm * 32 + 16 * tm + (lane & 15);
+                    const unsigned o = (nl >> 5) * BM * 64 + slab_off(row, (nl & 31) >> 3) + (nl & 7) * 2;
+                    uint2 p;
+                    p.x = pack2bf(a[0], a[1]);
+                    p.y = pack2bf(a[2], a[3]);
+                    *reinterpret_cast<uint2*>(A2s + o) = p;
+                    p.x = pack2bf(dh[0], dh[1]);
+                    p.y = pack2bf(dh[2], dh[3]);
+                    *reinterpret_cast<uint2*>(DHs + o) = p;
+                }
+            }
+            lds_barrier();
+#pragma unroll
+            for (int ks = 0; ks < KS2; ++ks) {
+                bf16x8_t af[2];
+#pragma unroll
+                for (int tm = 0; tm < 2; ++tm) af[tm] = frag(DHs + ks * BM * 64, wm * 32 + 16 * tm, lane);
+#pragma unroll
+                for (int tn = 0; tn < TN2; ++tn) {
+                    const bf16x8_t wf = frag(W1Ts + ks * C * 64, wn * (C / 2) + 16 * tn, lane);
+#pragma unroll
+                    for (int tm = 0; tm < 2; ++tm) dx[tn][tm] = __builtin_amdgcn_mfma_f32_16x16x32_bf16(wf, af[tm], dx[tn][tm], 0, 0, 0);
+                }
+            }
+            if constexpr (WG) {
+                static_assert(NDW == 1 || NDW == 6, "one case per chunk");
+                switch (j0 / HC) {
+                    case 0: wg_chunk(dw[0], bsum[0]); break;
+                    case 1: wg_chunk(dw[1 % NDW], bsum[1 % NDW]); break;
+                    case 2: wg_chunk(dw[2 % NDW], bsum[2 % NDW]); break;
+                    case 3: wg_chunk(dw[3 % NDW], bsum[3 % NDW]); break;
+                    case 4: wg_chunk(dw[4 % NDW], bsum[4 % NDW]); break;
+                    default: wg_chunk(dw[5 % NDW], bsum[5 % NDW]); break;
+                }
+            }
+            if (Aout || DHout) {
+                constexpr int PPR = HC / 8, NP = BM * PPR / 512;
+                static_assert(BM * PPR % 512 == 0, "chunk rows must split evenly");
+                int ctid = tid;
+                if constexpr (WG) asm volatile("" : "+v"(ctid));
+#pragma unroll
+                for (int i = 0; i < NP; ++i) {
+                    const int idx = ctid + 512 * i;
+                    const int r = idx / PPR, c = idx - r * PPR;
+                    const long m = m0 + r;
+                    if (m < d.M) {
+                        const unsigned o = (c >> 2) * BM * 64 + slab_off(r, c & 3);
+                        if (Aout) store16_nt(Aout + m * d.lda + j0 + c * 8, *reinterpret_cast<const uint4*>(A2s + o));
+                        if (DHout) store16_nt(DHout + m * d.lddh + j0 + c * 8, *reinterpret_cast<const uint4*>(DHs + o));
+                    }
+                }
+            }
+            if (more) w12_store();
+            lds_barrier();
+            if (more) w3_store();
+        };
+        for (int j0 = 0; j0 < d.H; j0 += HC) {
+            const bool last = j0 + HC >= d.H;
+            chunk(j0, !last || next_tile, last ? 0 : j0 + HC);
+        }
+        u32x4_t nopre[BM / 64][RowPre<C, 512>::NR];
+#pragma unroll
+        for (int i = 0; i < BM / 64; ++i)
+#pragma unroll
+            for (int j = 0; j < RowPre<C, 512>::NR; ++j) nopre[i][j] = u32x4_t{0, 0, 0, 0};
+        int stid = tid;
+        if constexpr (WG) asm volatile("" : "+v"(stid));
+        store_rows<C, 512, 4, 2>(reinterpret_cast<float*>(smem), dx, stid >> 7, (stid >> 6) & 1, stid & 63, m0, d.M, nullptr, nullptr, 1,
+                                 false, nopre, reinterpret_cast<bf16_t*>(d.DX), d.lddx, stid);
+        if (!next_tile) break;
+        tile += gridDim.x;
+        __syncthreads();
+    }
+    if constexpr (WG) {
+        float* P = d.partials + (long)blockIdx.x * (4 * C * C + 4 * C);
+        int etid = tid;
+        asm volatile("" : "+v"(etid));
+        const int lane = etid & 63, g = lane >> 4, jt = wu >> 1;
+#pragma unroll
+        for (int ch = 0; ch < NCH; ++ch) {
+#pragma unroll
+            for (int tc = 0; tc < 3; ++tc)
+#pragma unroll
+                for (int r = 0; r < 4; ++r)
+                    P[(ch * HC + 16 * jt + 4 * g + r) * C + 16 * (3 * (wu & 1) + tc) + (lane & 15)] = dw[ch][tc][r];
+            float v = bsum[ch];
+            v += __shfl_xor(v, 16, 64);
+            v += __shfl_xor(v, 32, 64);
+            if ((wu & 1) == 0 && lane < 16) P[4 * C * C + ch * HC + 16 * jt + lane] = v;
+        }
+    }
+}
+
+__global__ __launch_bounds__(256) void mlp_bwd_wg_reduce_kernel(const float* __restrict__ part, int nparts, int n, int nw, int C,
+                                                                float* __restrict__ dW1, long ldw, float* __restrict__ db1) {
+    __shared__ float4 sh[3][64];
+    const int q = threadIdx.x >> 6;
+    const long i = ((long)blockIdx.x * 64 + (threadIdx.x & 63)) * 4;
+    float4 a = make_float4(0.f, 0.f, 0.f, 0.f);
+    if (i < n) {
+#pragma unroll 4
+        for (int s = q; s < nparts; s += 4) {
+            const float4 b = *reinterpret_cast<const float4*>(part + (long)s * n + i);
+            a.x += b.x; a.y += b.y; a.z += b.z; a.w += b.w;
+        }
+    }
+    if (q) sh[q - 1][threadIdx.x & 63] = a;
     __syncthreads();
-
-    f32x4_t dx[TN2][2];
-#pragma unroll
-    for (int i = 0; i < TN2; ++i)
-#pragma unroll
-        for (int j = 0; j < 2; ++j) dx[i][j] = f32x4_t{0.f, 0.f, 0.f, 0.f};
-
-    for (int j0 = 0; j0 < d.H; j0 += HC) {
-        const bool more = j0 + HC < d.H;
-        if (more) w_load(j0 + HC);
-        f32x4_t h[TN1][2], t[TN1][2];
-#pragma unroll
-        for (int i = 0; i < TN1; ++i)
-#pragma unroll
-            for (int j = 0; j < 2; ++j) h[i][j] = t[i][j] = f32x4_t{0.f, 0.f, 0.f, 0.f};
-#pragma unroll
-        for (int ks = 0; ks < KS1; ++ks) {
-            bf16x8_t xf[2], df[2];
-#pragma unroll
-            for (int tm = 0; tm < 2; ++tm) {
-                xf[tm] = frag(Xs + ks * BM * 64, wm * 32 + 16 * tm, lane);
-                df[tm] = frag(Ds + ks * BM * 64, wm * 32 + 16 * tm, lane);
-            }
-#pragma unroll
-            for (int tn = 0; tn < TN1; ++tn) {
-                const bf16x8_t w1f = frag(W1s + ks * HC * 64, wn * (HC / 2) + 16 * tn, lane);
-                const bf16x8_t w2f = frag(W2Ts + ks * HC * 64, wn * (HC / 2) + 16 * tn, lane);
-#pragma unroll
-                for (int tm = 0; tm < 2; ++tm) {
-                    h[tn][tm] = __builtin_amdgcn_mfma_f32_16x16x32_bf16(w1f, xf[tm], h[tn][tm], 0, 0, 0);
-                    t[tn][tm] = __builtin_amdgcn_mfma_f32_16x16x32_bf16(w2f, df[tm], t[tn][tm], 0, 0, 0);
-                }
-            }
-        }
-#pragma unroll
-        for (int tn = 0; tn < TN1; ++tn) {
-            const int nl = wn * (HC / 2) + 16 * tn + 4 * g;
-            const float4 b = *reinterpret_cast<const float4*>(B1s + j0 + nl);
-            const float bb[4] = {b.x, b.y, b.z, b.w};
-#pragma unroll
-            for (int tm = 0; tm < 2; ++tm) {
-                float a[4], dh[4];
-#pragma unroll
-                for (int r = 0; r < 4; ++r) {
-                    float gr;
-                    gelu_both_fast(h[tn][tm][r] + bb[r], a[r], gr);
-                    dh[r] = t[tn][tm][r] * gr;
-                }
-                const int row = wm * 32 + 16 * tm + (lane & 15);
-                const unsigned o = (nl >> 5) * BM * 64 + slab_off(row, (nl & 31) >> 3) + (nl & 7) * 2;
-                uint2 p;
-                p.x = pack2bf(a[0], a[1]);
-                p.y = pack2bf(a[2], a[3]);
-                *reinterpret_cast<uint2*>(A2s + o) = p;
-                p.x = pack2bf(dh[0], dh[1]);
-                p.y = pack2bf(dh[2], dh[3]);
-                *reinterpret_cast<uint2*>(DHs + o) = p;
-            }
-        }
-        lds_barrier();
-#pragma unroll
-        for (int ks = 0; ks < KS2; ++ks) {
-            bf16x8_t af[2];
-#pragma unroll
-            for (int tm = 0; tm < 2; ++tm) af[tm] = frag(DHs + ks * BM * 64, wm * 32 + 16 * tm, lane);
-#pragma unroll
-            for (int tn = 0; tn < TN2; ++tn) {
-                const bf16x8_t wf = frag(W1Ts + ks * C * 64, wn * (C / 2) + 16 * tn, lane);
-#pragma unroll
-                for (int tm = 0; tm < 2; ++tm) dx[tn][tm] = __builtin_amdgcn_mfma_f32_16x16x32_bf16(wf, af[tm], dx[tn][tm], 0, 0, 0);
-            }
-        }
-        {
-            constexpr int PPR = HC / 8, NP = BM * PPR / 512;
-            static_assert(BM * PPR % 512 == 0, "chunk rows must split evenly");
-#pragma unroll
-            for (int i = 0; i < NP; ++i) {
-                const int idx = tid + 512 * i;
-                const int r = idx / PPR, c = idx - r * PPR;
-                const long m = m0 + r;
-                if (m < d.M) {
-                    const unsigned o = (c >> 2) * BM * 64 + slab_off(r, c & 3);
-                    store16_nt(Aout + m * d.lda + j0 + c * 8, *reinterpret_cast<const uint4*>(A2s + o));
-                    store16_nt(DHout + m * d.lddh + j0 + c * 8, *reinterpret_cast<const uint4*>(DHs + o));
-                }
-            }
-        }
-        if (more) w12_store();
-        lds_barrier();
-        if (more) w3_store();
-    }
-    u32x4_t nopre[BM / 64][RowPre<C, 512>::NR];
-#pragma unroll
-    for (int i = 0; i < BM / 64; ++i)
-#pragma unroll
-        for (int j = 0; j < RowPre<C, 512>::NR; ++j) nopre[i][j] = u32x4_t{0, 0, 0, 0};
-    store_rows<C, 512, 4, 2>(reinterpret_cast<float*>(smem), dx, wm, wn, lane, m0, d.M, nullptr, nullptr, 1, false, nopre,
-                             reinterpret_cast<bf16_t*>(d.DX), d.lddx);
+    if (q || i >= n) return;
+#pragma unroll
+    for (int s = 0; s < 3; ++s) {
+        const float4 b = sh[s][threadIdx.x];
+        a.x += b.x; a.y += b.y; a.z += b.z; a.w += b.w;
+    }
+    float* dst = i < nw ? dW1 + (i / C) * ldw + (i % C) : db1 + (i - nw);
+    dst[0] += a.x; dst[1] += a.y; dst[2] += a.z; dst[3] += a.w;
 }
 
 template <int C, int HC> constexpr int bwd_lds() {
@@ -427,27 +552,78 @@
     return ga_check_launch("ga_mlp_fwd");
 }
 
+extern "C" int ga_mlp_bwd_wgrad_supported(int C, int H, int dtype) { return dtype == GA_BF16 && C == 96 && H == 4 * C; }
+
+namespace {
+
+int num_cus() {
+    static int n = [] {
+        int c = 256;
+        ga_device_info(&c, nullptr, nullptr);
+        return c;
+    }();
+    return n;
+}
+
+int wg_grid(const ga_mlp_bwd_desc* d) {
+    constexpr int lds = bwd_lds<96, 64>();
+    static const int resident = [] {
+        auto kern = mlp_bwd_kernel<96, 64, true>;
+        if (!set_lds(kern, lds)) return 0;
+        int n = 0;
+        if (hipOccupancyMaxActiveBlocksPerMultiprocessor(&n, kern, 512, lds) != hipSuccess || n < 1) n = 1;
+        return n * num_cus();
+    }();
+    long grid = resident;
+    if (d->max_blocks > 0) grid = std::min<long>(grid, d->max_blocks);
+    return (int)std::min<long>(grid, (d->M + BM - 1) / BM);
+}
+
+}
+
+extern "C" size_t ga_mlp_bwd_partials(const ga_mlp_bwd_desc* d) {
+    if (!d || d->M <= 0 || !ga_mlp_bwd_wgrad_supported(d->C, d->H, d->dtype)) return 0;
+    return (size_t)wg_grid(d) * ((size_t)d->H * d->C + d->H) * sizeof(float);
+}
+
 extern "C" int ga_mlp_bwd(const ga_mlp_bwd_desc* d, ga_stream_t stream) {
-    GA_REQUIRE(d && d->X && d->DY && d->W1 && d->b1 && d->W2T && d->W1T && d->A && d->DH && d->DX && d->M > 0,
-               "ga_mlp_bwd: null / empty descriptor");
+    GA_REQUIRE(d && d->X && d->DY && d->W1 && d->b1 && d->W2T && d->W1T && d->DX && d->M > 0, "ga_mlp_bwd: null / empty descriptor");
     GA_REQUIRE(ga_mlp_supported(d->C, d->H, d->dtype), "ga_mlp_bwd: C=%d H=%d dtype=%d has no fused form (ga_mlp_supported)", d->C,
                d->H, d->dtype);
     GA_REQUIRE(aligned16(d->X) && aligned16(d->DY) && aligned16(d->W1) && aligned16(d->W2T) && aligned16(d->W1T) &&
                    aligned16(d->A) && aligned16(d->DH) && aligned16(d->DX) && aligned16(d->b1) && d->ldx % 8 == 0 &&
-                   d->lddy % 8 == 0 && d->ldw1 % 8 == 0 && d->ldw2t % 8 == 0 && d->ldw1t % 8 == 0 && d->lda % 8 == 0 &&
-                   d->lddh % 8 == 0 && d->lddx % 8 == 0 && d->ldx >= d->C && d->lddy >= d->C && d->ldw1 >= d->C &&
-                   d->ldw2t >= d->C && d->ldw1t >= d->H && d->lda >= d->H && d->lddh >= d->H && d->lddx >= d->C,
+                   d->lddy % 8 == 0 && d->ldw1 % 8 == 0 && d->ldw2t % 8 == 0 && d->ldw1t % 8 == 0 && (!d->A || d->lda % 8 == 0) &&
+                   (!d->DH || d->lddh % 8 == 0) && d->lddx % 8 == 0 && d->ldx >= d->C && d->lddy >= d->C && d->ldw1 >= d->C &&
+                   d->ldw2t >= d->C && d->ldw1t >= d->H && (!d->A || d->lda >= d->H) && (!d->DH || d->lddh >= d->H) &&
+                   d->lddx >= d->C,
                "ga_mlp_bwd: operands must be 16-byte aligned with leading dimensions in multiples of 8");
     hipStream_t s = reinterpret_cast<hipStream_t>(stream);
+    if (d->dW1) {
+        GA_REQUIRE(ga_mlp_bwd_wgrad_supported(d->C, d->H, d->dtype),
+                   "ga_mlp_bwd: dW1 is accumulated in the kernel at C=96 only, not C=%d H=%d dtype=%d (ga_mlp_bwd_wgrad_supported)",
+                   d->C, d->H, d->dtype);
+        GA_REQUIRE(d->db1 && d->partials && aligned16(d->partials) && d->ldw >= d->C && d->max_blocks >= 0,
+                   "ga_mlp_bwd: dW1 needs db1, 16-byte aligned partials and ldw >= C");
+        constexpr int lds = bwd_lds<96, 64>();
+        const int grid = wg_grid(d);
+        GA_REQUIRE(grid > 0, "ga_mlp_bwd: LDS");
+        const int n = d->H * d->C + d->H;
+        GA_REQUIRE(d->partials_bytes >= (size_t)grid * n * sizeof(float), "ga_mlp_bwd: partials holds %zu bytes, %zu needed (ga_mlp_bwd_partials)",
+                   (size_t)d->partials_bytes, (size_t)grid * n * sizeof(float));
+        hipLaunchKernelGGL((mlp_bwd_kernel<96, 64, true>), dim3(grid), dim3(512), lds, s, *d);
+        hipLaunchKernelGGL(mlp_bwd_wg_reduce_kernel, dim3((n / 4 + 63) / 64), dim3(256), 0, s, d->partials, grid, n, d->H * d->C, d->C,
+                           d->dW1, (long)d->ldw, d->db1);
+        return ga_check_launch("ga_mlp_bwd");
+    }
     const unsigned grid = (unsigned)((d->M + BM - 1) / BM);
     if (d->C == 96) {
         constexpr int lds = bwd_lds<96, 64>();
-        GA_REQUIRE(set_lds(mlp_bwd_kernel<96, 64>, lds), "ga_mlp_bwd: LDS");
-        hipLaunchKernelGGL((mlp_bwd_kernel<96, 64>), dim3(grid), dim3(512), lds, s, *d);
+        GA_REQUIRE(set_lds(mlp_bwd_kernel<96, 64, false>, lds), "ga_mlp_bwd: LDS");
+        hipLaunchKernelGGL((mlp_bwd_kernel<96, 64, false>), dim3(grid), dim3(512), lds, s, *d);
     } else {
         constexpr int lds = bwd_lds<192, 32>();
-        GA_REQUIRE(set_lds(mlp_bwd_kernel<192, 32>, lds), "ga_mlp_bwd: LDS");
-        hipLaunchKernelGGL((mlp_bwd_kernel<192, 32>), dim3(grid), dim3(512), lds, s, *d);
+        GA_REQUIRE(set_lds(mlp_bwd_kernel<192, 32, false>, lds), "ga_mlp_bwd: LDS");
+        hipLaunchKernelGGL((mlp_bwd_kernel<192, 32, false>), dim3(grid), dim3(512), lds, s, *d);
     }
     return ga_check_launch("ga_mlp_bwd");
 }
diff --git a/imagenet-models_amd/engine.py b/imagenet-models_amd/engine.py
--- a/imagenet-models_amd/engine.py
+++ b/imagenet-models_amd/engine.py
@@ -48,6 +48,7 @@
         self.bufs = {}
         self.tmps = {}
         self.async_wgrad = os.environ.get('GAEXT_ASYNC_WGRAD', '1') != '0'
+        self.mlp_wg1 = os.environ.get('GAEXT_MLP_WG1', '1') != '0'
         self.fwd_split = max(1, int(os.environ.get('GAEXT_FWD_SPLIT', '2')))
         self.par_branch = os.environ.get('GAEXT_PAR_BRANCH', '1') != '0'
         self.fwd_skew = int(os.environ.get('GAEXT_FWD_SKEW', '-1'))
@@ -509,12 +510,20 @@
         wl = ASYNC_LANE if side else Bk.lane
         ml = Bk.lane
         G2, gb2 = self.gbuf((C, 4 * C)), self.gbuf((C,))
-        dh = self.tmp('dh' + par, (M, 4 * C))
         gb1 = self.gbuf((4 * C,))
         G1 = self.gbuf((4 * C, C))
         g = self.tmp('g', (M, C))
-        if b['fused']:
+        if b['fused'] and self.mlp_wg1 and ops.mlp_bwd_wgrad_supported(C, 4 * C, dt):
             a = self.tmp('a' + par, (M, 4 * C))
+            part = self.tmp('mlpwg' + par, (ops.mlp_bwd_partials(M, C, dt) // 4,), torch.float32)
+            Bk.mlp_bwd(b['xn'], dyz, W[pre + self.NAMES['fc1'] + 'weight'], W[pre + 'b1e'], W[pre + self.NAMES['fc2'] + 'weight.T'],
+                       W[pre + self.NAMES['fc1'] + 'weight.T'], a, None, g, M, C, dt, dW1=G1, db1=gb1, partials=part, label=pre + 'mlpb')
+            Bk.lane = wl
+            Bk.wgrad(dyz, a, G2, M, C, 4 * C, dt, dbias=gb2, label=pre + 'wg2')
+            Bk.lane = ml
+        elif b['fused']:
+            a = self.tmp('a' + par, (M, 4 * C))
+            dh = self.tmp('dh' + par, (M, 4 * C))
             Bk.mlp_bwd(b['xn'], dyz, W[pre + self.NAMES['fc1'] + 'weight'], W[pre + 'b1e'], W[pre + self.NAMES['fc2'] + 'weight.T'],
                        W[pre + self.NAMES['fc1'] + 'weight.T'], a, dh, g, M, C, dt, label=pre + 'mlpb')
             Bk.lane = wl
@@ -522,6 +531,7 @@
             Bk.wgrad(dh, b['xn'], G1, M, 4 * C, C, dt, dbias=gb1, label=pre + 'wg1')
             Bk.lane = ml
         else:
+            dh = self.tmp('dh' + par, (M, 4 * C))
             Bk.lane = wl
             Bk.wgrad(dyz, b['a'], G2, M, C, 4 * C, dt, dbias=gb2, label=pre + 'wg2')
             Bk.lane = ml
diff --git a/imagenet-models_amd/ops.py b/imagenet-models_amd/ops.py
--- a/imagenet-models_amd/ops.py
+++ b/imagenet-models_amd/ops.py
@@ -411,7 +411,8 @@
         d.Y, d.ldy, d.M, d.C, d.H, d.dtype = _ptr(Y), Cdim, M, Cdim, H, dtype
         self._add('ga_mlp_fwd', (C.byref(d),), label, keep=(d, X, W1, b1, W2, b2, R, rowscale, Y))
 
-    def mlp_bwd(self, X, DY, W1, b1, W2T, W1T, A, DH, DX, M, Cdim, dtype, ldw1=None, ldw2t=None, ldw1t=None, label=None):
+    def mlp_bwd(self, X, DY, W1, b1, W2T, W1T, A, DH, DX, M, Cdim, dtype, ldw1=None, ldw2t=None, ldw1t=None, label=None,
+                dW1=None, db1=None, partials=None, max_blocks=0):
         d = L.MlpBwdDesc()
         H = 4 * Cdim
         d.X, d.ldx, d.DY, d.lddy = _ptr(X), Cdim, _ptr(DY), Cdim
@@ -419,7 +420,12 @@
         d.W2T, d.ldw2t, d.W1T, d.ldw1t = _ptr(W2T), (Cdim if ldw2t is None else ldw2t), _ptr(W1T), (H if ldw1t is None else ldw1t)
         d.A, d.lda, d.DH, d.lddh, d.DX, d.lddx = _ptr(A), H, _ptr(DH), H, _ptr(DX), Cdim
         d.M, d.C, d.H, d.dtype = M, Cdim, H, dtype
-        self._add('ga_mlp_bwd', (C.byref(d),), label, keep=(d, X, DY, W1, b1, W2T, W1T, A, DH, DX))
+        if dW1 is not None:
+            assert dW1.dtype == torch.float32 and db1 is not None and db1.dtype == torch.float32 and partials is not None
+            assert dW1.stride(-1) == 1 and partials.dtype == torch.float32 and partials.is_contiguous()
+            d.dW1, d.ldw, d.db1 = _ptr(dW1), dW1.stride(0), _ptr(db1)
+            d.partials, d.partials_bytes, d.max_blocks = _ptr(partials), partials.numel() * 4, max_blocks
+        self._add('ga_mlp_bwd', (C.byref(d),), label, keep=(d, X, DY, W1, b1, W2T, W1T, A, DH, DX, dW1, db1, partials))
 
     def wgrad(self, Y, X, dW, M, N, K, dtype, ldy=None, ldx=None, ldw=None, batch=1, strideY=0, strideX=0, strideW=0,
               x_kind=A_PLAIN, x_dims=(0, 0, 0), x_act=ACT_NONE, dbias=None, strideDbias=0, alpha=1.0, split_m=None,
@@ -895,6 +901,16 @@
     return bool(L.load().ga_mlp_supported(Cdim, H, dtype))
 
 
+def mlp_bwd_wgrad_supported(Cdim, H, dtype):
+    return bool(L.load().ga_mlp_bwd_wgrad_supported(Cdim, H, dtype))
+
+
+def mlp_bwd_partials(M, Cdim, dtype, max_blocks=0):
+    d = L.MlpBwdDesc()
+    d.M, d.C, d.H, d.dtype, d.max_blocks = M, Cdim, 4 * Cdim, dtype, max_blocks
+    return int(L.load().ga_mlp_bwd_partials(C.byref(d)))
+
+
 def cswin_attn_bwd_workspace(d):
     return int(L.load().ga_cswin_attn_bwd_workspace(C.byref(d)))
 
diff --git a/include/gaext.h b/include/gaext.h
--- a/include/gaext.h
+++ b/include/gaext.h
@@ -346,10 +346,16 @@
     void* DH; int64_t lddh;
     void* DX; int64_t lddx;
     int64_t M; int C, H, dtype;
+    float* dW1; int64_t ldw;
+    float* db1;
+    float* partials; size_t partials_bytes;
+    int max_blocks;
 } ga_mlp_bwd_desc;
 int ga_mlp_supported(int C, int H, int dtype);
 int ga_mlp_fwd(const ga_mlp_desc* d, ga_stream_t stream);
 int ga_mlp_bwd(const ga_mlp_bwd_desc* d, ga_stream_t stream);
+int ga_mlp_bwd_wgrad_supported(int C, int H, int dtype);
+size_t ga_mlp_bwd_partials(const ga_mlp_bwd_desc* d);
 
 typedef struct {
     int rows, groups, Ng, Kg;
```

Result: faster. 10930 images/sec, median of 6 (+1.5%).
